# aleflabo/COSKAD

Hardware: AMD Instinct MI355X
Metric: pose_clips_per_sec_fwd_bwd (higher is better)
Workload: dtype f32; 1 GPU; euclidean_encoder_dynamicCenter train step (fwd+mse-to-centre+L2 reg+bwd+Adam), synthetic clips B=4096/GPU T=12 V=17 C=2, channels 2-32-16-32-64, latent 16; clips_per_gpu=4096, global_batch=4096, head=euclidean, parallelism=dp1, hip_graph=False

## Files before the change

coskad_amd/csrc/bottleneck.hip:

```cpp
#include "tile_ops.h"

namespace coskad {

constexpr int kBtlBlock = 256;
constexpr int kBtlWaves = kBtlBlock / 64;
constexpr int kBtlFwdWaves = 8;

__global__ __launch_bounds__(64 * kBtlFwdWaves) void k_btlnk_fwd(const float* __restrict__ U,
                                                     const float* __restrict__ W,
                                                     const float* __restrict__ bias,
                                                     const float* __restrict__ slope,
                                                     float* __restrict__ z, int B, int K, int L) {
  __shared__ float red[kBtlFwdWaves][256];
  const int lane = threadIdx.x & 63, wave = threadIdx.x >> 6;
  const int i = lane & 15, kk = lane >> 4;
  const int n = blockIdx.x * 16 + i;
  const bool pre = slope != nullptr;
  const float a = pre ? slope[0] : 0.f;
  const bool rowok = n < B, colok = i < L;
  const float* up = U + (size_t)(rowok ? n : 0) * K;
  const float* wp = W + (size_t)(colok ? i : 0) * K;
  const int nsteps = ceil_div(K, 16);
  const int per = ceil_div(nsteps, kBtlFwdWaves);
  const int s0 = wave * per, s1 = min(nsteps, s0 + per);
  f32x4 acc = {0.f, 0.f, 0.f, 0.f};
  constexpr int UB = 4;
  for (int sb = s0; sb < s1; sb += UB) {
    float4 x[UB], w[UB];
#pragma unroll
    for (int u = 0; u < UB; ++u) {
      const int k = (sb + u) * 16 + 4 * kk;
      const bool ok = sb + u < s1 && k < K;
      x[u] = (ok && rowok) ? *reinterpret_cast<const float4*>(up + k) : float4{0.f, 0.f, 0.f, 0.f};
      w[u] = (ok && colok) ? *reinterpret_cast<const float4*>(wp + k) : float4{0.f, 0.f, 0.f, 0.f};
    }
#pragma unroll
    for (int u = 0; u < UB; ++u) {
      float4 xv = x[u];
      if (pre) { xv.x = prelu_f(xv.x, a); xv.y = prelu_f(xv.y, a); xv.z = prelu_f(xv.z, a); xv.w = prelu_f(xv.w, a); }
      acc = __builtin_amdgcn_mfma_f32_16x16x4f32(xv.x, w[u].x, acc, 0, 0, 0);
      acc = __builtin_amdgcn_mfma_f32_16x16x4f32(xv.y, w[u].y, acc, 0, 0, 0);
      acc = __builtin_amdgcn_mfma_f32_16x16x4f32(xv.z, w[u].z, acc, 0, 0, 0);
      acc = __builtin_amdgcn_mfma_f32_16x16x4f32(xv.w, w[u].w, acc, 0, 0, 0);
    }
  }
#pragma unroll
  for (int r = 0; r < 4; ++r) red[wave][(4 * (lane >> 4) + r) * 16 + (lane & 15)] = acc[r];
  __syncthreads();
  const int e = threadIdx.x, row = (e >> 4) & 15, col = e & 15;
  const int nn = blockIdx.x * 16 + row;
  if (e < 256 && nn < B && col < L) {
    float s = 0.f;
#pragma unroll
// ... 124 lines not shown
#pragma unroll
    for (int g = 0; g < 4; ++g) {
      const int nn = n0 + c, j = 4 * g + q;
      const float av = (nn < nend && j < L) ? dz[(size_t)nn * L + j] : 0.f;
      dx[0] = __builtin_amdgcn_mfma_f32_16x16x4f32(av, wf[g].x, dx[0], 0, 0, 0);
      dx[1] = __builtin_amdgcn_mfma_f32_16x16x4f32(av, wf[g].y, dx[1], 0, 0, 0);
      dx[2] = __builtin_amdgcn_mfma_f32_16x16x4f32(av, wf[g].z, dx[2], 0, 0, 0);
      dx[3] = __builtin_amdgcn_mfma_f32_16x16x4f32(av, wf[g].w, dx[3], 0, 0, 0);
    }
#pragma unroll
    for (int s = 0; s < 4; ++s) {
      const int nn = n0 + 4 * q + s;
      const bool ok = kok && nn < nend;
      const float4 u = ucur[s];
      float4 x = u;
      if (pre) { x.x = prelu_f(u.x, a); x.y = prelu_f(u.y, a); x.z = prelu_f(u.z, a); x.w = prelu_f(u.w, a); }
      const float dzv = (nn < nend && c < L) ? dz[(size_t)nn * L + c] : 0.f;
      dw[0] = __builtin_amdgcn_mfma_f32_16x16x4f32(dzv, x.x, dw[0], 0, 0, 0);
      dw[1] = __builtin_amdgcn_mfma_f32_16x16x4f32(dzv, x.y, dw[1], 0, 0, 0);
      dw[2] = __builtin_amdgcn_mfma_f32_16x16x4f32(dzv, x.z, dw[2], 0, 0, 0);
      dw[3] = __builtin_amdgcn_mfma_f32_16x16x4f32(dzv, x.w, dw[3], 0, 0, 0);
      float4 g = {dx[0][s], dx[1][s], dx[2][s], dx[3][s]};
      if (pre) {
        da += (u.x < 0.f ? g.x * u.x : 0.f) + (u.y < 0.f ? g.y * u.y : 0.f) +
              (u.z < 0.f ? g.z * u.z : 0.f) + (u.w < 0.f ? g.w * u.w : 0.f);
        g.x = u.x > 0.f ? g.x : a * g.x; g.y = u.y > 0.f ? g.y : a * g.y;
        g.z = u.z > 0.f ? g.z : a * g.z; g.w = u.w > 0.f ? g.w : a * g.w;
      }
      if (ok) *reinterpret_cast<float4*>(dU + (size_t)nn * K + kc) = g;
    }
#pragma unroll
    for (int s = 0; s < 4; ++s) ucur[s] = unext[s];
  }
  if (kok) {
    float* dst = dWp + (size_t)blockIdx.y * L * K;
#pragma unroll
    for (int r = 0; r < 4; ++r) {
      const int j = 4 * q + r;
      if (j < L) *reinterpret_cast<float4*>(dst + (size_t)j * K + kc) = float4{dw[0][r], dw[1][r], dw[2][r], dw[3][r]};
    }
  }
  da = wave_sum(da);
  if (lane == 0) sred[wave] = da;
  __syncthreads();
  if (threadIdx.x == 0) dap[blockIdx.y * gridDim.x + blockIdx.x] = (sred[0] + sred[1]) + (sred[2] + sred[3]);
}

__global__ __launch_bounds__(256) void k_btlnk_reduce(const float* __restrict__ partials, int P, size_t E,
                                                       float* __restrict__ out, const float* __restrict__ dz,
                                                       int B, int L, float* __restrict__ db,
                                                       const float* __restrict__ dap, int nda,
                                                       float* __restrict__ dslope, int accumulate,
                                                       const float* __restrict__ rows, int RP, int RE,
                                                       double* __restrict__ rsum) {
  __shared__ double sh[256];
  const unsigned nE = (unsigned)((E + 255) / 256);
  if (blockIdx.x > nE + L) {
    const int col = threadIdx.x & 15, slice = threadIdx.x >> 4;
    const int e = (int)(blockIdx.x - (nE + L + 1)) * 16 + col;
    double s = 0.0;
    if (e < RE) {
      const float* base = rows + e;
      int p = slice;
      for (; p + 7 * 16 < RP; p += 8 * 16) {
        float v[8];
#pragma unroll
        for (int u = 0; u < 8; ++u) v[u] = base[(size_t)(p + 16 * u) * RE];
#pragma unroll
        for (int u = 0; u < 8; ++u) s += (double)v[u];
      }
      for (; p < RP; p += 16) s += (double)base[(size_t)p * RE];
    }
    sh[threadIdx.x] = s;
    __syncthreads();
    if (slice == 0 && e < RE) {
      double t = 0.0;
#pragma unroll
      for (int k = 0; k < 16; ++k) t += sh[col + 16 * k];
      rsum[e] = t;
    }
    return;
  }
  if (blockIdx.x < nE) {
    const size_t e = (size_t)blockIdx.x * 256 + threadIdx.x;
    if (e >= E) return;
    double s = 0.0;
    int p = 0;
    for (; p + 8 <= P; p += 8) {
      float v[8];
#pragma unroll
      for (int u = 0; u < 8; ++u) v[u] = partials[(size_t)(p + u) * E + e];
#pragma unroll
      for (int u = 0; u < 8; ++u) s += (double)v[u];
    }
    for (; p < P; ++p) s += (double)partials[(size_t)p * E + e];
    out[e] = accumulate ? out[e] + (float)s : (float)s;
    return;
  }
  const int r = (int)(blockIdx.x - nE);
  double s = 0.0;
  if (r < L) {
    if (!db) return;
    for (int n = threadIdx.x; n < B; n += 256) s += (double)dz[(size_t)n * L + r];
  } else {
    if (!dslope) return;
    for (int i = threadIdx.x; i < nda; i += 256) s += (double)dap[i];
  }
  sh[threadIdx.x] = s;
  __syncthreads();
  for (int w = 128; w > 0; w >>= 1) {
    if ((int)threadIdx.x < w) sh[threadIdx.x] += sh[threadIdx.x + w];
    __syncthreads();
  }
  if (threadIdx.x == 0) {
    float* o = r < L ? db + r : dslope;
    o[0] = accumulate ? o[0] + (float)sh[0] : (float)sh[0];
  }
}

static int btl_chunks(int B, int K) {
  const int gx = ceil_div(K, 256);
  int s = (1024 + gx / 2) / gx;
  const int smax = ceil_div(B, 16);
  if (s > smax) s = smax;
  if (s > 64) s = 64;
  return s < 1 ? 1 : s;
}

int launch_btlnk_reduce(const float* partials, int P, size_t E, float* out, const float* dz, int B, int L, float* db,
                        const float* dap, int nda, float* dslope, int accumulate, hipStream_t stream, const float* rows,
                        int RP, int RE, double* rsum) {
  const unsigned extra = rows ? (unsigned)ceil_div(RE, 16) : 0u;
  hipLaunchKernelGGL(k_btlnk_reduce, dim3((unsigned)((E + 255) / 256) + L + 1 + extra), dim3(256), 0, stream, partials, P, E, out, dz,
                     B, L, db, dap, nda, dslope, accumulate, rows, RP, RE, rsum);
  return check_launch("btlnk_bwd_reduce");
}

constexpr int kBtlWideMax = 512;
size_t wide_btlnk_fwd_ws_bytes(int B, int K, int L);
size_t wide_btlnk_bwd_ws_bytes(int B, int K, int L);
int wide_btlnk_fwd(const float* U, const float* W, const float* bias, const float* slope, float* z, void* ws, int B, int K, int L,
                   hipStream_t stream);
int wide_btlnk_bwd(const float* U, const float* W, const float* dz, const float* slope, float* dU, float* dW, float* db,
                   float* dslope, void* ws, int accumulate, int B, int K, int L, hipStream_t stream);

}

using namespace coskad;

extern "C" {

int coskad_btlnk_fwd_f32(const float* U, const float* W, const float* bias, const float* slope, float* z,
                         int B, int K, int L, hipStream_t stream) {
  if (!U || !W || !z) return fail(COSKAD_ERR_ARG, "btlnk_fwd: null pointer");
  if (B <= 0 || K <= 0 || L <= 0) return fail(COSKAD_ERR_ARG, "btlnk_fwd: B=%d K=%d L=%d", B, K, L);
  if (L > 16) return fail(COSKAD_ERR_SHAPE, "btlnk_fwd: latent_dim=%d > 16 needs the workspace entry point coskad_btlnk_fwd_ws_f32", L);
  if (K % 4) return fail(COSKAD_ERR_SHAPE, "btlnk_fwd: K=%d must be a multiple of 4", K);
  hipLaunchKernelGGL(k_btlnk_fwd, dim3(ceil_div(B, 16)), dim3(64 * kBtlFwdWaves), 0, stream, U, W, bias, slope, z, B, K, L);
  return check_launch("btlnk_fwd");
}

size_t coskad_btlnk_fwd_ws_bytes(int B) { return (size_t)kBtlKS * (size_t)(B > 0 ? B : 0) * 16 * sizeof(float); }

size_t coskad_btlnk_fwd_ws_bytes_l(int B, int K, int L) {
  if (L > 16 && L <= kBtlWideMax) return wide_btlnk_fwd_ws_bytes(B, K, L);
  return coskad_btlnk_fwd_ws_bytes(B);
}

int coskad_btlnk_fwd_ws_f32(const float* U, const float* W, const float* bias, const float* slope, float* z, void* ws,
                            size_t ws_bytes, int B, int K, int L, hipStream_t stream) {
  if (!U || !W || !z || !ws) return fail(COSKAD_ERR_ARG, "btlnk_fwd_ws: null pointer");
  if (B <= 0 || K <= 0 || L <= 0) return fail(COSKAD_ERR_ARG, "btlnk_fwd_ws: B=%d K=%d L=%d", B, K, L);
  if (L > kBtlWideMax) return fail(COSKAD_ERR_SHAPE, "btlnk_fwd_ws: latent_dim=%d > %d not supported", L, kBtlWideMax);
  if (L > 16) {
    if (ws_bytes < wide_btlnk_fwd_ws_bytes(B, K, L)) return fail(COSKAD_ERR_WORKSPACE, "btlnk_fwd_ws: workspace too small");
    return wide_btlnk_fwd(U, W, bias, slope, z, ws, B, K, L, stream);
  }
  if (K % 16) return fail(COSKAD_ERR_SHAPE, "btlnk_fwd_ws: K=%d must be a multiple of 16", K);
  if (ws_bytes < coskad_btlnk_fwd_ws_bytes(B)) return fail(COSKAD_ERR_WORKSPACE, "btlnk_fwd_ws: workspace too small");
  float* part = reinterpret_cast<float*>(ws);
  hipLaunchKernelGGL(k_btlnk_fwd_t, dim3(ceil_div(B, 64), kBtlKS), dim3(256), 0, stream, U, W, slope, part, B, K, L);
  int rc;
  if ((rc = check_launch("btlnk_fwd_t"))) return rc;
  hipLaunchKernelGGL(k_btlnk_fwd_sum, dim3(ceil_div(B * 16, 256)), dim3(256), 0, stream, part, bias, z, B, L, kBtlKS);
  return check_launch("btlnk_fwd_sum");
}

size_t coskad_btlnk_bwd_ws_bytes(int B, int K, int L) {
  if (L > 16 && L <= kBtlWideMax) return wide_btlnk_bwd_ws_bytes(B, K, L);
  const int S = btl_chunks(B, K);
  return ((size_t)S * L * K + (size_t)S * ceil_div(K, 256) + 64) * sizeof(float);
}

int coskad_btlnk_bwd_f32(const float* U, const float* W, const float* dz, const float* slope, float* dU,
                         float* dW, float* db, float* dslope, void* ws, size_t ws_bytes, int accumulate,
                         int B, int K, int L, hipStream_t stream) {
  if (!U || !W || !dz || !dU || !dW || !ws) return fail(COSKAD_ERR_ARG, "btlnk_bwd: null pointer");
  if (B <= 0 || K <= 0 || L <= 0) return fail(COSKAD_ERR_ARG, "btlnk_bwd: B=%d K=%d L=%d", B, K, L);
  if (L > kBtlWideMax) return fail(COSKAD_ERR_SHAPE, "btlnk_bwd: latent_dim=%d > %d not supported", L, kBtlWideMax);
  if (ws_bytes < coskad_btlnk_bwd_ws_bytes(B, K, L)) return fail(COSKAD_ERR_WORKSPACE, "btlnk_bwd: workspace too small");
  if (L > 16) return wide_btlnk_bwd(U, W, dz, slope, dU, dW, db, dslope, ws, accumulate, B, K, L, stream);
  if (K % 4) return fail(COSKAD_ERR_SHAPE, "btlnk_bwd: K=%d must be a multiple of 4", K);
  const int S = btl_chunks(B, K);
  const int chunk = round_up(ceil_div(B, S), 16);
  const int gx = ceil_div(K, 256);
  float* dWp = reinterpret_cast<float*>(ws);
  float* dap = dWp + (size_t)S * L * K;
  {
    ProbeScope probe(KID_BTLNK_BWD, 0, L, stream);
    hipLaunchKernelGGL(k_btlnk_bwd, dim3(gx, S), dim3(kBtlBlock), 0, stream, U, W, dz, slope, dU, dWp, dap, B, K, L, chunk);
  }
  int rc = check_launch("btlnk_bwd");
  if (rc) return rc;
  return launch_btlnk_reduce(dWp, S, (size_t)L * K, dW, dz, B, L, db, dap, gx * S, (dslope && slope) ? dslope : nullptr, accumulate, stream,
                             nullptr, 0, 0, nullptr);
}

}
```

coskad_amd/csrc/btlnk_chain.hip:

```cpp
#include "fused_ops.h"

namespace coskad {
namespace bc {

using ff::f32x4; using ff::mfma; using ff::BufRes; using ff::make_res; using ff::buf_load4; using ff::buf_load1;
__device__ __forceinline__ void buf_store1(BufRes r, int voff, int soff, float v) {
  __builtin_amdgcn_raw_buffer_store_b32(__float_as_uint(v), r, voff, soff, 0);
}

constexpr int HID = 64;
constexpr int PT = 16;
constexpr int NCL = 16;
constexpr int RSTR = 17;
constexpr int kThreads = 512;
#ifndef BC_XCD
#define BC_XCD 1
#endif
#ifndef BC_PF
#define BC_PF 1
#endif
#ifndef BC_SKIP
#define BC_SKIP 0
#endif

// ... 172 lines not shown
        if (j < L && pok) dst[(size_t)j * K + (ch0 + i) * TV] = dw[i][r];
      }
  }
  float* row = lds;
  float* red = lds + E;
  const float s4 = ssum + __shfl_xor(ssum, 16, 64);
  const float sch = s4 + __shfl_xor(s4, 32, 64);
  da = wave_sum(da);
  for (int hh = 0; hh < 2; ++hh) {
    if (h == hh) {
#pragma unroll
      for (int t = 0; t < CT; ++t)
#pragma unroll
        for (int r = 0; r < 4; ++r) {
          const int o = 16 * wc + 4 * q + r, cc = 16 * t + c;
          float* p = row + o * Ci + cc;
          p[0] = (hh ? p[0] : 0.f) + pacc[t][r];
          p[HID * Ci] = (hh ? p[HID * Ci] : 0.f) + qacc[t][r];
        }
      if (q == 0) {
        float* p = row + 2 * HID * Ci + 16 * wc + c;
        p[0] = (hh ? p[0] : 0.f) + sch;
      }
      if (lane == 0) red[wave] = da;
    }
    __syncthreads();
  }
  float* dstrow = prow + (size_t)wg * E;
  for (int e = tid; e < E; e += kThreads) dstrow[e] = row[e];
  if (tid == 0) dap[wg] = ((red[0] + red[1]) + (red[2] + red[3])) + ((red[4] + red[5]) + (red[6] + red[7]));
}

struct Plan {
  int npt, S, chunk;
};
static Plan plan(int B, int TV) {
  Plan p;
  p.npt = ceil_div(TV, PT);
  int s = 256 / p.npt;
  const int smax = ceil_div(B, NCL);
  if (s > smax) s = smax;
  if (s < 1) s = 1;
  p.chunk = round_up(ceil_div(B, s), NCL);
  p.S = ceil_div(B, p.chunk);
  return p;
}
static inline size_t sums_offset(int rows, int E) { return ((size_t)rows * E + 1) / 2 * 2; }

}

int launch_btlnk_reduce(const float* partials, int P, size_t E, float* out, const float* dz, int B, int L, float* db,
                        const float* dap, int nda, float* dslope, int accumulate, hipStream_t stream, const float* rows,
                        int RP, int RE, double* rsum);
}

using namespace coskad;

extern "C" {

int coskad_btlnk_bwd_chain_ok(int K, int TV, int below_Ci) {
  return TV > 0 && TV % 4 == 0 && K == bc::HID * TV && (below_Ci == 16 || below_Ci == 32);
}

int coskad_btlnk_bwd_chain_rows(int B, int TV) {
  if (B <= 0 || TV <= 0) return 0;
  const bc::Plan p = bc::plan(B, TV);
  return p.npt * p.S;
}

size_t coskad_btlnk_bwd_chain_floats(int B, int TV, int below_Ci) {
  const size_t E = 2 * (size_t)bc::HID * below_Ci + bc::HID;
  return bc::sums_offset(coskad_btlnk_bwd_chain_rows(B, TV), (int)E) + 2 * E;
}

size_t coskad_btlnk_bwd_chain_ws_bytes(int B, int K, int L, int TV) {
  if (B <= 0 || TV <= 0) return 0;
  const bc::Plan p = bc::plan(B, TV);
  return ((size_t)p.S * L * K + (size_t)p.S * p.npt + 64) * sizeof(float);
}

int coskad_btlnk_bwd_chain_f32(const float* U, const float* W, const float* dz, const float* slope, float* dU, float* dW,
                               float* db, float* dslope, void* ws, size_t ws_bytes, int accumulate, int B, int K, int L,
                               const float* below_in, const float* below_Z, const float* below_in_slope, int below_Ci, int TV,
                               float* stats_out, size_t stats_out_bytes, int* stats_rows, hipStream_t stream) {
  if (!U || !W || !dz || !dU || !dW || !ws || !below_in || !below_Z || !stats_out || !stats_rows)
    return fail(COSKAD_ERR_ARG, "btlnk_bwd_chain: null pointer");
  if (B <= 0 || K <= 0 || L <= 0) return fail(COSKAD_ERR_ARG, "btlnk_bwd_chain: B=%d K=%d L=%d", B, K, L);
  if (L > 16) return fail(COSKAD_ERR_SHAPE, "btlnk_bwd_chain: latent_dim=%d > 16 not supported", L);
  if (!coskad_btlnk_bwd_chain_ok(K, TV, below_Ci))
    return fail(COSKAD_ERR_SHAPE, "btlnk_bwd_chain: K=%d TV=%d below_Ci=%d (needs K = 64 TV, TV %% 4 == 0, 16 / 32 channels below)", K, TV, below_Ci);
  if ((size_t)stats_out & 7) return fail(COSKAD_ERR_ARG, "btlnk_bwd_chain: stats_out must be 8-byte aligned");
  if (ws_bytes < coskad_btlnk_bwd_chain_ws_bytes(B, K, L, TV)) return fail(COSKAD_ERR_WORKSPACE, "btlnk_bwd_chain: workspace too small");
  if (stats_out_bytes < coskad_btlnk_bwd_chain_floats(B, TV, below_Ci) * sizeof(float))
    return fail(COSKAD_ERR_WORKSPACE, "btlnk_bwd_chain: stats_out %zu bytes too small", stats_out_bytes);
  const bc::Plan p = bc::plan(B, TV);
  const int rows = p.npt * p.S;
  const int E = 2 * bc::HID * below_Ci + bc::HID;
  float* dWp = reinterpret_cast<float*>(ws);
  float* dap = dWp + (size_t)p.S * L * K;
  const size_t lds = (size_t)bc::NCL * ((bc::HID * bc::RSTR + 4) + (2 * below_Ci * bc::RSTR + 4)) * sizeof(float);
  int rc;
  {
  ProbeScope probe(KID_BTLNK_BWD, below_Ci, L, stream);
  if (below_Ci == 32) {
    auto k = bc::k_btlnk_bwd_stats<2>;
    (void)hipFuncSetAttribute((const void*)k, hipFuncAttributeMaxDynamicSharedMemorySize, (int)lds);
    hipLaunchKernelGGL(k, dim3(p.npt * p.S), dim3(bc::kThreads), lds, stream, U, W, dz, slope, dU, dWp, dap, below_in, below_Z,
                       below_in_slope, stats_out, B, TV, L, p.chunk);
  } else {
    auto k = bc::k_btlnk_bwd_stats<1>;
    (void)hipFuncSetAttribute((const void*)k, hipFuncAttributeMaxDynamicSharedMemorySize, (int)lds);
    hipLaunchKernelGGL(k, dim3(p.npt * p.S), dim3(bc::kThreads), lds, stream, U, W, dz, slope, dU, dWp, dap, below_in, below_Z,
                       below_in_slope, stats_out, B, TV, L, p.chunk);
  }
  }
  if ((rc = check_launch("btlnk_bwd_stats"))) return rc;
  *stats_rows = rows;
  return launch_btlnk_reduce(dWp, p.S, (size_t)L * K, dW, dz, B, L, db, dap, rows, (dslope && slope) ? dslope : nullptr, accumulate, stream,
                             stats_out, rows, E, reinterpret_cast<double*>(stats_out + bc::sums_offset(rows, E)));
}

}
```

coskad_amd/csrc/fused_apply_next.hip:

```cpp
#include "fused_ops.h"

#ifndef FN_ABLATE
#define FN_ABLATE 0
#endif

namespace coskad {
namespace fn {

using namespace ff;

struct FtabArgs {
  const float* A[4];
  const float* Tm[4];
  float* tab[4];
};
__global__ void k_build_ftab(FtabArgs args) {
  const int layer = blockIdx.y;
  const float* __restrict__ Aw = args.A[layer];
  const float* __restrict__ Tw = args.Tm[layer];
  const int e = blockIdx.x * blockDim.x + threadIdx.x;
  if (e >= LAYER_F4 * 4) return;
  float val = 0.f;
  if (e < TEMP_F4 * 4) {
    const int v = e / 256, l = (e >> 2) & 63, s = e & 3, j = l & 15, q = l >> 4;
    if (s < 3 && j < T) val = Tw[v * T * T + (4 * s + q) * T + j];
  } else {
    const int r = e - TEMP_F4 * 4;
    const int t = r / (3 * 256), c = (r / 256) % 3, l = (r >> 2) & 63, k = 4 * c + (r & 3), j = l & 15, q = l >> 4;
    if (k < 10) {
      const int s = k < 5 ? k : k - 5, w = 4 * s + q;
      if (w < V) val = Aw[t * V * V + w * V + (k < 5 ? j : 16)];
    }
  }
  args.tab[layer][e] = val;
}

template <int CT, int OTP>
__global__ __launch_bounds__(256, 1) void k_layer_apply_next(const float* __restrict__ in, const float* __restrict__ Zg,
                                                            const float* __restrict__ wfold, const float* __restrict__ bias,
                                                            const float* __restrict__ in_slope, const float* __restrict__ out_slope,
                                                            const float* __restrict__ ftab, float* __restrict__ out,
                                                            float* __restrict__ Znext, float* __restrict__ partials, int B) {
  constexpr int Ci = CT ? 16 * CT : 2, Co = 16 * OTP, CoP = Co, NG = 2 * CT;
  constexpr int NACC = OTP == 1 ? 2 : 3;
  constexpr int E = 2 * (Co * Co + Co);
  static_assert(OTP == 1 || OTP == 2, "the 32-row image holds the whole output");
  extern __shared__ __attribute__((aligned(16))) float lds_all[];
  const int lane = threadIdx.x & 63;
  const int wave = __builtin_amdgcn_readfirstlane(threadIdx.x >> 6);
  float* lds = lds_all + wave * WAVE_LDS_W;
  float* r1 = lds + R1;
  float* r2 = lds + R2;
  auto geo = [&]() {
    int l = lane;
    asm volatile("" : "+v"(l));
    return Lane{l & 15, l >> 4};
  };
  auto olane = [&]() {
    int l = lane;
    asm volatile("" : "+v"(l));
    return l;
  };
  const bool pre = in_slope != nullptr;
  const float a_in = pre ? in_slope[0] : 0.f;
  const float a_out = out_slope[0];
  const int l16 = lane * 16;
  const BufRes wres = make_res(wfold, 2 * Ci * CoP * 4u);
  const BufRes bres = make_res(bias, CoP * 4u);
  const BufRes tabres = make_res(ftab, LAYER_F4 * 16u);
  const int nwaves = gridDim.x * 4;
  auto clip_res = [&](const float* base, int c, int rows) {
    const bool in_range = c < B;
#ifdef COSKAD_HOT
    return make_res(base + (size_t)(in_range ? (c & 63) : 0) * rows * TV, in_range ? rows * TV * 4u : 0u);
#else
    return make_res(base + (size_t)(in_range ? c : 0) * rows * TV, in_range ? rows * TV * 4u : 0u);
#endif
  };
  constexpr int QTAIL = 4 * (TV / 4) - 192;
  const int l16t = lane < QTAIL ? l16 : 0x7ffffff0;
  float4 gb[16];
  auto qload = [&](const BufRes& res, int row0, int q) {
#pragma unroll
    for (int c = 0; c < 4; ++c) gb[4 * q + c] = buf_load4(res, c < 3 ? l16 : l16t, ((row0 + 4 * q) * (TV / 4) + 64 * c) * 16);
  };
  auto qstore = [&](int q, bool act) {
    const int ln = olane();
// ... 337 lines not shown
```

coskad_amd/csrc/fused_ops.h:

```cpp
#pragma once
#include "common.h"

namespace coskad {
namespace ff {

using f32x4 = __attribute__((ext_vector_type(4))) float;

constexpr int T = 12, V = 17, TV = T * V;
#ifndef FF_LD
#define FF_LD 206
#endif
constexpr int LD = FF_LD;
constexpr int R1 = 0, R2 = 32 * LD;
constexpr int PADCOL = TV;
constexpr int WAVE_LDS = 48 * LD;
constexpr int LDW = 208;
constexpr int WAVE_LDS_W = 32 * LD + 16 * LDW;
constexpr int NTILE = T + 1;
#ifndef FF_AB_UNROLL
#define FF_AB_UNROLL _Pragma("unroll")
#endif
#ifndef FF_ABLATE
#define FF_ABLATE 0
#endif
#ifndef FF_CABL
#define FF_CABL 0
#endif
#ifndef FF_TILE_FENCE
#define FF_TILE_FENCE
#endif
constexpr int KP = NTILE * 4 * 64 * 4;
constexpr int TEMP_F4 = V * 64;
constexpr int LAYER_F4 = TEMP_F4 + T * 3 * 64;
enum { W1A = 0, W1B = 2, WP = 4, WR = 12, WX3 = 20, WZ3 = 28, WZ4 = 36, WX4 = 68, B1 = 100, B2 = 108, B3 = 112, B4 = 120, NWREG = 136 };

__device__ __forceinline__ f32x4 mfma(float a, float b, f32x4 c) {
  return __builtin_amdgcn_mfma_f32_16x16x4f32(a, b, c, 0, 0, 0);
}
__device__ __forceinline__ float prelu(float x, float a) { return x > 0.f ? x : a * x; }
__device__ __forceinline__ f32x4 prelu4(f32x4 v, float a) {
  return f32x4{prelu(v[0], a), prelu(v[1], a), prelu(v[2], a), prelu(v[3], a)};
}

struct Lane {
  int j, q;
};

using u32x4 = __attribute__((ext_vector_type(4))) unsigned int;
using BufRes = __amdgpu_buffer_rsrc_t;
__device__ __forceinline__ BufRes make_res(const void* p, unsigned bytes) {
  return __builtin_amdgcn_make_buffer_rsrc(const_cast<void*>(p), 0, bytes, 0x00020000);
}
__device__ __forceinline__ float4 buf_load4(BufRes r, int voff, int soff) {
  const u32x4 v = __builtin_amdgcn_raw_buffer_load_b128(r, voff, soff, 0);
  return float4{__uint_as_float(v[0]), __uint_as_float(v[1]), __uint_as_float(v[2]), __uint_as_float(v[3])};
}
__device__ __forceinline__ float buf_load1(BufRes r, int voff, int soff) {
  return __uint_as_float(__builtin_amdgcn_raw_buffer_load_b32(r, voff, soff, 0));
}
__device__ __forceinline__ void buf_store4(BufRes r, int voff, int soff, const float4& v) {
  const u32x4 u = {__float_as_uint(v.x), __float_as_uint(v.y), __float_as_uint(v.z), __float_as_uint(v.w)};
  __builtin_amdgcn_raw_buffer_store_b128(u, r, voff, soff, 0);
}

struct TOp {
  float a0, a1, a2;
};
template <int ROWS, bool ACT = false>
__device__ __forceinline__ TOp temporal_read(const float* img, int rt, int v, const Lane& L, float slope = 0.f) {
  const float* p = img + (16 * rt + L.j) * LD + L.q * V + v;
  TOp o{p[0], p[4 * V], p[8 * V]};
  if (ACT) { o.a0 = prelu(o.a0, slope); o.a1 = prelu(o.a1, slope); o.a2 = prelu(o.a2, slope); }
  if (ROWS < 16) {
    const bool ok = L.j < ROWS;
    o.a0 = ok ? o.a0 : 0.f; o.a1 = ok ? o.a1 : 0.f; o.a2 = ok ? o.a2 : 0.f;
  }
  return o;
}
__device__ __forceinline__ f32x4 temporal_mm(const TOp& o, const float4& rec) {
  f32x4 acc = {0.f, 0.f, 0.f, 0.f};
  acc = mfma(o.a0, rec.x, acc);
  acc = mfma(o.a1, rec.y, acc);
  acc = mfma(o.a2, rec.z, acc);
  return acc;
}
template <int ROWS>
__device__ __forceinline__ void temporal_store(float* img, int rt, int v, const f32x4& acc, const Lane& L) {
// ... 229 lines not shown
```

coskad_amd/csrc/heads.hip:

```cpp
#include "tile_ops.h"
#include "heads_common.h"

namespace coskad {

struct Vec {
  float v[LMAX];
};

__device__ __forceinline__ Vec load_vec(const float* p, int L) {
  Vec r;
#pragma unroll
  for (int j = 0; j < LMAX; ++j) r.v[j] = j < L ? p[j] : 0.f;
  return r;
}
__device__ __forceinline__ void store_vec(float* p, const Vec& a, int L) {
#pragma unroll
  for (int j = 0; j < LMAX; ++j)
    if (j < L) p[j] = a.v[j];
}
__device__ __forceinline__ float dot(const Vec& a, const Vec& b) {
  float s = 0.f;
#pragma unroll
  for (int j = 0; j < LMAX; ++j) s = fmaf(a.v[j], b.v[j], s);
  return s;
// ... 31 lines not shown
  const float D = den + kMobiusEps;
  Vec m;
#pragma unroll
  for (int j = 0; j < LMAX; ++j) m.v[j] = (alpha * (-c.v[j]) + beta * p.v[j]) / D;
  const float mn = sqrtf(dot(m, m));
  const float mc = fminf(fmaxf(mn, -1.f + kArtanhEps), 1.f - kArtanhEps);
  const float d = (log1pf(mc) - log1pf(-mc));
  if (gp) {
    const float gmn = 2.f / (1.f - mc * mc);
    const float inv = mn > 0.f ? gmn / mn : 0.f;
    Vec gm;
#pragma unroll
    for (int j = 0; j < LMAX; ++j) gm.v[j] = inv * m.v[j];
    const float gD = -dot(gm, m) / D;
    float galpha = 0.f;
#pragma unroll
    for (int j = 0; j < LMAX; ++j) galpha = fmaf(gm.v[j] / D, -c.v[j], galpha);
#pragma unroll
    for (int j = 0; j < LMAX; ++j) {
      const float x = -c.v[j], y = p.v[j];
      gp->v[j] = beta * gm.v[j] / D + galpha * (2.f * x + 2.f * y) + gD * (2.f * x + 2.f * x2 * y);
    }
  }
  return d;
}

__device__ __forceinline__ Vec hyp_embed_bwd(const Vec& u, const Embed& em, const Vec& gp) {
  const float f = em.tn / em.un;
  Vec ge;
  if (em.clamped) {
    const float maxnorm = 1.f - kBallEps;
    const float en = em.en_raw;
    float egp = 0.f;
#pragma unroll
    for (int j = 0; j < LMAX; ++j) egp = fmaf(f * u.v[j], gp.v[j], egp);
#pragma unroll
    for (int j = 0; j < LMAX; ++j) ge.v[j] = maxnorm * (gp.v[j] / en - f * u.v[j] * egp / (en * en * en));
  } else {
    ge = gp;
  }
  Vec gu;
  float gf = dot(ge, u);
  float coef = 0.f;
  if (em.un_raw > kMinNorm) {
    const float sech2 = em.un < kTanhClamp ? 1.f - em.tn * em.tn : 0.f;
    const float df = (sech2 * em.un - em.tn) / (em.un * em.un);
    coef = gf * df / em.un_raw;
  }
#pragma unroll
  for (int j = 0; j < LMAX; ++j) gu.v[j] = f * ge.v[j] + coef * u.v[j];
  return gu;
}

constexpr int kHeadSlots = LMAX + 3;

constexpr int kHeadSingleRows = kFlatBlock;
__host__ __device__ inline int head_blocks(int B) { return B <= kHeadSingleRows ? 1 : ceil_div(B, kFlatBlock); }

__device__ __forceinline__ void block_partials(const float (&vals)[kHeadSlots], float* partials, float scale0, float* stats,
                                               float* acc) {
  __shared__ float sh[kFlatBlock / 64][kHeadSlots];
  const int lane = threadIdx.x & 63, wave = threadIdx.x >> 6;
#pragma unroll
  for (int k = 0; k < kHeadSlots; ++k) {
    const float s = wave_sum(vals[k]);
    if (lane == 0) sh[wave][k] = s;
  }
  __syncthreads();
  if (threadIdx.x < kHeadSlots) {
    float s = 0.f;
    for (int w = 0; w < kFlatBlock / 64; ++w) s += sh[w][threadIdx.x];
    if (gridDim.x == 1) {
      if (stats) stats[threadIdx.x] = threadIdx.x == 0 ? s * scale0 : s;
      if (acc) acc[threadIdx.x] += s;
    } else {
      partials[blockIdx.x * kHeadSlots + threadIdx.x] = s;
    }
  }
}

__global__ __launch_bounds__(kFlatBlock) void k_mse_head(const float* __restrict__ z,
                                                    const float* __restrict__ cvec,
                                                    float* __restrict__ dz, float* __restrict__ score,
                                                    float* __restrict__ partials, int B, int L,
                                                    float gscale, float scale0, float* __restrict__ stats,
                                                    float* __restrict__ acc) {
  float vals[kHeadSlots];
#pragma unroll
  for (int k = 0; k < kHeadSlots; ++k) vals[k] = 0.f;
  const Vec c = load_vec(cvec, L);
#pragma unroll 4
  for (int n = blockIdx.x * kFlatBlock + threadIdx.x; n < B; n += gridDim.x * kFlatBlock) {
    const Vec u = load_vec(z + (size_t)n * L, L);
    Vec g;
    float sq = 0.f;
#pragma unroll
    for (int j = 0; j < LMAX; ++j) {
      const float d = j < L ? u.v[j] - c.v[j] : 0.f;
      sq = fmaf(d, d, sq);
      g.v[j] = 2.f * d * gscale;
      vals[1 + j] += u.v[j];
    }
    vals[0] += sq;
    vals[LMAX + 1] += 1.f;
    vals[LMAX + 2] += sqrtf(dot(u, u));
    if (dz) store_vec(dz + (size_t)n * L, g, L);
    if (score) score[n] = sq / (float)L;
  }
  block_partials(vals, partials, scale0, stats, acc);
}

__global__ __launch_bounds__(kFlatBlock) void k_mahalanobis_head(const float* __restrict__ z,
                                                            const float* __restrict__ cvec,
                                                            const float* __restrict__ VI,
                                                            float* __restrict__ dz, float* __restrict__ score,
                                                            float* __restrict__ partials, int B, int L,
                                                            float gscale, float scale0, float* __restrict__ stats,
                                                            float* __restrict__ acc) {
  __shared__ float vi[LMAX * LMAX];
  for (int e = threadIdx.x; e < LMAX * LMAX; e += kFlatBlock) {
    const int r = e / LMAX, q = e - r * LMAX;
    vi[e] = (r < L && q < L) ? VI[r * L + q] : 0.f;
  }
  __syncthreads();
  float vals[kHeadSlots];
#pragma unroll
  for (int k = 0; k < kHeadSlots; ++k) vals[k] = 0.f;
  const Vec c = load_vec(cvec, L);
  for (int n = blockIdx.x * kFlatBlock + threadIdx.x; n < B; n += gridDim.x * kFlatBlock) {
    const Vec u = load_vec(z + (size_t)n * L, L);
    Vec d, w, wt;
#pragma unroll
    for (int j = 0; j < LMAX; ++j) { d.v[j] = j < L ? u.v[j] - c.v[j] : 0.f; w.v[j] = 0.f; wt.v[j] = 0.f; }
#pragma unroll
    for (int r = 0; r < LMAX; ++r)
#pragma unroll
      for (int q = 0; q < LMAX; ++q) {
        const float a = vi[r * LMAX + q];
        w.v[r] = fmaf(a, d.v[q], w.v[r]);
        wt.v[q] = fmaf(a, d.v[r], wt.v[q]);
      }
    const float dist = sqrtf(dot(d, w));
    vals[0] += dist;
#pragma unroll
    for (int j = 0; j < LMAX; ++j) vals[1 + j] += u.v[j];
    vals[LMAX + 1] += 1.f;
// ... 19 lines not shown
  for (int n0 = 0; n0 < B; n0 += CH) {
    const int nc = min(CH, B - n0);
    __syncthreads();
    for (int e = threadIdx.x; e < nc * L; e += LMAX * LMAX) {
      const int r = e / L, q = e - r * L;
      zs[r * LMAX + q] = z[(size_t)(n0 + r) * L + q];
    }
    __syncthreads();
    if (i < L && j < L)
      for (int r = 0; r < nc; ++r) s = fmaf(zs[r * LMAX + i], zs[r * LMAX + j], s);
  }
  if (i < L && j < L) gram[i * L + j] = accumulate ? gram[i * L + j] + s : s;
}

__global__ __launch_bounds__(kFlatBlock) void k_poincare_head(const float* __restrict__ z,
                                                         const float* __restrict__ cvec,
                                                         float* __restrict__ dz, float* __restrict__ zh,
                                                         float* __restrict__ score,
                                                         float* __restrict__ partials, int B, int L,
                                                         float gscale, float scale0, float* __restrict__ stats,
                                                         float* __restrict__ acc) {
  float vals[kHeadSlots];
#pragma unroll
  for (int k = 0; k < kHeadSlots; ++k) vals[k] = 0.f;
  for (int n = blockIdx.x * kFlatBlock + threadIdx.x; n < B; n += gridDim.x * kFlatBlock) {
    const Vec u = load_vec(z + (size_t)n * L, L);
    const Embed em = hyp_embed(u);
    if (zh) store_vec(zh + (size_t)n * L, em.p, L);
    const float y2 = dot(em.p, em.p);
    const float gamma = 2.f / (1.f - y2);
#pragma unroll
    for (int j = 0; j < LMAX; ++j) vals[1 + j] += gamma * em.p.v[j];
    vals[LMAX + 1] += gamma - 1.f;
    vals[LMAX + 2] += sqrtf(y2);
    if (cvec) {
      const Vec c = load_vec(cvec, L);
      Vec gp;
      const float d = poincare_dist(c, em.p, dz ? &gp : nullptr);
      vals[0] += d;
      if (score) score[n] = d;
      if (dz) {
#pragma unroll
        for (int j = 0; j < LMAX; ++j) gp.v[j] *= gscale;
        store_vec(dz + (size_t)n * L, hyp_embed_bwd(u, em, gp), L);
      }
    }
  }
  block_partials(vals, partials, scale0, stats, acc);
}

__global__ __launch_bounds__(64) void k_head_finalize(const float* __restrict__ partials, int P,
                                                       float scale0, float* __restrict__ stats,
                                                       float* __restrict__ acc) {
  const int k = threadIdx.x;
  if (k >= kHeadSlots) return;
  double s = 0.0;
  for (int p = 0; p < P; ++p) s += (double)partials[p * kHeadSlots + k];
  if (stats) stats[k] = (float)(k == 0 ? s * (double)scale0 : s);
  if (acc) acc[k] += (float)s;
}

__global__ __launch_bounds__(kFlatBlock) void k_poincare_dist(const float* __restrict__ zh,
                                                         const float* __restrict__ cvec,
                                                         float* __restrict__ score, int B, int L) {
  const int n = blockIdx.x * kFlatBlock + threadIdx.x;
  if (n >= B) return;
  const Vec p = load_vec(zh + (size_t)n * L, L), c = load_vec(cvec, L);
  score[n] = poincare_dist(c, p, nullptr);
}

__global__ __launch_bounds__(kFlatBlock) void k_poincare_logmap0(const float* __restrict__ y, float* __restrict__ out, int B, int L) {
  const int n = blockIdx.x * kFlatBlock + threadIdx.x;
  if (n >= B) return;
  const Vec p = load_vec(y + (size_t)n * L, L);
  const float yn = fmaxf(sqrtf(dot(p, p)), kMinNorm);
  const float yc = fminf(fmaxf(yn, -1.f + kArtanhEps), 1.f - kArtanhEps);
  const float at = 0.5f * (log1pf(yc) - log1pf(-yc));
  Vec o;
#pragma unroll
  for (int j = 0; j < LMAX; ++j) o.v[j] = p.v[j] / yn * at;
  store_vec(out + (size_t)n * L, o, L);
}

__global__ void k_midpoint_finalize(const float* __restrict__ acc, float* __restrict__ cvec, int L) {
  if (threadIdx.x != 0 || blockIdx.x != 0) return;
  const double s = fmax((double)acc[LMAX + 1], 1e-10);
  double m[LMAX], mn2 = 0.0;
  for (int j = 0; j < L; ++j) { m[j] = (double)acc[1 + j] / s; mn2 += m[j] * m[j]; }
  const double mn = fmax(sqrt(mn2), 1e-15);
  const double mc = fmin(mn, 1.0 - 1e-7);
  const double at = 0.5 * log((1.0 + mc) / (1.0 - mc));
  const double sc = tanh(0.5 * at) / mn;
  for (int j = 0; j < L; ++j) cvec[j] = (float)(sc * m[j]);
}

__global__ void k_center_finalize(const float* __restrict__ acc, float eps, float* __restrict__ cvec,
                                  int L) {
  const int j = threadIdx.x;
  if (j >= L || blockIdx.x != 0) return;
  float c = acc[1 + j] / acc[LMAX + 1];
  if (fabsf(c) < eps && c < 0.f) c = -eps;
  if (fabsf(c) < eps && c > 0.f) c = eps;
  cvec[j] = c;
}

__global__ __launch_bounds__(256) void k_sqnorm_masked(const float* __restrict__ p,
                                                        const float* __restrict__ mask, size_t n,
                                                        float* __restrict__ partials) {
  __shared__ float sh[4];
  float s = 0.f;
  for (size_t i = (size_t)blockIdx.x * 256 + threadIdx.x; i < n; i += (size_t)gridDim.x * 256) {
    const float v = p[i];
// ... 12 lines not shown
                                               float bc2_sqrt, float gscale, float reg_coef) {
  const size_t i = (size_t)blockIdx.x * 256 + threadIdx.x;
  if (i >= n) return;
  const float pi = p[i];
  float gi = g[i] * gscale;
  if (reg_coef != 0.f) gi = fmaf(reg_coef * (mask ? mask[i] : 1.f), pi, gi);
  const float mi = beta1 * m[i] + (1.f - beta1) * gi;
  const float vi = beta2 * v[i] + (1.f - beta2) * gi * gi;
  m[i] = mi;
  v[i] = vi;
  const float denom = sqrtf(vi) / bc2_sqrt + eps;
  p[i] = pi - (lr / bc1) * (mi / denom);
}

__global__ void k_adam_tick(float* __restrict__ hyper, float beta1, float beta2) {
  if (threadIdx.x == 0 && blockIdx.x == 0) {
    hyper[1] *= beta1;
    hyper[2] *= beta2;
  }
}

__global__ __launch_bounds__(256) void k_adam_dev(float* __restrict__ p, const float* __restrict__ g,
                                                   float* __restrict__ m, float* __restrict__ v,
                                                   const float* __restrict__ mask, size_t n,
                                                   const float* __restrict__ hyper, float beta1, float beta2,
                                                   float eps, float gscale, float reg_coef) {
  const size_t i = (size_t)blockIdx.x * 256 + threadIdx.x;
  if (i >= n) return;
  const float lr = hyper[0], bc1 = 1.f - hyper[1], bc2s = sqrtf(1.f - hyper[2]);
  const float pi = p[i];
  float gi = g[i] * gscale;
  if (reg_coef != 0.f) gi = fmaf(reg_coef * (mask ? mask[i] : 1.f), pi, gi);
  const float mi = beta1 * m[i] + (1.f - beta1) * gi;
  const float vi = beta2 * v[i] + (1.f - beta2) * gi * gi;
  m[i] = mi;
  v[i] = vi;
  p[i] = pi - (lr / bc1) * (mi / (sqrtf(vi) / bc2s + eps));
}

__global__ __launch_bounds__(256) void k_scale_sum(const float* __restrict__ v, int n, float scale,
                                                    float* __restrict__ out) {
  __shared__ double sh[256];
  double s = 0.0;
  for (int i = threadIdx.x; i < n; i += 256) s += (double)v[i];
  sh[threadIdx.x] = s;
  __syncthreads();
  for (int w = 128; w > 0; w >>= 1) {
    if (threadIdx.x < w) sh[threadIdx.x] += sh[threadIdx.x + w];
    __syncthreads();
  }
  if (threadIdx.x == 0) out[0] = (float)(sh[0] * (double)scale);
}

}

using namespace coskad;

extern "C" {

int coskad_head_slots(void) { return kHeadSlots; }
size_t coskad_head_ws_floats(int B) { return (size_t)ceil_div(B, kFlatBlock) * kHeadSlots; }
int coskad_head_slots_l(int L) { return L > 0 && L <= kWideLMax ? head_slots_for(L) : 0; }
size_t coskad_head_ws_floats_l(int B, int L) {
  if (L > LMAX && L <= kWideLMax) return wide_head_ws_floats(B, L);
  return coskad_head_ws_floats(B);
}

int coskad_mse_head_f32(const float* z, const float* c, float* dz, float* score, float* stats, float* acc,
                        float upstream, float* ws, int B, int L, hipStream_t stream) {
  if (!z || !c || !ws) return fail(COSKAD_ERR_ARG, "mse_head: null pointer");
  if (B <= 0 || L <= 0 || L > kWideLMax) return fail(COSKAD_ERR_SHAPE, "mse_head: B=%d latent=%d (max %d)", B, L, kWideLMax);
  if (L > LMAX) return wide_mse_head(z, c, dz, score, stats, acc, upstream, ws, B, L, stream);
  const int P = head_blocks(B);
  hipLaunchKernelGGL(k_mse_head, dim3(P), dim3(kFlatBlock), 0, stream, z, c, dz, score, ws, B, L,
                     upstream / ((float)B * (float)L), 1.f / ((float)B * (float)L), stats, acc);
  if ((stats || acc) && P > 1)
    hipLaunchKernelGGL(k_head_finalize, dim3(1), dim3(64), 0, stream, ws, P, 1.f / ((float)B * (float)L), stats, acc);
  return check_launch("mse_head");
}

int coskad_mahalanobis_head_f32(const float* z, const float* c, const float* VI, float* dz, float* score,
                                float* stats, float* acc, float* gram, int gram_accumulate, float upstream,
                                float* ws, int B, int L, hipStream_t stream) {
  if (!z || !c || !VI || !ws) return fail(COSKAD_ERR_ARG, "mahalanobis_head: null pointer");
  if (B <= 0 || L <= 0 || L > kWideLMax) return fail(COSKAD_ERR_SHAPE, "mahalanobis_head: B=%d latent=%d (max %d)", B, L, kWideLMax);
  if (L > LMAX) return wide_mahalanobis_head(z, c, VI, dz, score, stats, acc, gram, gram_accumulate, upstream, ws, B, L, stream);
  const int P = head_blocks(B);
  hipLaunchKernelGGL(k_mahalanobis_head, dim3(P), dim3(kFlatBlock), 0, stream, z, c, VI, dz, score, ws, B, L,
                     upstream / (float)B, 1.f / (float)B, stats, acc);
  if ((stats || acc) && P > 1)
    hipLaunchKernelGGL(k_head_finalize, dim3(1), dim3(64), 0, stream, ws, P, 1.f / (float)B, stats, acc);
  if (gram) hipLaunchKernelGGL(k_gram, dim3(1), dim3(LMAX * LMAX), 0, stream, z, gram, B, L, gram_accumulate);
  return check_launch("mahalanobis_head");
}

int coskad_poincare_head_f32(const float* z, const float* c, float* dz, float* zh, float* score,
                             float* stats, float* acc, float upstream, float* ws, int B, int L,
                             hipStream_t stream) {
  if (!z || !ws) return fail(COSKAD_ERR_ARG, "poincare_head: null pointer");
  if (B <= 0 || L <= 0 || L > kWideLMax) return fail(COSKAD_ERR_SHAPE, "poincare_head: B=%d latent=%d (max %d)", B, L, kWideLMax);
  if (L > LMAX) return wide_poincare_head(z, c, dz, zh, score, stats, acc, upstream, ws, B, L, stream);
  const int P = head_blocks(B);
  hipLaunchKernelGGL(k_poincare_head, dim3(P), dim3(kFlatBlock), 0, stream, z, c, dz, zh, score, ws, B, L,
                     upstream / (float)B, 1.f / (float)B, stats, acc);
  if ((stats || acc) && P > 1)
    hipLaunchKernelGGL(k_head_finalize, dim3(1), dim3(64), 0, stream, ws, P, 1.f / (float)B, stats, acc);
  return check_launch("poincare_head");
}

int coskad_poincare_dist_f32(const float* zh, const float* c, float* score, int B, int L, hipStream_t stream) {
  if (!zh || !c || !score) return fail(COSKAD_ERR_ARG, "poincare_dist: null pointer");
  if (B <= 0 || L <= 0 || L > kWideLMax) return fail(COSKAD_ERR_SHAPE, "poincare_dist: B=%d latent=%d (max %d)", B, L, kWideLMax);
  if (L > LMAX) return wide_poincare_dist(zh, c, score, B, L, stream);
  hipLaunchKernelGGL(k_poincare_dist, dim3(ceil_div(B, kFlatBlock)), dim3(kFlatBlock), 0, stream, zh, c, score, B, L);
  return check_launch("poincare_dist");
}

int coskad_poincare_logmap0_f32(const float* y, float* out, int B, int L, hipStream_t stream) {
  if (!y || !out) return fail(COSKAD_ERR_ARG, "poincare_logmap0: null pointer");
  if (B <= 0 || L <= 0 || L > kWideLMax) return fail(COSKAD_ERR_SHAPE, "poincare_logmap0: B=%d latent=%d (max %d)", B, L, kWideLMax);
  if (L > LMAX) return wide_poincare_logmap0(y, out, B, L, stream);
  hipLaunchKernelGGL(k_poincare_logmap0, dim3(ceil_div(B, kFlatBlock)), dim3(kFlatBlock), 0, stream, y, out, B, L);
  return check_launch("poincare_logmap0");
}

int coskad_center_finalize_f32(const float* acc, float* c, float eps, int L, hipStream_t stream) {
  if (!acc || !c || L <= 0 || L > kWideLMax) return fail(COSKAD_ERR_ARG, "center_finalize: bad argument (latent=%d, max %d)", L, kWideLMax);
// ... 52 lines not shown
```

coskad_amd/csrc/heads_common.h:

```cpp
#pragma once
#include "common.h"

namespace coskad {

constexpr int LMAX = 16;
constexpr int kWideLMax = 512;
constexpr float kMinNorm = 1e-5f;
constexpr float kBallEps = 1e-3f;
constexpr float kArtanhEps = 1e-5f;
constexpr float kMobiusEps = 1e-5f;
constexpr float kTanhClamp = 15.f;

__host__ __device__ inline int head_lp(int L) { return L > LMAX ? L : LMAX; }
__host__ __device__ inline int head_slots_for(int L) { return head_lp(L) + 3; }

size_t wide_head_ws_floats(int B, int L);
int wide_mse_head(const float* z, const float* c, float* dz, float* score, float* stats, float* acc, float upstream, float* ws,
                  int B, int L, hipStream_t stream);
int wide_mahalanobis_head(const float* z, const float* c, const float* VI, float* dz, float* score, float* stats, float* acc,
                          float* gram, int gram_accumulate, float upstream, float* ws, int B, int L, hipStream_t stream);
int wide_poincare_head(const float* z, const float* c, float* dz, float* zh, float* score, float* stats, float* acc,
                       float upstream, float* ws, int B, int L, hipStream_t stream);
int wide_poincare_dist(const float* zh, const float* c, float* score, int B, int L, hipStream_t stream);
int wide_poincare_logmap0(const float* y, float* out, int B, int L, hipStream_t stream);
int wide_center_finalize(const float* acc, float* c, float eps, int L, hipStream_t stream);
int wide_midpoint_finalize(const float* acc, float* c, int L, hipStream_t stream);

}
```

coskad_amd/csrc/stsgcn_train.hip:

```cpp
#include "mfma_ops.h"

namespace coskad {

constexpr int kMaxGrid = 768;

template <int T, int V, int NTC>
__global__ __launch_bounds__((Geo<T, V>::Block), (Geo<T, V>::Block <= 512 && NTC <= 2 ? 6 : 4)) void k_fwd_moments(const float* __restrict__ in,
                                                       const float* __restrict__ Aw,
                                                       const float* __restrict__ Tw,
                                                       const float* __restrict__ in_slope,
                                                       float* __restrict__ partials, int B, int Ci,
                                                       int NB, int need_x, float* __restrict__ Zout) {
  constexpr int kScratchFloats = Geo<T, V>::Scratch;
  constexpr int TV = Geo<T, V>::TV, LD = TV + 2;
  extern __shared__ __attribute__((aligned(16))) float lds[];
  float* scratch = lds;
  float* AwL = lds + max(NB * Ci * LD, kScratchFloats);
  float* TwL = AwL + T * V * V;
  copy_to_lds(AwL, Aw, T * V * V);
  copy_to_lds(TwL, Tw, V * T * T);
  const bool pre = in_slope != nullptr;
  const float a_in = pre ? in_slope[0] : 0.f;
  f32x4 mx[NTC][NTC], mz[NTC][NTC];
  float sx[NTC], sz[NTC];
  zero_acc(mx); zero_acc(mz);
#pragma unroll
  for (int t = 0; t < NTC; ++t) { sx[t] = 0.f; sz[t] = 0.f; }

  const int ntiles = ceil_div(B, NB);
  for (int tile = blockIdx.x; tile < ntiles; tile += gridDim.x) {
    const int clip0 = tile * NB;
    const int nb = min(NB, B - clip0);
    const int rows = nb * Ci;
    lds_barrier();
    stage_rows<T, V, LD>(in + (size_t)clip0 * Ci * TV, lds, rows * TV, pre, a_in);
    lds_barrier();
    if (need_x) {
      for (int n = 0; n < nb; ++n) moment_accum<T, V, NTC, LD>(lds + n * Ci * LD, Ci, mx, sx);
      lds_barrier();
    }
    gcn_mfma<T, V, false, LD>(lds, rows, AwL, TwL);
    lds_barrier();
    if (Zout) unstage_rows<T, V, LD>(Zout + (size_t)clip0 * Ci * TV, lds, rows * TV);
    for (int n = 0; n < nb; ++n) moment_accum<T, V, NTC, LD>(lds + n * Ci * LD, Ci, mz, sz);
  }
  float* dst = partials + (size_t)blockIdx.x * (2 * (Ci * Ci + Ci));
  store_moments<NTC>(mx, sx, scratch, dst, Ci, dst + Ci * Ci, Ci);
  store_moments<NTC>(mz, sz, scratch, dst + Ci * Ci + Ci, Ci, dst + 2 * Ci * Ci + Ci, Ci);
}

constexpr int kRedCols = 16;
__global__ __launch_bounds__(1024) void k_reduce_partials(const float* __restrict__ partials, int P, int E,
                                                           double* __restrict__ out) {
  __shared__ double sh[1024];
  const int e = blockIdx.x * kRedCols + (threadIdx.x % kRedCols);
  const double t = column_sum_f64<kRedCols>(partials, P, (size_t)E, e, e < E, sh);
  if ((int)threadIdx.x < kRedCols && e < E) out[e] = t;
}

__host__ __device__ inline int stat_floats(int Ci, int Co) { return 2 * Ci + 2 * Co * Ci + 4 * Co; }

#ifdef COSKAD_FOLD_TIMING
__device__ long long g_tfold_stamps[16];
#define TFOLD_STAMP(k) do { if (threadIdx.x == 0) g_tfold_stamps[k] = wall_clock64(); } while (0)
#else
#define TFOLD_STAMP(k) do {} while (0)
#endif

constexpr int kFoldSelfSum = 48;
__global__ __launch_bounds__(1024) void k_train_fold(
    const double* __restrict__ red, double npos, const float* __restrict__ Wt,
    const float* __restrict__ bt, const float* __restrict__ gs, const float* __restrict__ bs,
    float* __restrict__ rm_s, float* __restrict__ rv_s, long long* __restrict__ nbt_s,
    const float* __restrict__ Wr, const float* __restrict__ br, const float* __restrict__ gr,
    const float* __restrict__ brr, float* __restrict__ rm_r, float* __restrict__ rv_r,
    long long* __restrict__ nbt_r, float momentum, float* __restrict__ wfold,
    float* __restrict__ bias, float* __restrict__ stat, int Ci, int Co, int CoP,
    const float* __restrict__ parts, int P) {
  extern __shared__ double shd[];
  const bool ident = Wr == nullptr;
  const int CC = Co * Ci;
  double* Cl = shd;
  double* mul = shd + 2 * Ci * Ci;
  float* Wl = reinterpret_cast<float*>(mul + 2 * Ci);
  float* WCl = Wl + 2 * CC;
  float* meanl = WCl + 2 * CC;
  float* istdl = meanl + 2 * Co;
  __shared__ double red_l[kFoldSelfSum];
  if (parts) {
    __shared__ double shs[1024];
    const int E = 2 * (Ci * Ci + Ci);
    for (int e0 = 0; e0 < E; e0 += kRedCols) {
      const int e = e0 + (int)(threadIdx.x % kRedCols);
      const double t = column_sum_f64<kRedCols>(parts, P, (size_t)E, e, e < E, shs);
      if ((int)threadIdx.x < kRedCols && e < E) red_l[e] = t;
      __syncthreads();
    }
  }
  const double* redp = parts ? red_l : red;
  const double* MX = redp;
  const double* SX = redp + Ci * Ci;
  const double* MZ = redp + Ci * Ci + Ci;
  const double* SZ = redp + 2 * Ci * Ci + Ci;
  float* muX = stat;
  float* muZ = stat + Ci;
  float* WCs = stat + 2 * Ci;
  float* WCr = WCs + CC;
  float* mean_s = WCr + CC;
  float* istd_s = mean_s + Co;
  float* mean_r = istd_s + Co;
  float* istd_r = mean_r + Co;
  const double inv_n = 1.0 / npos;
  const int chunk = (Co + gridDim.x - 1) / gridDim.x;
  const int o_lo = blockIdx.x * chunk, o_hi = min(Co, o_lo + chunk), no = max(0, o_hi - o_lo);
  const bool first = blockIdx.x == 0;

  TFOLD_STAMP(0);
  for (int c = threadIdx.x; c < Ci; c += blockDim.x) {
    const double mz = SZ[c] * inv_n, mx = SX[c] * inv_n;
    mul[c] = mz;
    mul[Ci + c] = mx;
    if (first) { muZ[c] = (float)mz; muX[c] = (float)mx; }
  }
  for (int i = threadIdx.x; i < CC; i += blockDim.x) {
    Wl[i] = Wt[i];
    Wl[CC + i] = ident ? 0.f : Wr[i];
  }
  for (int i = threadIdx.x; i < Ci * Ci; i += blockDim.x) {
    const int k = i / Ci, c = i - k * Ci;
    Cl[i] = MZ[i] * inv_n - (SZ[k] * inv_n) * (SZ[c] * inv_n);
    Cl[Ci * Ci + i] = ident ? 0.0 : MX[i] * inv_n - (SX[k] * inv_n) * (SX[c] * inv_n);
  }
  __syncthreads();
  TFOLD_STAMP(1);
  const int Cq = (Ci + 3) / 4;
  for (int i = threadIdx.x; i < 2 * no * Cq; i += blockDim.x) {
    const int b = i / (no * Cq);
    const int j = i - b * no * Cq;
    const int o = o_lo + j / Cq, c0 = 4 * (j % Cq);
    double a0 = 0.0, a1 = 0.0, a2 = 0.0, a3 = 0.0;
    if (!(b == 1 && ident)) {
      const float* W = Wl + b * CC + o * Ci;
      const double* C = Cl + b * Ci * Ci + c0;
      if (c0 + 3 < Ci) {
        for (int k = 0; k < Ci; ++k) {
          const double w = (double)W[k];
          const double* r = C + k * Ci;
          a0 += w * r[0]; a1 += w * r[1]; a2 += w * r[2]; a3 += w * r[3];
        }
      } else {
        for (int k = 0; k < Ci; ++k) {
          const double w = (double)W[k];
          const double* r = C + k * Ci;
          a0 += w * r[0];
          if (c0 + 1 < Ci) a1 += w * r[1];
          if (c0 + 2 < Ci) a2 += w * r[2];
        }
      }
    }
    const double acc[4] = {a0, a1, a2, a3};
#pragma unroll
    for (int u = 0; u < 4; ++u)
      if (c0 + u < Ci) {
        const int e = b * CC + o * Ci + c0 + u;
        WCl[e] = (float)acc[u];
        (b ? WCr : WCs)[o * Ci + c0 + u] = (float)acc[u];
      }
  }
  __syncthreads();
  TFOLD_STAMP(2);
  const double unbias = npos > 1.0 ? npos / (npos - 1.0) : 1.0;
  for (int i0 = 0; i0 < 2 * no; i0 += blockDim.x / 8) {
    const int ii = i0 + (threadIdx.x >> 3), l8 = threadIdx.x & 7;
    const bool live = ii < 2 * no;
    const int b = live ? ii / no : 0, o = live ? o_lo + ii - b * no : 0;
    const int i = b * Co + o;
    double m = 0.0, var = 0.0;
    if (live && !(b == 1 && ident)) {
      const float* W = Wl + b * CC + o * Ci;
      const float* WC = WCl + b * CC + o * Ci;
      for (int k = l8; k < Ci; k += 8) {
        const double w = (double)W[k];
        m += w * mul[b * Ci + k];
        var += w * (double)WC[k];
      }
    }
#pragma unroll
    for (int off = 4; off > 0; off >>= 1) {
      m += __shfl_xor(m, off, 8);
      var += __shfl_xor(var, off, 8);
    }
    if (live && l8 == 0) {
      if (b == 1 && ident) { mean_r[o] = 0.f; istd_r[o] = 1.f; meanl[i] = 0.f; istdl[i] = 1.f; }
      else {
        const float* bb = b ? br : bt;
        m += bb ? (double)bb[o] : 0.0;
        var = var > 0.0 ? var : 0.0;
        const float mf = (float)m, isf = (float)(1.0 / sqrt(var + (double)kBnEps));
        (b ? mean_r : mean_s)[o] = mf;
        (b ? istd_r : istd_s)[o] = isf;
        meanl[i] = mf;
        istdl[i] = isf;
        float* rm = b ? rm_r : rm_s;
        float* rv = b ? rv_r : rv_s;
        if (rm) {
          rm[o] = (1.f - momentum) * rm[o] + momentum * (float)m;
          rv[o] = (1.f - momentum) * rv[o] + momentum * (float)(var * unbias);
        }
      }
    }
  }
  if (threadIdx.x == 0 && first) {
    if (nbt_s) nbt_s[0] += 1;
    if (nbt_r && !ident) nbt_r[0] += 1;
  }
  __syncthreads();
  TFOLD_STAMP(3);
  const bool last = blockIdx.x == gridDim.x - 1;
  const int w_hi = last ? CoP : min(o_lo + chunk, CoP), nw = max(0, w_hi - o_lo);
  for (int i = threadIdx.x; i < 2 * Ci * nw; i += blockDim.x) {
    const int row = i / nw, o = o_lo + i - row * nw;
    float w = 0.f;
    if (o < Co) {
      if (row < Ci) w = gs[o] * istdl[o] * Wl[o * Ci + row];
      else {
        const int c = row - Ci;
        w = ident ? (c == o ? 1.f : 0.f) : gr[o] * istdl[Co + o] * Wl[CC + o * Ci + c];
      }
    }
    wfold[row * CoP + o] = w;
  }
  for (int o = o_lo + threadIdx.x; o < w_hi; o += blockDim.x) {
    float b = 0.f;
    if (o < Co) {
      b = bs[o] + gs[o] * istdl[o] * ((bt ? bt[o] : 0.f) - meanl[o]);
      if (!ident) b += brr[o] + gr[o] * istdl[Co + o] * ((br ? br[o] : 0.f) - meanl[Co + o]);
    }
    bias[o] = b;
  }
  TFOLD_STAMP(4);
}

static int pick_nb_rows(int rows_per_clip, int B, int LD, int budget_bytes) {
  int nb = rows_per_clip >= 64 ? 1 : 64 / rows_per_clip;
  if (nb < 1) nb = 1;
  while (nb > 1 && (size_t)nb * rows_per_clip * LD * 4 > (size_t)budget_bytes) --nb;
  if (nb > B) nb = B;
  return nb;
}

int launch_first_moments(const float* in, const float* Aw, const float* Tw, const float* in_slope, float* partials, int B, int Ci,
                         int T, int V, float* Zout, int max_rows, hipStream_t st, int* rows_out);
bool fwd_moments_bpc_ok(int T_, int V_, int Ci);
int launch_fwd_moments_bpc(const float* in, const float* Aw, const float* Tw, const float* in_slope, float* partials, int B, int Ci,
                           int T_, int V_, int need_x, float* Zout, hipStream_t st, int* rows_out);

size_t train_stats_ws_bytes(int Ci) {
  const size_t E = 2 * ((size_t)Ci * Ci + Ci);
  return kMaxGrid * E * sizeof(float) + round_up((int)(E * sizeof(double)), 256) + 256;
}

static int launch_reduce_fold(const float* partials, int rows, double* red, double npos, const float* Wt, const float* bt,
                              const float* gs, const float* bs, float* rm_s, float* rv_s, long long* nbt_s, const float* Wr,
                              const float* br, const float* gr, const float* brr, float* rm_r, float* rv_r, long long* nbt_r,
                              float momentum, float* wfold, float* bias, float* stat, int Ci, int Co, hipStream_t st) {
  const int E = 2 * (Ci * Ci + Ci);
  int rc = 0;
  const bool self_sum = partials && Wt && E <= kFoldSelfSum;
  if (partials && !self_sum) {
    hipLaunchKernelGGL(k_reduce_partials, dim3(ceil_div(E, kRedCols)), dim3(1024), 0, st, partials, rows, E, red);
    if ((rc = check_launch("reduce_partials"))) return rc;
  }
  if (!Wt) return 0;
  const size_t fold_lds = (2 * (size_t)Ci * Ci + 2 * Ci) * sizeof(double) + (4 * (size_t)Co * Ci + 4 * Co) * sizeof(float);
  if (fold_lds > 64 * 1024) (void)hipFuncSetAttribute((const void*)k_train_fold, hipFuncAttributeMaxDynamicSharedMemorySize, (int)fold_lds);
  const int fold_blocks = Co >= 32 ? 8 : (Co >= 16 ? 4 : 1);
  hipLaunchKernelGGL(k_train_fold, dim3(fold_blocks), dim3(1024), fold_lds, st, red, npos, Wt, bt, gs, bs, rm_s,
                     rv_s, nbt_s, Wr, br, gr, brr, rm_r, rv_r, nbt_r, momentum, wfold, bias, stat, Ci,
                     Co, round_up(Co, 16), self_sum ? partials : (const float*)nullptr, rows);
  return check_launch("train_fold");
}

template <int T, int V>
static int launch_train_stats(const float* in, const float* Aw, const float* Tw, const float* in_slope,
                              const float* Wt, const float* bt, const float* gs, const float* bs,
                              float* rm_s, float* rv_s, long long* nbt_s, const float* Wr,
                              const float* br, const float* gr, const float* brr, float* rm_r,
                              float* rv_r, long long* nbt_r, float momentum, float* wfold, float* bias,
                              float* stat, void* ws, size_t ws_bytes, int B, int Ci, int Co,
                              hipStream_t st, float* Zout = nullptr, double* sums_out = nullptr, int need_x_sums = 1) {
  constexpr int kBlock = Geo<T, V>::Block;
  constexpr int kScratchFloats = Geo<T, V>::Scratch;
  constexpr int TV = Geo<T, V>::TV, LD = TV + 2;
  static_assert(TV % 4 == 0, "the moments kernel stages with float4 and needs TV + 2 == 2 (mod 4)");
  if (Ci > 64) return fail(COSKAD_ERR_SHAPE, "train_stats: C_in=%d > 64 not supported", Ci);
  if (ws_bytes < train_stats_ws_bytes(Ci))
    return fail(COSKAD_ERR_WORKSPACE, "train_stats: workspace %zu < %zu bytes", ws_bytes, train_stats_ws_bytes(Ci));
  const int E = 2 * (Ci * Ci + Ci);
  int NB = Ci >= 32 ? 1 : 32 / Ci;
  if (NB > B) NB = B;
  const size_t img = (size_t)NB * Ci * LD > (size_t)kScratchFloats ? (size_t)NB * Ci * LD : (size_t)kScratchFloats;
  const size_t lds = (img + (size_t)T * V * V + (size_t)V * T * T) * sizeof(float);
  if (lds > (size_t)kMaxLdsBytes) return fail(COSKAD_ERR_SHAPE, "train_stats: LDS %zu too large", lds);
  const int ntiles = ceil_div(B, NB);
  const int per_cu = lds <= (size_t)52 * 1024 && Ci <= 32 && kBlock <= 512 ? 3 : (lds <= (size_t)80 * 1024 ? 2 : 1);
  const int grid = ntiles < 256 * per_cu ? ntiles : 256 * per_cu;
  float* partials = reinterpret_cast<float*>(ws);
  double* red = reinterpret_cast<double*>(reinterpret_cast<char*>(ws) + round_up((int)(kMaxGrid * (size_t)E * sizeof(float)), 256));
  const int need_x = sums_out ? need_x_sums : (Wr != nullptr);
  const int ntc = ceil_div(Ci, 16);
  int rows = grid;
  if (Zout && Ci <= 4 && TV % 4 == 0) {
    int rc1 = launch_first_moments(in, Aw, Tw, in_slope, partials, B, Ci, T, V, Zout, kMaxGrid, st, &rows);
    if (rc1) return rc1;
  } else if (Zout && fwd_moments_bpc_ok(T, V, Ci)) {
    ProbeScope probe(KID_FWD_MOMENTS, Ci, Co, st);
    int rc1 = launch_fwd_moments_bpc(in, Aw, Tw, in_slope, partials, B, Ci, T, V, need_x, Zout, st, &rows);
    if (rc1) return rc1;
  } else {
#define LAUNCH_M(NTC)                                                                           \
  do {                                                                                          \
    auto k = k_fwd_moments<T, V, NTC>;                                                          \
    if (lds > 64 * 1024) (void)hipFuncSetAttribute((const void*)k, hipFuncAttributeMaxDynamicSharedMemorySize, (int)lds); \
    hipLaunchKernelGGL(k, dim3(grid), dim3(kBlock), lds, st, in, Aw, Tw, in_slope, partials, B, Ci, NB, need_x, Zout); \
  } while (0)
  {
  ProbeScope probe(KID_FWD_MOMENTS, Ci, Co, st);
  if (ntc == 1) LAUNCH_M(1);
  else if (ntc == 2) LAUNCH_M(2);
  else if (ntc == 3) LAUNCH_M(3);
  else LAUNCH_M(4);
  }
#undef LAUNCH_M
  }
  int rc = check_launch("fwd_moments");
  if (rc) return rc;
  if (sums_out)
    return launch_reduce_fold(partials, rows, sums_out, 0.0, nullptr, nullptr, nullptr, nullptr, nullptr, nullptr, nullptr, nullptr,
                              nullptr, nullptr, nullptr, nullptr, nullptr, nullptr, 0.f, nullptr, nullptr, nullptr, Ci, Co, st);
  return launch_reduce_fold(partials, rows, red, (double)B * TV, Wt, bt, gs, bs, rm_s, rv_s, nbt_s, Wr, br, gr, brr, rm_r, rv_r,
                            nbt_r, momentum, wfold, bias, stat, Ci, Co, st);
}

}

using namespace coskad;

extern "C" {

size_t coskad_train_stats_ws_bytes(int Ci) { return train_stats_ws_bytes(Ci); }
int coskad_stat_floats(int Ci, int Co) { return stat_floats(Ci, Co); }

int coskad_layer_train_stats_f32(const float* in, const float* A, const float* Tm, const float* in_slope,
                                 const float* Wt, const float* bt, const float* gamma_t,
                                 const float* beta_t, float* rmean_t, float* rvar_t, long long* nbt_t,
                                 const float* Wr, const float* br, const float* gamma_r,
                                 const float* beta_r, float* rmean_r, float* rvar_r, long long* nbt_r,
                                 float momentum, float* wfold, float* bias, float* stat, void* ws,
                                 size_t ws_bytes, int B, int Ci, int Co, int T, int V,
                                 hipStream_t stream) {
  if (!in || !A || !Tm || !Wt || !gamma_t || !beta_t || !wfold || !bias || !stat || !ws)
    return fail(COSKAD_ERR_ARG, "layer_train_stats: null pointer");
  if (Wr && (!gamma_r || !beta_r)) return fail(COSKAD_ERR_ARG, "layer_train_stats: residual BN missing");
  if (!Wr && Ci != Co) return fail(COSKAD_ERR_ARG, "layer_train_stats: identity residual needs Ci == Co");
  if (B <= 0 || Ci <= 0 || Co <= 0) return fail(COSKAD_ERR_ARG, "layer_train_stats: B=%d Ci=%d Co=%d", B, Ci, Co);
#define CALL(T_, V_)                                                                                   \
  return launch_train_stats<T_, V_>(in, A, Tm, in_slope, Wt, bt, gamma_t, beta_t, rmean_t, rvar_t, nbt_t, \
                                    Wr, br, gamma_r, beta_r, rmean_r, rvar_r, nbt_r, momentum, wfold, \
                                    bias, stat, ws, ws_bytes, B, Ci, Co, stream)
  COSKAD_DISPATCH_TV(T, V, CALL);
#undef CALL
}

int coskad_layer_train_stats_z_f32(const float* in, const float* A, const float* Tm, const float* in_slope,
                                 const float* Wt, const float* bt, const float* gamma_t,
                                 const float* beta_t, float* rmean_t, float* rvar_t, long long* nbt_t,
                                 const float* Wr, const float* br, const float* gamma_r,
                                 const float* beta_r, float* rmean_r, float* rvar_r, long long* nbt_r,
                                 float momentum, float* wfold, float* bias, float* stat, void* ws,
                                 size_t ws_bytes, int B, int Ci, int Co, int T, int V,
                                 hipStream_t stream, float* Z) {
  if (!in || !A || !Tm || !Wt || !gamma_t || !beta_t || !wfold || !bias || !stat || !ws)
    return fail(COSKAD_ERR_ARG, "layer_train_stats: null pointer");
  if (Wr && (!gamma_r || !beta_r)) return fail(COSKAD_ERR_ARG, "layer_train_stats: residual BN missing");
  if (!Wr && Ci != Co) return fail(COSKAD_ERR_ARG, "layer_train_stats: identity residual needs Ci == Co");
  if (B <= 0 || Ci <= 0 || Co <= 0) return fail(COSKAD_ERR_ARG, "layer_train_stats: B=%d Ci=%d Co=%d", B, Ci, Co);
#define CALL(T_, V_)                                                                                   \
  return launch_train_stats<T_, V_>(in, A, Tm, in_slope, Wt, bt, gamma_t, beta_t, rmean_t, rvar_t, nbt_t, \
                                    Wr, br, gamma_r, beta_r, rmean_r, rvar_r, nbt_r, momentum, wfold, \
                                    bias, stat, ws, ws_bytes, B, Ci, Co, stream, Z)
  COSKAD_DISPATCH_TV(T, V, CALL);
#undef CALL
}

int coskad_layer_train_fold_f32(const float* partials, int rows, const float* Wt, const float* bt, const float* gamma_t,
                                const float* beta_t, float* rmean_t, float* rvar_t, long long* nbt_t,
                                const float* Wr, const float* br, const float* gamma_r,
                                const float* beta_r, float* rmean_r, float* rvar_r, long long* nbt_r,
                                float momentum, float* wfold, float* bias, float* stat, void* ws,
                                size_t ws_bytes, int B, int Ci, int Co, int T, int V, hipStream_t stream) {
  if (!partials || !Wt || !gamma_t || !beta_t || !wfold || !bias || !stat || !ws)
    return fail(COSKAD_ERR_ARG, "layer_train_fold: null pointer");
  if (Wr && (!gamma_r || !beta_r)) return fail(COSKAD_ERR_ARG, "layer_train_fold: residual BN missing");
  if (!Wr && Ci != Co) return fail(COSKAD_ERR_ARG, "layer_train_fold: identity residual needs Ci == Co");
  if (B <= 0 || Ci <= 0 || Co <= 0 || Ci > 64 || rows <= 0) return fail(COSKAD_ERR_ARG, "layer_train_fold: B=%d Ci=%d Co=%d rows=%d", B, Ci, Co, rows);
  const size_t E = 2 * ((size_t)Ci * Ci + Ci);
  if (ws_bytes < round_up((int)(E * sizeof(double)), 256)) return fail(COSKAD_ERR_WORKSPACE, "layer_train_fold: workspace %zu too small", ws_bytes);
  return launch_reduce_fold(partials, rows, reinterpret_cast<double*>(ws), (double)B * T * V, Wt, bt, gamma_t, beta_t, rmean_t,
                            rvar_t, nbt_t, Wr, br, gamma_r, beta_r, rmean_r, rvar_r, nbt_r, momentum, wfold, bias, stat, Ci, Co,
                            stream);
}


int coskad_layer_train_moments_f32(const float* in, const float* A, const float* Tm, const float* in_slope, float* Z, double* sums,
                                   void* ws, size_t ws_bytes, int B, int Ci, int T, int V, hipStream_t stream) {
  if (!in || !A || !Tm || !sums || !ws) return fail(COSKAD_ERR_ARG, "layer_train_moments: null pointer");
  if (B <= 0 || Ci <= 0) return fail(COSKAD_ERR_ARG, "layer_train_moments: B=%d Ci=%d", B, Ci);
  if ((size_t)sums & 7) return fail(COSKAD_ERR_ARG, "layer_train_moments: sums must be 8-byte aligned");
#define CALL(T_, V_)                                                                                                       \
  return launch_train_stats<T_, V_>(in, A, Tm, in_slope, nullptr, nullptr, nullptr, nullptr, nullptr, nullptr, nullptr, nullptr, \
                                    nullptr, nullptr, nullptr, nullptr, nullptr, nullptr, 0.f, nullptr, nullptr, nullptr, ws,     \
                                    ws_bytes, B, Ci, Ci, stream, Z, sums, 1)
  COSKAD_DISPATCH_TV(T, V, CALL);
#undef CALL
}

int coskad_layer_moment_sums_f32(const float* partials, int rows, int Ci, double* sums, hipStream_t stream) {
  if (!partials || !sums || rows <= 0 || Ci <= 0 || Ci > 64) return fail(COSKAD_ERR_ARG, "layer_moment_sums: bad argument");
  if ((size_t)sums & 7) return fail(COSKAD_ERR_ARG, "layer_moment_sums: sums must be 8-byte aligned");
  return launch_reduce_fold(partials, rows, sums, 0.0, nullptr, nullptr, nullptr, nullptr, nullptr, nullptr, nullptr, nullptr,
                            nullptr, nullptr, nullptr, nullptr, nullptr, nullptr, 0.f, nullptr, nullptr, nullptr, Ci, Ci, stream);
}

int coskad_layer_train_fold_sums_f32(const double* sums, double count, const float* Wt, const float* bt, const float* gamma_t,
                                     const float* beta_t, float* rmean_t, float* rvar_t, long long* nbt_t,
                                     const float* Wr, const float* br, const float* gamma_r,
                                     const float* beta_r, float* rmean_r, float* rvar_r, long long* nbt_r,
                                     float momentum, float* wfold, float* bias, float* stat, int Ci, int Co, hipStream_t stream) {
  if (!sums || !Wt || !gamma_t || !beta_t || !wfold || !bias || !stat) return fail(COSKAD_ERR_ARG, "layer_train_fold_sums: null pointer");
  if (Wr && (!gamma_r || !beta_r)) return fail(COSKAD_ERR_ARG, "layer_train_fold_sums: residual BN missing");
  if (!Wr && Ci != Co) return fail(COSKAD_ERR_ARG, "layer_train_fold_sums: identity residual needs Ci == Co");
  if (count <= 0.0 || Ci <= 0 || Co <= 0 || Ci > 64) return fail(COSKAD_ERR_ARG, "layer_train_fold_sums: count=%g Ci=%d Co=%d", count, Ci, Co);
  return launch_reduce_fold(nullptr, 0, const_cast<double*>(sums), count, Wt, bt, gamma_t, beta_t, rmean_t, rvar_t, nbt_t, Wr, br,
                            gamma_r, beta_r, rmean_r, rvar_r, nbt_r, momentum, wfold, bias, stat, Ci, Co, stream);
}

#ifdef COSKAD_FOLD_TIMING
// ... 5 lines not shown
```

coskad_amd/engine.py:

```python
from __future__ import annotations

import os
from dataclasses import dataclass, field
from typing import Dict, List, Optional

import torch

from . import ops

Tensor = torch.Tensor


@dataclass
class LayerTensors:
    A: Tensor
    T: Tensor
    Wt: Tensor
    bt: Optional[Tensor]
    gt: Tensor
    bet: Tensor
    rm_t: Tensor
    rv_t: Tensor
    nbt_t: Tensor
    Wr: Optional[Tensor]
# ... 45 lines not shown
            ns.append("bt")
        ns += ["gt", "bet"]
        if self.Wr is not None:
            ns.append("Wr")
            if self.br is not None:
                ns.append("br")
            ns += ["gr", "ber"]
        ns.append("slope")
        return ns


class Workspace:

    def __init__(self) -> None:
        self.buf: Optional[Tensor] = None

    def get(self, nbytes: int, device) -> Tensor:
        if self.buf is None or self.buf.numel() < nbytes or self.buf.device != device:
            self.buf = torch.empty(int(nbytes), dtype=torch.uint8, device=device)
        return self.buf


@dataclass
class ChainCtx:
    inputs: List[Tensor] = field(default_factory=list)
    stats: List[Tensor] = field(default_factory=list)
    zs: List[Optional[Tensor]] = field(default_factory=list)
    in_slope: Optional[Tensor] = None
    sync: object = None
    sync_count: float = 0.0


EVAL_FIRST_PAIR = True


def chain_forward(x: Tensor, layers: List[LayerTensors], training: bool, ws: Workspace,
                  in_slope: Optional[Tensor] = None, want_ctx: bool = False, sync=None, pending0=None):
    B, C, T, V = x.shape
    ctx = ChainCtx(in_slope=in_slope) if want_ctx else None
    sync_count = None
    batch_stats = [training or L.rm_t is None for L in layers]
    if sync is not None and training:
        import torch.distributed as dist
        if not STORE_Z:
            raise ValueError("SyncBN runs on the stored-Z training path")
        cnt = torch.tensor([float(B * T * V)], device=x.device, dtype=torch.float64)
        dist.all_reduce(cnt, group=sync)
        sync_count = float(cnt.item())
        if ctx is not None:
            ctx.sync, ctx.sync_count = sync, sync_count
    h, slope = x, in_slope
    n = len(layers)
    fuse = [False] * n
    ftab = None
    if all(batch_stats) and STORE_Z and FUSE_NEXT:
        for i in range(n - 1):
            fuse[i] = layers[i + 1].Ci == layers[i].Co and ops.layer_apply_next_ok(layers[i].Ci, layers[i].Co, T, V)
        nxt = [i + 1 for i in range(n - 1) if fuse[i]]
        if nxt:
            ftab = torch.empty(n, ops.ftab_floats(), device=x.device, dtype=torch.float32)
            for k in range(0, len(nxt), 4):
                grp = nxt[k:k + 4]
                ops.build_ftabs([layers[i].A for i in grp], [layers[i].T for i in grp], [ftab[i] for i in grp])
    fuse_flat = [False] * n
    if all(batch_stats) and STORE_Z and FUSE_NEXT and sync is None:
        for i in range(n - 1):
            fuse_flat[i] = (not fuse[i] and layers[i + 1].Ci == layers[i].Co and layers[i].Wr is not None
                            and ops.layer_apply_next_flat_ok(layers[i].Ci, layers[i].Co, T, V))
    def eval_fold(L):
        key = L.fold_key() if L.cache is not None else None
        if key is not None and L.cache.get("key") == key:
            return L.cache["fold"]
        wb = ops.bn_fold(L.w2(L.Wt), L.bt, L.gt, L.bet, L.rm_t, L.rv_t, L.w2(L.Wr), L.br, L.gr, L.ber, L.rm_r, L.rv_r)
        if key is not None:
            L.cache["key"], L.cache["fold"] = key, wb
        return wb

    skip = -1
    pending = pending0
    if pending0 is not None and not (batch_stats[0] and STORE_Z and sync is None):
        raise ValueError("chain_forward: pending0 is for the stored-Z training path without SyncBN")
    for i, L in enumerate(layers):
        if i == skip:
            continue
        if h.shape[1] != L.Ci:
            raise ValueError(f"layer expects {L.Ci} input channels, got {h.shape[1]}")
        Z = None
        if batch_stats[i]:
            if L.cache:
                L.cache.clear()
            buf = ws.get(ops.train_stats_ws_bytes(L.Ci), x.device)
            if sync_count is not None:
                if pending is not None:
                    Z, partials, rows = pending
                    sums = ops.layer_moment_sums(partials, rows, L.Ci)
                else:
                    Z = torch.empty_like(h)
                    sums = ops.layer_train_moments(h, L.A, L.T, slope, buf, Z=Z)
                dist.all_reduce(sums, group=sync)
                wfold, bias, stat = ops.layer_train_fold_sums(
                    sums, sync_count, L.w2(L.Wt), L.bt, L.gt, L.bet, L.rm_t, L.rv_t, L.nbt_t,
                    L.w2(L.Wr), L.br, L.gr, L.ber, L.rm_r, L.rv_r, L.nbt_r, momentum=L.step_momentum())
            elif pending is not None:
                Z, partials, rows = pending
                wfold, bias, stat = ops.layer_train_fold(
                    partials, rows, B, T, V, L.w2(L.Wt), L.bt, L.gt, L.bet, L.rm_t, L.rv_t, L.nbt_t,
                    L.w2(L.Wr), L.br, L.gr, L.ber, L.rm_r, L.rv_r, L.nbt_r, buf, momentum=L.step_momentum())
            else:
                if STORE_Z:
                    Z = torch.empty_like(h)
                wfold, bias, stat = ops.layer_train_stats(
                    h, L.A, L.T, slope, L.w2(L.Wt), L.bt, L.gt, L.bet, L.rm_t, L.rv_t, L.nbt_t,
                    L.w2(L.Wr), L.br, L.gr, L.ber, L.rm_r, L.rv_r, L.nbt_r, buf, momentum=L.step_momentum(), Z=Z)
        else:
            wfold, bias = eval_fold(L)
            stat = None
            if (EVAL_FIRST_PAIR and i == 0 and ctx is None and slope is None and n > 1 and not batch_stats[1] and layers[1].Ci == L.Co
                    and L.Wr is not None and wfold.shape[1] == L.Co
                    and ops.layer_first_pair_ok(L.Ci, L.Co, layers[1].Co, T, V)):
                N = layers[1]
                wf2, b2 = eval_fold(N)
                if wf2.shape[1] == N.Co:
                    h = ops.layer_first_pair_apply(h, L.A, L.T, wfold, bias, N.A, N.T, wf2, b2, L.Co, N.Co, L.slope)
                    slope, skip = N.slope, 1
                    continue
        pending = None
        if fuse[i]:
            rows_max = ops.layer_apply_next_rows(B, h.shape[1], L.Co)
            partials = torch.empty(rows_max * 2 * (L.Co * L.Co + L.Co), device=x.device, dtype=torch.float32)
            u, Zn, rows = ops.layer_apply_next(Z, h, wfold, bias, L.Co, slope, L.slope, ftab[i + 1], partials, T, V)
            pending = (Zn, partials, rows)
        elif fuse_flat[i] and Z is not None:
            u, Zn, partials, rows = ops.layer_apply_next_flat(Z, h, wfold, bias, L.Co, slope, L.slope, layers[i + 1].A, layers[i + 1].T)
            pending = (Zn, partials, rows)
        elif Z is not None:
            u = ops.layer_apply_z(Z, h, L.A, L.T, wfold, bias, L.Co, in_slope=slope)
        else:
            u = ops.layer_apply(h, L.A, L.T, wfold, bias, L.Co, in_slope=slope)
        if ctx is not None:
            ctx.inputs.append(h)
            ctx.stats.append(stat)
            ctx.zs.append(Z)
        h, slope = u, L.slope
    return h, ctx


STORE_Z = True
FUSE_BELOW = True
CHAIN_SKIP = frozenset()
FUSE_TOP = True
FUSE_NEXT = True


class SideStream:

    def __init__(self) -> None:
        self.stream: Optional[torch.cuda.Stream] = None
        self.dz = [None, None]
        self.ws = None
        self.done = [None, None]

    def ensure(self, nfloats: int, ws_bytes: int, device) -> None:
        if self.stream is None:
            self.stream = torch.cuda.Stream(device=device)
        for k in range(2):
            if self.dz[k] is None or self.dz[k].numel() < nfloats:
                self.dz[k] = torch.empty(nfloats, device=device, dtype=torch.float32)
        if self.ws is None or self.ws.numel() < ws_bytes:
            self.ws = torch.empty(ws_bytes, device=device, dtype=torch.uint8)


def btlnk_backward(ctx: Optional[ChainCtx], layers: List[LayerTensors], U: Tensor, W: Tensor, dz: Tensor, slope: Optional[Tensor],
                   dW: Tensor, db: Optional[Tensor], dslope: Optional[Tensor], ws: Workspace):
    B = U.shape[0]
    K, L = U.numel() // B, W.shape[0]
    i = len(layers) - 1 if layers else -1
    Z = ctx.zs[i] if (ctx is not None and ctx.zs and i >= 0) else None
    if (FUSE_TOP and Z is not None and U.dim() == 4 and layers[i].Wr is not None and L <= 16
            and ops.btlnk_bwd_chain_ok(K, U.shape[2] * U.shape[3], layers[i].Ci)):
        in_slope = layers[i - 1].slope if i > 0 else ctx.in_slope
        return ops.btlnk_bwd_chain(U, W, dz, slope, dW, db, dslope, ws, ctx.inputs[i], Z, in_slope)
    buf = ws.get(ops.btlnk_bwd_ws_bytes(B, K, L), U.device)
    return ops.btlnk_bwd(U, W, dz, slope, dW, db, dslope, buf), None


def chain_backward(ctx: ChainCtx, layers: List[LayerTensors], dU: Tensor, ws: Workspace,
                   grads: List[Dict[str, Tensor]], need_dx: bool, accumulate: bool = False,
                   side: Optional[SideStream] = None, stats_in=None, in_slope_grad: Optional[Tensor] = None) -> Optional[Tensor]:
    n = len(layers)
    if side is not None and stats_in is not None:
        raise ValueError("chain_backward: the side-stream path runs its own batch reductions (stats_in must be None)")
    if ctx.sync is not None and side is not None:
        raise ValueError("SyncBN runs on the main stream (side=None)")
    main = torch.cuda.current_stream() if side is not None else None
    if side is not None:
        side.done = [None, None]
    for i in range(n - 1, -1, -1):
        L = layers[i]
        x_in = ctx.inputs[i]
        B, Ci, T, V = x_in.shape
        in_slope = layers[i - 1].slope if i > 0 else ctx.in_slope
        g = dict(grads[i])
        g.pop("slope", None)
        if i > 0:
            g["slope_in"] = grads[i - 1]["slope"]
        elif in_slope_grad is not None and in_slope is not None:
            g["slope_in"] = in_slope_grad
        want_dx = need_dx or i > 0
        buf = ws.get(ops.layer_bwd_ws_bytes(B, Ci, L.Co, T, V), x_in.device)
        args = (x_in, dU, L.A, L.T, in_slope, ctx.stats[i], L.w2(L.Wt), L.gt, L.w2(L.Wr), L.gr, _as2d(g), buf)
        if side is None:
            sync = ctx.sync
            if sync is not None:
                import torch.distributed as dist
                if stats_in is None:
                    stats_in = ops.layer_bwd_stats(x_in, dU, L.A, L.T, in_slope, L.Wr is not None, buf, Z=ctx.zs[i])
                dist.all_reduce(ops.chain_sums(stats_in[0], stats_in[1], Ci, L.Co), group=sync)
            below = None
            Zi = ctx.zs[i] if ctx.zs else None
            if (FUSE_BELOW and i not in CHAIN_SKIP and Zi is not None and i > 0 and ctx.zs[i - 1] is not None
                    and in_slope is not None and layers[i - 1].Wr is not None):
                cb = ctx.inputs[i - 1].shape[1]
                rows = ops.layer_bwd_below_rows(B, Ci, L.Co, cb, T, V)
                if rows:
                    below = (ctx.inputs[i - 1], ctx.zs[i - 1], layers[i - 2].slope if i > 1 else ctx.in_slope,
                             torch.empty(ops.layer_bwd_below_floats(B, Ci, L.Co, cb, T, V), device=x_in.device, dtype=torch.float32))
            dIn = ops.layer_bwd(*args, need_dx=want_dx, accumulate=accumulate, Z=Zi,
                                stats_in=stats_in, below=below, stats_count=ctx.sync_count if sync is not None else 0.0)
            stats_in = (below[3], rows) if below is not None else None
        else:
            k = i & 1
            side.ensure(max(x.numel() for x in ctx.inputs), ops.layer_gcn_params_ws_bytes(T, V), x_in.device)
            if side.done[k] is not None:
                main.wait_event(side.done[k])
            dz = side.dz[k][:x_in.numel()].view(B, Ci, T, V)
            dIn = ops.layer_bwd_data(*args, dZ=dz, need_dx=want_dx, accumulate=accumulate, Z=ctx.zs[i] if ctx.zs else None)
# ... 68 lines not shown
```

coskad_amd/ops.py:

```python
from __future__ import annotations

import ctypes
from typing import Optional

import torch

from . import _lib
from ._lib import call, i32, ptr

Tensor = torch.Tensor


def _stream() -> ctypes.c_void_p:
    return ctypes.c_void_p(torch.cuda.current_stream().cuda_stream)


def _chk(t: Optional[Tensor], name: str, shape=None, dtype=torch.float32, optional=False) -> None:
    if t is None:
        if optional:
            return
        raise ValueError(f"{name}: tensor required")
    if not t.is_cuda:
        raise _lib.CoskadHipError(f"{name}: expected a CUDA (ROCm) tensor, got device {t.device}; "
                                  "the COSKAD hot path runs only on the HIP extension (no CPU fallback)")
# ... 37 lines not shown


def layer_apply(x: Tensor, A: Tensor, Tm: Tensor, wfold: Tensor, bias: Tensor, Co: int,
                in_slope: Optional[Tensor] = None, out_slope: Optional[Tensor] = None,
                out: Optional[Tensor] = None) -> Tensor:
    B, Ci, T, V = x.shape
    _chk(x, "x"); _chk(A, "A", (T, V, V)); _chk(Tm, "T", (V, T, T))
    _chk(wfold, "wfold", (2 * Ci, cop(Co))); _chk(bias, "bias", (cop(Co),))
    _chk(in_slope, "in_slope", (1,), optional=True); _chk(out_slope, "out_slope", (1,), optional=True)
    if out is None:
        out = torch.empty(B, Co, T, V, device=x.device, dtype=torch.float32)
    else:
        _chk(out, "out", (B, Co, T, V))
    call("coskad_layer_apply_f32", ptr(x), ptr(out), ptr(A), ptr(Tm), ptr(wfold), ptr(bias),
         ptr(in_slope), ptr(out_slope), i32(B), i32(Ci), i32(Co), i32(T), i32(V), _stream(), tag=(Ci, Co))
    return out


def layer_first_pair_ok(Ci: int, Cm: int, Co: int, T: int, V: int) -> bool:
    return bool(_lib.lib().coskad_layer_first_pair_ok(i32(T), i32(V), i32(Ci), i32(Cm), i32(Co)))


def layer_first_pair_apply(x: Tensor, A1: Tensor, T1: Tensor, wfold1: Tensor, bias1: Tensor, A2: Tensor, T2: Tensor, wfold2: Tensor,
                           bias2: Tensor, Cm: int, Co: int, mid_slope: Tensor, out_slope: Optional[Tensor] = None) -> Tensor:
    B, Ci, T, V = x.shape
    _chk(x, "x", (B, 2, T, V)); _chk(A1, "A1", (T, V, V)); _chk(T1, "T1", (V, T, T)); _chk(A2, "A2", (T, V, V)); _chk(T2, "T2", (V, T, T))
    _chk(wfold1, "wfold1", (4, Cm)); _chk(bias1, "bias1", (Cm,)); _chk(wfold2, "wfold2", (2 * Cm, Co)); _chk(bias2, "bias2", (Co,))
    _chk(mid_slope, "mid_slope", (1,)); _chk(out_slope, "out_slope", (1,), optional=True)
    out = torch.empty(B, Co, T, V, device=x.device, dtype=torch.float32)
    call("coskad_layer_first_pair_apply_f32", ptr(x), ptr(out), ptr(A1), ptr(T1), ptr(wfold1), ptr(bias1), ptr(A2), ptr(T2), ptr(wfold2),
         ptr(bias2), ptr(mid_slope), ptr(out_slope), i32(B), i32(Cm), i32(Co), i32(T), i32(V), _stream())
    return out


def layer_fits(Ci: int, Co: int, T: int, V: int) -> bool:
    fn = _lib.lib().coskad_layer_fits
    fn.restype = ctypes.c_int
    return bool(fn(i32(Ci), i32(Co), i32(T), i32(V)))


def stat_floats(Ci: int, Co: int) -> int:
    fn = _lib.lib().coskad_stat_floats
    fn.restype = ctypes.c_int
    return fn(i32(Ci), i32(Co))


def train_stats_ws_bytes(Ci: int) -> int:
    fn = _lib.lib().coskad_train_stats_ws_bytes
    fn.restype = ctypes.c_size_t
    return fn(i32(Ci))


def layer_train_stats(x, A, Tm, in_slope, Wt, bt, gt, bet, rm_t, rv_t, nbt_t,
                      Wr, br, gr, ber, rm_r, rv_r, nbt_r, ws, momentum: float = 0.1, Z: Optional[Tensor] = None):
    B, Ci, T, V = x.shape
    Co = Wt.shape[0]
    _chk(x, "x"); _chk(A, "A", (T, V, V)); _chk(Tm, "T", (V, T, T))
    _chk(Wt, "Wt", (Co, Ci)); _chk(gt, "gamma_t", (Co,)); _chk(bet, "beta_t", (Co,))
    for n, t in (("bt", bt), ("rm_t", rm_t), ("rv_t", rv_t), ("br", br), ("gamma_r", gr), ("beta_r", ber),
                 ("rm_r", rm_r), ("rv_r", rv_r)):
        _chk(t, n, (Co,), optional=True)
    _chk(Wr, "Wr", (Co, Ci), optional=True)
    _chk(in_slope, "in_slope", (1,), optional=True)
    _chk(nbt_t, "nbt_t", (), dtype=torch.int64, optional=True)
    _chk(nbt_r, "nbt_r", (), dtype=torch.int64, optional=True)
    need = train_stats_ws_bytes(Ci)
    if ws is None or ws.numel() * ws.element_size() < need:
        raise ValueError(f"workspace too small: need {need} bytes")
    wfold = torch.empty(2 * Ci, cop(Co), device=x.device, dtype=torch.float32)
    bias = torch.empty(cop(Co), device=x.device, dtype=torch.float32)
    stat = torch.empty(stat_floats(Ci, Co), device=x.device, dtype=torch.float32)
    _chk(Z, "Z", tuple(x.shape), optional=True)
    args = (ptr(x), ptr(A), ptr(Tm), ptr(in_slope), ptr(Wt), ptr(bt), ptr(gt),
            ptr(bet), ptr(rm_t), ptr(rv_t), ptr(nbt_t), ptr(Wr), ptr(br), ptr(gr), ptr(ber), ptr(rm_r),
            ptr(rv_r), ptr(nbt_r), ctypes.c_float(momentum), ptr(wfold), ptr(bias), ptr(stat), ptr(ws),
            ctypes.c_size_t(ws.numel() * ws.element_size()), i32(B), i32(Ci), i32(Co), i32(T), i32(V), _stream())
    if Z is None:
        call("coskad_layer_train_stats_f32", *args)
    else:
        call("coskad_layer_train_stats_z_f32", *args, ptr(Z))
    return wfold, bias, stat


def layer_train_moments(x, A, Tm, in_slope, ws, Z: Optional[Tensor] = None) -> Tensor:
    B, Ci, T, V = x.shape
    _chk(x, "x"); _chk(A, "A", (T, V, V)); _chk(Tm, "T", (V, T, T)); _chk(in_slope, "in_slope", (1,), optional=True)
    _chk(Z, "Z", tuple(x.shape), optional=True)
    need = train_stats_ws_bytes(Ci)
    if ws is None or _bytes(ws) < need:
        raise ValueError(f"workspace too small: need {need} bytes")
    sums = torch.empty(2 * (Ci * Ci + Ci), device=x.device, dtype=torch.float64)
    call("coskad_layer_train_moments_f32", ptr(x), ptr(A), ptr(Tm), ptr(in_slope), ptr(Z), ptr(sums), ptr(ws),
         ctypes.c_size_t(_bytes(ws)), i32(B), i32(Ci), i32(T), i32(V), _stream())
    return sums


def layer_moment_sums(partials: Tensor, rows: int, Ci: int) -> Tensor:
    _chk(partials, "partials")
    if partials.numel() < rows * 2 * (Ci * Ci + Ci):
        raise ValueError("layer_moment_sums: partials smaller than rows x 2 (Ci^2 + Ci)")
    sums = torch.empty(2 * (Ci * Ci + Ci), device=partials.device, dtype=torch.float64)
    call("coskad_layer_moment_sums_f32", ptr(partials), i32(rows), i32(Ci), ptr(sums), _stream())
    return sums


def layer_train_fold_sums(sums, count, Wt, bt, gt, bet, rm_t, rv_t, nbt_t, Wr, br, gr, ber, rm_r, rv_r, nbt_r, momentum: float = 0.1):
    Co, Ci = Wt.shape
    _chk(sums, "sums", (2 * (Ci * Ci + Ci),), dtype=torch.float64); _chk(Wt, "Wt", (Co, Ci)); _chk(gt, "gamma_t", (Co,)); _chk(bet, "beta_t", (Co,))
    for n, t in (("bt", bt), ("rm_t", rm_t), ("rv_t", rv_t), ("br", br), ("gamma_r", gr), ("beta_r", ber), ("rm_r", rm_r), ("rv_r", rv_r)):
        _chk(t, n, (Co,), optional=True)
    _chk(Wr, "Wr", (Co, Ci), optional=True)
    _chk(nbt_t, "nbt_t", (), dtype=torch.int64, optional=True); _chk(nbt_r, "nbt_r", (), dtype=torch.int64, optional=True)
    wfold = torch.empty(2 * Ci, cop(Co), device=Wt.device, dtype=torch.float32)
    bias = torch.empty(cop(Co), device=Wt.device, dtype=torch.float32)
    stat = torch.empty(stat_floats(Ci, Co), device=Wt.device, dtype=torch.float32)
    call("coskad_layer_train_fold_sums_f32", ptr(sums), ctypes.c_double(float(count)), ptr(Wt), ptr(bt), ptr(gt), ptr(bet), ptr(rm_t),
         ptr(rv_t), ptr(nbt_t), ptr(Wr), ptr(br), ptr(gr), ptr(ber), ptr(rm_r), ptr(rv_r), ptr(nbt_r), ctypes.c_float(momentum),
         ptr(wfold), ptr(bias), ptr(stat), i32(Ci), i32(Co), _stream())
    return wfold, bias, stat


def layer_bwd_stats(x_in, dU, A, Tm, in_slope, has_residual: bool, ws, Z=None):
    B, Ci, T, V = x_in.shape
    Co = dU.shape[1]
    _chk(x_in, "x_in"); _chk(dU, "dU", (B, Co, T, V)); _chk(A, "A", (T, V, V)); _chk(Tm, "T", (V, T, T))
    _chk(in_slope, "in_slope", (1,), optional=True); _chk(Z, "Z", (B, Ci, T, V), optional=True)
    need = layer_bwd_ws_bytes(B, Ci, Co, T, V)
    if ws is None or _bytes(ws) < need:
        raise ValueError(f"workspace too small: need {need} bytes")
    fn = _lib.lib().coskad_layer_bwd_stats_floats
    fn.restype = ctypes.c_size_t
    buf = torch.empty(fn(i32(B), i32(Ci), i32(Co), i32(T), i32(V)), device=x_in.device, dtype=torch.float32)
    rows = ctypes.c_int(0)
    call("coskad_layer_bwd_stats_f32", ptr(x_in), ptr(dU), ptr(A), ptr(Tm), ptr(in_slope), i32(1 if has_residual else 0), ptr(buf),
         ctypes.c_size_t(_bytes(buf)), ctypes.byref(rows), ptr(ws), ctypes.c_size_t(_bytes(ws)), i32(B), i32(Ci), i32(Co), i32(T), i32(V),
         _stream(), ptr(Z))
    return buf, rows.value


def chain_sums(buf: Tensor, rows: int, Ci: int, Co: int) -> Tensor:
    fn = _lib.lib().coskad_layer_bwd_sums_offset
    fn.restype = ctypes.c_size_t
    off = fn(i32(rows), i32(Ci), i32(Co))
    E = 2 * Co * Ci + Co
    return buf[off:off + 2 * E].view(torch.float64)


def layer_apply_z(Z, x, A, Tm, wfold, bias, Co, in_slope=None, out_slope=None, out=None):
    B, Ci, T, V = x.shape
    _chk(x, "x"); _chk(Z, "Z", (B, Ci, T, V)); _chk(wfold, "wfold", (2 * Ci, cop(Co))); _chk(bias, "bias", (cop(Co),))
    _chk(in_slope, "in_slope", (1,), optional=True); _chk(out_slope, "out_slope", (1,), optional=True)
    if out is None:
        out = torch.empty(B, Co, T, V, device=x.device, dtype=torch.float32)
    _chk(A, "A", (T, V, V)); _chk(Tm, "T", (V, T, T))
    call("coskad_layer_apply_z_f32", ptr(Z), ptr(x), ptr(out), ptr(A), ptr(Tm), ptr(wfold), ptr(bias), ptr(in_slope), ptr(out_slope),
         i32(B), i32(Ci), i32(Co), i32(T), i32(V), _stream())
    return out


def layer_apply_next_ok(Ci: int, Co: int, T: int, V: int) -> bool:
    fn = _lib.lib().coskad_layer_apply_next_ok
    fn.restype = ctypes.c_int
    return bool(fn(i32(Ci), i32(Co), i32(T), i32(V)))


def layer_apply_next_rows(B: int, Ci: int, Co: int) -> int:
    fn = _lib.lib().coskad_layer_apply_next_rows
    fn.restype = ctypes.c_int
    return fn(i32(B), i32(Ci), i32(Co))


def ftab_floats() -> int:
    fn = _lib.lib().coskad_ftab_floats
    fn.restype = ctypes.c_int
    return fn()


def build_ftabs(As, Ts, tabs) -> None:
    n = len(As)
    if not (1 <= n <= 4) or len(Ts) != n or len(tabs) != n:
        raise ValueError("build_ftabs: 1..4 layers, equal list lengths")
    T, V = As[0].shape[0], As[0].shape[1]
    nf = ftab_floats()
    for A, Tm, tab in zip(As, Ts, tabs):
        _chk(A, "A", (T, V, V)); _chk(Tm, "T", (V, T, T)); _chk(tab, "tab", (nf,))
    arr = ctypes.c_void_p * n
    call("coskad_build_ftab_f32", arr(*[t.data_ptr() for t in As]), arr(*[t.data_ptr() for t in Ts]),
         arr(*[t.data_ptr() for t in tabs]), i32(n), i32(T), i32(V), _stream())


def layer_apply_next(Z, x, wfold, bias, Co, in_slope, out_slope, ftab_next, partials, T, V, out=None, Z_next=None):
    B, Ci = x.shape[0], x.shape[1]
    _chk(x, "x", (B, Ci, T, V)); _chk(Z, "Z", (B, Ci, T, V)); _chk(wfold, "wfold", (2 * Ci, cop(Co))); _chk(bias, "bias", (cop(Co),))
    _chk(in_slope, "in_slope", (1,), optional=True); _chk(out_slope, "out_slope", (1,)); _chk(ftab_next, "ftab_next", (ftab_floats(),))
    _chk(partials, "partials")
    if out is None:
        out = torch.empty(B, Co, T, V, device=x.device, dtype=torch.float32)
    if Z_next is None:
        Z_next = torch.empty(B, Co, T, V, device=x.device, dtype=torch.float32)
    _chk(out, "out", (B, Co, T, V)); _chk(Z_next, "Z_next", (B, Co, T, V))
    rows = layer_apply_next_rows(B, Ci, Co)
    call("coskad_layer_apply_next_f32", ptr(Z), ptr(x), ptr(out), ptr(wfold), ptr(bias), ptr(in_slope), ptr(out_slope),
         ptr(ftab_next), ptr(Z_next), ptr(partials), ctypes.c_size_t(_bytes(partials)), i32(B), i32(Ci), i32(Co), i32(T), i32(V),
         _stream(), tag=(Ci, Co))
    return out, Z_next, rows


def layer_apply_next_flat_ok(Ci: int, Co: int, T: int, V: int) -> bool:
    return bool(_lib.lib().coskad_layer_apply_next_flat_ok(i32(Ci), i32(Co), i32(T), i32(V)))


def layer_apply_next_flat(Z, x, wfold, bias, Co, in_slope, out_slope, A_next, T_next):
    B, Ci, T, V = x.shape
    _chk(x, "x"); _chk(Z, "Z", (B, Ci, T, V)); _chk(wfold, "wfold", (2 * Ci, cop(Co))); _chk(bias, "bias", (cop(Co),))
    _chk(in_slope, "in_slope", (1,), optional=True); _chk(out_slope, "out_slope", (1,))
    _chk(A_next, "A_next", (T, V, V)); _chk(T_next, "T_next", (V, T, T))
    rows = int(_lib.lib().coskad_layer_apply_next_flat_rows(i32(B)))
    out = torch.empty(B, Co, T, V, device=x.device, dtype=torch.float32)
    Zn = torch.empty(B, Co, T, V, device=x.device, dtype=torch.float32)
    partials = torch.empty(rows * 2 * (Co * Co + Co), device=x.device, dtype=torch.float32)
    call("coskad_layer_apply_next_flat_f32", ptr(Z), ptr(x), ptr(out), ptr(wfold), ptr(bias), ptr(in_slope), ptr(out_slope), ptr(A_next),
         ptr(T_next), ptr(Zn), ptr(partials), ctypes.c_size_t(_bytes(partials)), i32(B), i32(Ci), i32(Co), i32(T), i32(V), _stream(),
         tag=(Ci, Co))
    return out, Zn, partials, rows


def layer_train_fold(partials, rows, B, T, V, Wt, bt, gt, bet, rm_t, rv_t, nbt_t, Wr, br, gr, ber, rm_r, rv_r, nbt_r, ws,
                     momentum: float = 0.1):
    Co, Ci = Wt.shape
    _chk(partials, "partials"); _chk(Wt, "Wt", (Co, Ci)); _chk(gt, "gamma_t", (Co,)); _chk(bet, "beta_t", (Co,))
    for n, t in (("bt", bt), ("rm_t", rm_t), ("rv_t", rv_t), ("br", br), ("gamma_r", gr), ("beta_r", ber),
                 ("rm_r", rm_r), ("rv_r", rv_r)):
        _chk(t, n, (Co,), optional=True)
    _chk(Wr, "Wr", (Co, Ci), optional=True)
    _chk(nbt_t, "nbt_t", (), dtype=torch.int64, optional=True)
    _chk(nbt_r, "nbt_r", (), dtype=torch.int64, optional=True)
    if partials.numel() < rows * 2 * (Ci * Ci + Ci):
        raise ValueError("layer_train_fold: partials smaller than rows x 2 (Ci^2 + Ci)")
    need = train_stats_ws_bytes(Ci)
    if ws is None or _bytes(ws) < need:
        raise ValueError(f"workspace too small: need {need} bytes")
# ... 113 lines not shown
        raise ValueError(f"workspace too small: need {need} bytes")
    if need_dx and dIn is None:
        dIn = torch.empty_like(x_in)
    call("coskad_layer_bwd_data_f32", ptr(x_in), ptr(dU), ptr(A), ptr(Tm), ptr(in_slope), ptr(stat), ptr(Wt), ptr(gt),
         ptr(Wr), ptr(gr), ptr(dIn if need_dx else None), ptr(dZ), ptr(grads["Wt"]), ptr(grads.get("bt")),
         ptr(grads["gt"]), ptr(grads["bet"]), ptr(grads.get("Wr")), ptr(grads.get("br")), ptr(grads.get("gr")),
         ptr(grads.get("ber")), ptr(grads.get("slope_in")), ptr(ws), ctypes.c_size_t(_bytes(ws)),
         i32(1 if accumulate else 0), i32(B), i32(Ci), i32(Co), i32(T), i32(V), _stream(), ptr(Z))
    return dIn if need_dx else None


def layer_gcn_params_ws_bytes(T, V) -> int:
    fn = _lib.lib().coskad_layer_gcn_params_ws_bytes
    fn.restype = ctypes.c_size_t
    return fn(i32(T), i32(V))


def layer_gcn_params(x_in, in_slope, dZ, A, Tm, dA, dT, ws, accumulate=False):
    B, Ci, T, V = x_in.shape
    _chk(x_in, "x_in"); _chk(dZ, "dZ", (B, Ci, T, V)); _chk(A, "A", (T, V, V)); _chk(Tm, "T", (V, T, T))
    _chk(dA, "dA", (T, V, V)); _chk(dT, "dT", (V, T, T)); _chk(in_slope, "in_slope", (1,), optional=True)
    if ws is None or _bytes(ws) < layer_gcn_params_ws_bytes(T, V):
        raise ValueError("workspace too small")
    call("coskad_layer_gcn_params_f32", ptr(x_in), ptr(in_slope), ptr(dZ), ptr(A), ptr(Tm), ptr(dA), ptr(dT), ptr(ws),
         ctypes.c_size_t(_bytes(ws)), i32(1 if accumulate else 0), i32(B), i32(Ci), i32(T), i32(V), _stream())


def btlnk_fwd(U: Tensor, W: Tensor, bias: Optional[Tensor], slope: Optional[Tensor], ws=None) -> Tensor:
    B = U.shape[0]
    K = U.numel() // B
    L = W.shape[0]
    _chk(U, "U"); _chk(W, "W", (L, K)); _chk(bias, "bias", (L,), optional=True); _chk(slope, "slope", (1,), optional=True)
    z = torch.empty(B, L, device=U.device, dtype=torch.float32)
    if L > 16:
        fn = _lib.lib().coskad_btlnk_fwd_ws_bytes_l
        fn.restype = ctypes.c_size_t
        nbytes = fn(i32(B), i32(K), i32(L))
        buf = ws.get(nbytes, U.device) if ws is not None else torch.empty(nbytes, dtype=torch.uint8, device=U.device)
        call("coskad_btlnk_fwd_ws_f32", ptr(U), ptr(W), ptr(bias), ptr(slope), ptr(z), ptr(buf), ctypes.c_size_t(nbytes),
             i32(B), i32(K), i32(L), _stream())
        return z
    if B >= BTLNK_SPLITK_MIN_B and K % 16 == 0:
        fn = _lib.lib().coskad_btlnk_fwd_ws_bytes
        fn.restype = ctypes.c_size_t
        nbytes = fn(i32(B))
        buf = ws.get(nbytes, U.device) if ws is not None else torch.empty(nbytes, dtype=torch.uint8, device=U.device)
        call("coskad_btlnk_fwd_ws_f32", ptr(U), ptr(W), ptr(bias), ptr(slope), ptr(z), ptr(buf), ctypes.c_size_t(nbytes),
             i32(B), i32(K), i32(L), _stream())
        return z
    call("coskad_btlnk_fwd_f32", ptr(U), ptr(W), ptr(bias), ptr(slope), ptr(z), i32(B), i32(K), i32(L), _stream())
    return z


BTLNK_SPLITK_MIN_B = 1
BTLNK_LMAX = 512


def btlnk_bwd_ws_bytes(B, K, L) -> int:
    fn = _lib.lib().coskad_btlnk_bwd_ws_bytes
    fn.restype = ctypes.c_size_t
    return fn(i32(B), i32(K), i32(L))


def btlnk_bwd(U, W, dz, slope, dW, db, dslope, ws, dU=None, accumulate=False):
    B = U.shape[0]
    K = U.numel() // B
    L = W.shape[0]
    _chk(U, "U"); _chk(W, "W", (L, K)); _chk(dz, "dz", (B, L)); _chk(dW, "dW", (L, K))
    _chk(db, "db", (L,), optional=True); _chk(dslope, "dslope", (1,), optional=True); _chk(slope, "slope", (1,), optional=True)
    need = btlnk_bwd_ws_bytes(B, K, L)
    if ws is None or _bytes(ws) < need:
        raise ValueError(f"workspace too small: need {need} bytes")
    if dU is None:
        dU = torch.empty_like(U)
    call("coskad_btlnk_bwd_f32", ptr(U), ptr(W), ptr(dz), ptr(slope), ptr(dU), ptr(dW), ptr(db), ptr(dslope), ptr(ws),
         ctypes.c_size_t(_bytes(ws)), i32(1 if accumulate else 0), i32(B), i32(K), i32(L), _stream())
    return dU


def btlnk_bwd_chain_ok(K: int, TV: int, below_Ci: int) -> bool:
    fn = _lib.lib().coskad_btlnk_bwd_chain_ok
    fn.restype = ctypes.c_int
    return bool(fn(i32(K), i32(TV), i32(below_Ci)))


def btlnk_bwd_chain(U, W, dz, slope, dW, db, dslope, ws, below_in, below_Z, below_in_slope, dU=None, accumulate=False):
    B, Ch, T, V = U.shape
    TV = T * V
    K = Ch * TV
    L = W.shape[0]
    Ci = below_in.shape[1]
    _chk(U, "U"); _chk(W, "W", (L, K)); _chk(dz, "dz", (B, L)); _chk(dW, "dW", (L, K))
    _chk(db, "db", (L,), optional=True); _chk(dslope, "dslope", (1,), optional=True); _chk(slope, "slope", (1,), optional=True)
    _chk(below_in, "below_in", (B, Ci, T, V)); _chk(below_Z, "below_Z", (B, Ci, T, V)); _chk(below_in_slope, "below_in_slope", (1,), optional=True)
    if not btlnk_bwd_chain_ok(K, TV, Ci):
        raise ValueError(f"btlnk_bwd_chain: shape K={K} TV={TV} Ci={Ci} not supported")
    lib = _lib.lib()
    lib.coskad_btlnk_bwd_chain_ws_bytes.restype = ctypes.c_size_t
    lib.coskad_btlnk_bwd_chain_floats.restype = ctypes.c_size_t
    need = lib.coskad_btlnk_bwd_chain_ws_bytes(i32(B), i32(K), i32(L), i32(TV))
    buf = ws.get(need, U.device)
    stats = torch.empty(lib.coskad_btlnk_bwd_chain_floats(i32(B), i32(TV), i32(Ci)), device=U.device, dtype=torch.float32)
    if dU is None:
        dU = torch.empty_like(U)
    rows = ctypes.c_int(0)
    call("coskad_btlnk_bwd_chain_f32", ptr(U), ptr(W), ptr(dz), ptr(slope), ptr(dU), ptr(dW), ptr(db), ptr(dslope), ptr(buf),
         ctypes.c_size_t(_bytes(buf)), i32(1 if accumulate else 0), i32(B), i32(K), i32(L), ptr(below_in), ptr(below_Z),
         ptr(below_in_slope), i32(Ci), i32(TV), ptr(stats), ctypes.c_size_t(_bytes(stats)), ctypes.byref(rows), _stream())
    return dU, (stats, rows.value)


def _cuda_f32(t: Tensor, name: str) -> None:
    if not t.is_cuda:
        raise _lib.CoskadHipError(f"{name}: expected a CUDA (ROCm) tensor, got device {t.device}; no CPU fallback")
    if t.dtype != torch.float32:
        raise TypeError(f"{name}: expected float32, got {t.dtype}")


def _b3(t: Tensor):
    if t.dim() == 2:
        return 1, t.shape[0], t.shape[1], 0, t.stride(0), t.stride(1)
    if t.dim() == 3:
        return t.shape[0], t.shape[1], t.shape[2], t.stride(0), t.stride(1), t.stride(2)
    raise ValueError("gemm operands are 2-D or 3-D")


def gemm(A: Tensor, B: Tensor, out: Optional[Tensor] = None, bias: Optional[Tensor] = None, bias_mode: int = 0,
         bias_mod: int = 1, relu: bool = False, accumulate: bool = False) -> Tensor:
    _cuda_f32(A, "A"); _cuda_f32(B, "B")
    ba, M, K, sab, sam, sak = _b3(A)
    bb, K2, N, sbb, sbk, sbn = _b3(B)
    if K != K2:
        raise ValueError(f"gemm: inner sizes differ ({K} vs {K2})")
    batch = max(ba, bb)
    if ba not in (1, batch) or bb not in (1, batch):
        raise ValueError("gemm: batch sizes do not broadcast")
    if ba == 1:
        sab = 0
    if bb == 1:
        sbb = 0
    if out is None:
        out = torch.empty((batch, M, N) if (A.dim() == 3 or B.dim() == 3) else (M, N), device=A.device, dtype=torch.float32)
    _cuda_f32(out, "out")
    bc, Mc, Nc, scb, scm, scn = _b3(out)
    if (Mc, Nc) != (M, N) or bc != batch:
        raise ValueError(f"gemm: out has shape {tuple(out.shape)}, expected batch {batch} x {M} x {N}")
    _chk(bias, "bias", optional=True)
    ll = ctypes.c_longlong
    call("coskad_gemm_f32", ptr(A), ptr(B), ptr(out), ptr(bias), ll(sab), ll(sam), ll(sak), ll(sbb), ll(sbk), ll(sbn),
         ll(scb), ll(scm), ll(scn), i32(M), i32(N), i32(K), i32(batch), i32(bias_mode), i32(bias_mod), i32(1 if relu else 0),
         i32(0), i32(0), ll(0), i32(1 if accumulate else 0), _stream())
    return out


def gemm_reduce(A: Tensor, B: Tensor, out: Tensor, target_chunks: int = 64, ktotal: int = 0, accumulate: bool = False) -> Tensor:
    _cuda_f32(A, "A"); _cuda_f32(B, "B"); _chk(out, "out")
    ba, M, K, sab, sam, sak = _b3(A)
    bb, K2, N, sbb, sbk, sbn = _b3(B)
    if K != K2 or ba != bb or tuple(out.shape) != (M, N):
        raise ValueError("gemm_reduce: shape mismatch")
    chunk = max(1, (ba + target_chunks - 1) // target_chunks)
# ... 660 lines not shown
```

coskad_amd/trainer.py:

```python
from __future__ import annotations

from typing import Dict, List, Optional

import torch
import torch.distributed as dist

from . import engine, ops, parallel
from .models.graph_layers.stsgcn import layer_tensors

Tensor = torch.Tensor


class FlatParams:

    def __init__(self, module: torch.nn.Module) -> None:
        named = [(n, p) for n, p in module.named_parameters()]
        self.names = [n for n, _ in named]
        al = lambda k: (k + 3) // 4 * 4
        total = sum(al(p.numel()) for _, p in named)
        dev = named[0][1].device
        self.flat = torch.zeros(total, device=dev, dtype=torch.float32)
        self.grad = torch.zeros(total, device=dev, dtype=torch.float32)
        self.reg_mask = torch.zeros(total, device=dev, dtype=torch.float32)
        self.views: Dict[str, Tensor] = {}
# ... 330 lines not shown
            g = {"gamma": gv[bname + "weight"], "beta": gv[bname + "bias"], "W2": gv[lname + "weight"], "b2": gv.get(lname + "bias")}
            d = ops.mlp_head_bwd(y_in, stat, bn.weight, bn.bias, lin.weight, d, g, True)
        return d


class STSETrainStep(_FlatStep, _OneClassHead):

    def __init__(self, model, lr: float = 1e-4, alpha: float = 1e-6, head: str = 'euclidean',
                 betas=(0.9, 0.999), eps: float = 1e-8, process_group=None, use_graph: bool = False,
                 side_stream: bool = False, sync_bn: bool = False) -> None:
        from .models.sts.ae import STSE
        from .models.common.components import MLP
        self.mlp = isinstance(model.btlnk, MLP)
        if not isinstance(model, STSE) or not (isinstance(model.btlnk, torch.nn.Linear) or (self.mlp and model.btlnk.hip_ok)):
            raise TypeError("STSETrainStep drives an STSE with projector='linear' or an 'mlp' within the kernels' widths")
        super().__init__(model, lr, alpha, betas, eps, process_group)
        self.head = head
        dev = self.fp.flat.device
        self.hyper = torch.tensor([lr, 1.0, 1.0, 0.0], device=dev, dtype=torch.float32)
        L = model.latent_dim
        self.center_acc = torch.zeros(ops.head_slots(L), device=dev, dtype=torch.float32)
        self.gram_acc = torch.zeros(L, L, device=dev, dtype=torch.float32) if head == 'mahalanobis' else None
        wide = any(l.is_wide for l in model.encoder.model)
        if wide and (side_stream or use_graph):
            raise ValueError("an encoder with wide layers runs on the main stream, outside hipGraph capture")
        self.side = engine.SideStream() if side_stream else None
        self.sync_group = None
        if sync_bn and self.world > 1:
            if self.mlp or side_stream or use_graph or wide:
                raise ValueError("sync_bn: encoder BatchNorm only (STS-GCN encoder within the tile kernels, linear projector), on the "
                                 "main stream, outside hipGraph capture")
            self.sync_group = process_group if process_group is not None else dist.group.WORLD
        plain = not wide and (use_graph or side_stream or sync_bn or not any(_is_commute(l) for l in model.encoder.model))
        self.stack = _FlatStack(list(model.encoder.model), self.fp, "encoder.model.", plain=plain, side=self.side, sync=self.sync_group)
        names = self.fp.names
        first_tail = next((i for i, n in enumerate(names) if n.startswith("btlnk.")), None)
        tail = first_tail is not None and all(n.startswith("btlnk.") for n in names[first_tail:])
        self.tail_off = self.fp.offsets[names[first_tail]] if tail else None
        if use_graph and any(isinstance(b, torch.nn.modules.batchnorm._BatchNorm) and b.momentum is None for b in model.modules()):
            raise ValueError("use_graph: BatchNorm with momentum=None changes its averaging factor every step (a launch argument here); "
                             "capture needs a fixed momentum")
        self.use_graph = use_graph
        self._graph = self._x_static = self._stats_static = None

    @property
    def layers(self) -> List[engine.LayerTensors]:
        segs = self.stack.segs
        return segs[0].layers if len(segs) == 1 and segs[0].kind == 'tile' else []

    def set_lr(self, lr: float) -> None:
        self.hyper[0] = lr
        self.lr = float(lr)

    def _body(self, x: Tensor) -> Tensor:
        m, gv = self.model, self.fp.gviews
        U, slope, saved_stack = self.stack.forward(x, self.ws)
        ctx, top_layers = self.stack.top(saved_stack)
        if self.mlp:
            wname, W = "btlnk.net.0.", m.btlnk.net[0].weight
            z, saved = self._mlp_forward(U, slope)
        else:
            wname, W = "btlnk.", m.btlnk.weight
            z = ops.btlnk_fwd(U, W, m.btlnk.bias, slope, ws=self.ws)
        stats, dz = self._head(z)
        if self.mlp:
            dz = self._mlp_backward(saved, dz)
        dU, top_stats = engine.btlnk_backward(ctx if self.side is None else None, top_layers or [], U, W, dz, slope, gv[wname + "weight"],
                                              gv.get(wname + "bias"), self.stack.last_slope_grad, self.ws)
        work = None
        if self.world > 1 and self.tail_off is not None:
            work = dist.all_reduce(self.fp.grad[self.tail_off:], group=self.pg, async_op=True)
        self.stack.backward(saved_stack, dU, self.ws, need_dx=False, top_stats=top_stats)
        if self.world > 1:
            head = self.fp.grad if work is None else self.fp.grad[:self.tail_off]
            dist.all_reduce(head, group=self.pg)
            if work is not None:
                work.wait()
        self._adam()
        return stats

    def step(self, x: Tensor) -> Tensor:
        self.steps += 1
        x = x.contiguous()
        if not self.use_graph:
            return self._body(x)
        if self._graph is None or self._x_static.shape != x.shape:
            self._x_static = x.clone()
            s = torch.cuda.Stream()
            s.wait_stream(torch.cuda.current_stream())
            with torch.cuda.stream(s):
                self._body(self._x_static)
            torch.cuda.current_stream().wait_stream(s)
            self.steps += 1
            self._graph = torch.cuda.CUDAGraph()
            with torch.cuda.graph(self._graph):
                self._stats_static = self._body(self._x_static)
        self._x_static.copy_(x)
        self._graph.replay()
        return self._stats_static


class STSAETrainStep(_FlatStep):

    def __init__(self, model, mode: str = 'ae', lr: float = 1e-4, alpha: float = 0.0, lambda_: float = 0.01, phi: float = 1.0,
                 beta: float = 1.0, gamma: float = 1.0, betas=(0.9, 0.999), eps: float = 1e-8, process_group=None) -> None:
        from .models.sts.ae import STSAE
        from .models.sts.vae import STSVAE
        from .models.common.components import Encoder
        if not isinstance(model, STSAE) or not isinstance(model.encoder, Encoder):
            raise TypeError("STSAETrainStep drives an STSAE / STSVAE with the STS-GCN encoder")
        if mode not in ('ae', 'vae') or (mode == 'vae') != isinstance(model, STSVAE):
            raise ValueError(f"mode {mode!r} does not fit {type(model).__name__}")
        if not self.supports(model):
            raise TypeError("STSAETrainStep: projector / latent size outside the bottleneck kernels (latent rows <= 16, "
                            "'linear' projector)")
        super().__init__(model, lr, alpha, betas, eps, process_group)
        self.mode = mode
        self.lambda_, self.phi, self.beta, self.gamma = float(lambda_), float(phi), float(beta), float(gamma)
        self.enc = _FlatStack(list(model.encoder.model), self.fp, "encoder.model.")
        from . import lowrank
        dec_layers = list(model.decoder.model)
# ... 201 lines not shown
```

include/coskad_hip.h:

```cpp
#ifndef COSKAD_HIP_H
#define COSKAD_HIP_H
#include <hip/hip_runtime_api.h>

#ifdef __cplusplus
extern "C" {
#endif

int coskad_abi_version(void);
const char* coskad_last_error(void);

int coskad_probe_begin(int kernel, int Ci, int Co);
int coskad_probe_stride(int n);
int coskad_probe_end(float* avg_ms, int* launches);


int coskad_gcn_f32(const float* in, float* out, const float* A, const float* Tm, int rows, int T, int V,
                   int adjoint, hipStream_t stream);

int coskad_bn_fold_f32(const float* Wt, const float* bt, const float* gamma_t, const float* beta_t,
                       const float* mean_t, const float* var_t, const float* Wr, const float* br,
                       const float* gamma_r, const float* beta_r, const float* mean_r,
                       const float* var_r, float* wfold, float* bias, int Ci, int Co,
                       hipStream_t stream);

int coskad_layer_apply_f32(const float* in, float* out, const float* A, const float* Tm,
                           const float* wfold, const float* bias, const float* in_slope,
                           const float* out_slope, int B, int Ci, int Co, int T, int V,
                           hipStream_t stream);

int coskad_prelu_fwd_f32(const float* u, const float* slope, float* out, size_t n, hipStream_t stream);
int coskad_prelu_bwd_f32(const float* u, const float* dout, const float* slope, float* du, float* dslope,
                         float* ws, int accumulate, size_t n, hipStream_t stream);

int coskad_rec_head_f32(const float* U, const float* x, const float* slope, float* xrec, float* dU, float* loss, float* dslope,
                        float upstream, float* ws, int accumulate, size_t n, hipStream_t stream);

size_t coskad_rev_btlnk_ws_floats(int B, int N, int L);
int coskad_rev_btlnk_fwd_f32(const float* z, const float* W, const float* bias, float* H, int B, int N, int L, hipStream_t stream);
int coskad_rev_btlnk_bwd_f32(const float* dH, const float* z, const float* W, float* dz, int dz_accumulate, float* dW, float* db,
                             int accumulate, float* ws, int B, int N, int L, hipStream_t stream);


size_t coskad_train_stats_ws_bytes(int Ci);
int coskad_stat_floats(int Ci, int Co);

int coskad_layer_train_stats_f32(const float* in, const float* A, const float* Tm, const float* in_slope,
                                 const float* Wt, const float* bt, const float* gamma_t,
                                 const float* beta_t, float* rmean_t, float* rvar_t, long long* nbt_t,
                                 const float* Wr, const float* br, const float* gamma_r,
                                 const float* beta_r, float* rmean_r, float* rvar_r, long long* nbt_r,
                                 float momentum, float* wfold, float* bias, float* stat, void* ws,
                                 size_t ws_bytes, int B, int Ci, int Co, int T, int V,
                                 hipStream_t stream);

int coskad_layer_train_stats_z_f32(const float* in, const float* A, const float* Tm, const float* in_slope,
                                   const float* Wt, const float* bt, const float* gamma_t,
                                   const float* beta_t, float* rmean_t, float* rvar_t, long long* nbt_t,
                                   const float* Wr, const float* br, const float* gamma_r,
                                   const float* beta_r, float* rmean_r, float* rvar_r, long long* nbt_r,
                                   float momentum, float* wfold, float* bias, float* stat, void* ws,
                                   size_t ws_bytes, int B, int Ci, int Co, int T, int V,
                                   hipStream_t stream, float* Z);
int coskad_layer_apply_z_f32(const float* Z, const float* in, float* out, const float* A, const float* Tm,
                             const float* wfold, const float* bias, const float* in_slope, const float* out_slope,
                             int B, int Ci, int Co, int T, int V, hipStream_t stream);

int coskad_layer_apply_next_ok(int Ci, int Co, int T, int V);
int coskad_ftab_floats(void);
int coskad_layer_apply_next_rows(int B, int Ci, int Co);
int coskad_build_ftab_f32(const float* const* A, const float* const* Tm, float* const* tab, int n, int T, int V,
                          hipStream_t stream);
int coskad_layer_apply_next_f32(const float* Z, const float* in, float* out, const float* wfold, const float* bias,
                                const float* in_slope, const float* out_slope, const float* ftab_next, float* Z_next,
                                float* partials, size_t partials_bytes, int B, int Ci, int Co, int T, int V,
                                hipStream_t stream);
int coskad_layer_train_fold_f32(const float* partials, int rows, const float* Wt, const float* bt, const float* gamma_t,
                                const float* beta_t, float* rmean_t, float* rvar_t, long long* nbt_t,
                                const float* Wr, const float* br, const float* gamma_r,
                                const float* beta_r, float* rmean_r, float* rvar_r, long long* nbt_r,
                                float momentum, float* wfold, float* bias, float* stat, void* ws,
                                size_t ws_bytes, int B, int Ci, int Co, int T, int V, hipStream_t stream);

int coskad_gather_f32(const float* src, const int* idx, float* out, size_t n, hipStream_t stream);
int coskad_fused_encoder_out_floats(void);
int coskad_fused_encoder_f32(const float* x, float* out, const float* tab, const float* wreg, const float* slopes, int B,
                             int T, int V, hipStream_t stream);

int coskad_gemm_f32(const float* A, const float* B, float* C, const float* bias, long long sa_b, long long sa_m,
                    long long sa_k, long long sb_b, long long sb_k, long long sb_n, long long sc_b, long long sc_m,
                    long long sc_n, int M, int N, int K, int batch, int bias_mode, int bias_mod, int relu, int reduce,
                    int chunk, long long ktotal, int accum, hipStream_t stream);
int coskad_gemm_sum_f32(const float* partials, int chunks, size_t E, float* out, int accumulate, hipStream_t stream);
int coskad_relu_bwd_f32(const float* out, const float* dout, float* g, float* part, int Nb, int C, int P, int slices,
                        hipStream_t stream);
int coskad_softmax_rows_f32(const float* x, float* y, int n, hipStream_t stream);
int coskad_softmax_rows_bwd_f32(const float* y, const float* dy, float* dx, int n, hipStream_t stream);

int coskad_conv1x1_ok(int M, int K, int P);
int coskad_conv1x1_stat_rows(int M, int K, int P, int batch);
int coskad_conv1x1_f32(const float* A, long long sa_m, long long sa_k, const float* In, float* Out, const float* bias, double* stats,
                       int M, int K, int P, int batch, int accumulate, hipStream_t stream);
int coskad_bn2_stats_parts_f32(const double* parts, int rows, float* stat, float* running_mean, float* running_var,
                               long long* num_batches_tracked, float momentum, float eps, double count, int C, hipStream_t stream);
int coskad_conv1x1_wgrad_ok(int M, int K, int P);
int coskad_conv1x1_wgrad_f32(const float* G, const float* X, float* partials, int M, int K, int P, int batch, int chunk,
                             hipStream_t stream);

size_t coskad_bn2_ws_bytes(int Nb, int C);
size_t coskad_bn2_bwd_ws_bytes(int Nb, int C);
int coskad_bn2_stats_f32(const float* x, float* stat, float* running_mean, float* running_var, long long* num_batches_tracked,
                         float momentum, float eps, int training, void* ws, size_t ws_bytes, int Nb, int C, int P,
                         hipStream_t stream);
int coskad_bn2_apply_prelu_f32(const float* Ct, const float* Cr, const float* stat_t, const float* gamma_t, const float* beta_t,
                               const float* stat_r, const float* gamma_r, const float* beta_r, const float* slope, float* out,
                               int Nb, int C, int P, hipStream_t stream, float drop_p, unsigned long long drop_seed);
// ... 41 lines not shown
size_t coskad_layer_bwd_stats_floats(int B, int Ci, int Co, int T, int V);
size_t coskad_layer_bwd_sums_offset(int rows, int Ci, int Co);
int coskad_layer_bwd_stats_f32(const float* in, const float* dU, const float* A, const float* Tm, const float* in_slope,
                               int has_residual, float* stats_out, size_t stats_out_bytes, int* rows_out, void* ws, size_t ws_bytes,
                               int B, int Ci, int Co, int T, int V, hipStream_t stream, const float* Z);

int coskad_layer_bwd_f32(const float* in, const float* dU, const float* A, const float* Tm,
                         const float* in_slope, const float* stat, const float* Wt, const float* gamma_t,
                         const float* Wr, const float* gamma_r, float* dIn, float* dA, float* dT, float* dWt,
                         float* dbt, float* dgamma_t, float* dbeta_t, float* dWr, float* dbr,
                         float* dgamma_r, float* dbeta_r, float* dslope_in, void* ws, size_t ws_bytes,
                         int accumulate, int B, int Ci, int Co, int T, int V, hipStream_t stream);

int coskad_layer_bwd_z_f32(const float* in, const float* dU, const float* A, const float* Tm,
                           const float* in_slope, const float* stat, const float* Wt, const float* gamma_t,
                           const float* Wr, const float* gamma_r, float* dIn, float* dA, float* dT, float* dWt,
                           float* dbt, float* dgamma_t, float* dbeta_t, float* dWr, float* dbr,
                           float* dgamma_r, float* dbeta_r, float* dslope_in, void* ws, size_t ws_bytes,
                           int accumulate, int B, int Ci, int Co, int T, int V, hipStream_t stream, const float* Z);

int coskad_layer_bwd_data_f32(const float* in, const float* dU, const float* A, const float* Tm,
                              const float* in_slope, const float* stat, const float* Wt, const float* gamma_t,
                              const float* Wr, const float* gamma_r, float* dIn, float* dZ, float* dWt, float* dbt,
                              float* dgamma_t, float* dbeta_t, float* dWr, float* dbr, float* dgamma_r,
                              float* dbeta_r, float* dslope_in, void* ws, size_t ws_bytes, int accumulate, int B,
                              int Ci, int Co, int T, int V, hipStream_t stream, const float* Z );
size_t coskad_layer_gcn_params_ws_bytes(int T, int V);
int coskad_layer_gcn_params_f32(const float* in, const float* in_slope, const float* dZ, const float* A,
                                const float* Tm, float* dA, float* dT, void* ws, size_t ws_bytes, int accumulate,
                                int B, int Ci, int T, int V, hipStream_t stream);

size_t coskad_gcn_bwd_params_ws_bytes(int T, int V);
int coskad_gcn_bwd_params_f32(const float* x, const float* dZ, const float* A, const float* Tm, float* dA,
                              float* dT, void* ws, size_t ws_bytes, int accumulate, int rows, int T, int V,
                              hipStream_t stream);

int coskad_gcn_bwd_params_dx_f32(const float* x, const float* dZ, const float* A, const float* Tm, float* dA, float* dT,
                                 float* dX, const float* dX_add, void* ws, size_t ws_bytes, int accumulate, int rows, int T,
                                 int V, hipStream_t stream);


int coskad_btlnk_fwd_f32(const float* U, const float* W, const float* bias, const float* slope, float* z,
                         int B, int K, int L, hipStream_t stream);

size_t coskad_btlnk_fwd_ws_bytes(int B);
size_t coskad_btlnk_fwd_ws_bytes_l(int B, int K, int L);
int coskad_btlnk_fwd_ws_f32(const float* U, const float* W, const float* bias, const float* slope, float* z, void* ws,
                            size_t ws_bytes, int B, int K, int L, hipStream_t stream);
size_t coskad_btlnk_bwd_ws_bytes(int B, int K, int L);
int coskad_btlnk_bwd_f32(const float* U, const float* W, const float* dz, const float* slope, float* dU,
                         float* dW, float* db, float* dslope, void* ws, size_t ws_bytes, int accumulate,
                         int B, int K, int L, hipStream_t stream);

int coskad_btlnk_bwd_chain_ok(int K, int TV, int below_Ci);
int coskad_btlnk_bwd_chain_rows(int B, int TV);
size_t coskad_btlnk_bwd_chain_floats(int B, int TV, int below_Ci);
size_t coskad_btlnk_bwd_chain_ws_bytes(int B, int K, int L, int TV);
int coskad_btlnk_bwd_chain_f32(const float* U, const float* W, const float* dz, const float* slope, float* dU, float* dW,
                               float* db, float* dslope, void* ws, size_t ws_bytes, int accumulate, int B, int K, int L,
                               const float* below_in, const float* below_Z, const float* below_in_slope, int below_Ci, int TV,
                               float* stats_out, size_t stats_out_bytes, int* stats_rows, hipStream_t stream);


int coskad_gather_transform_f32(const float* xy, const long long* index, const float* mats, float* out, int B, int N,
                                int ntrans, int TV, hipStream_t stream);


int coskad_head_slots(void);
size_t coskad_head_ws_floats(int B);
int coskad_head_slots_l(int L);
size_t coskad_head_ws_floats_l(int B, int L);

int coskad_mse_head_f32(const float* z, const float* c, float* dz, float* score, float* stats, float* acc,
                        float upstream, float* ws, int B, int L, hipStream_t stream);

int coskad_mahalanobis_head_f32(const float* z, const float* c, const float* VI, float* dz, float* score,
                                float* stats, float* acc, float* gram, int gram_accumulate, float upstream,
                                float* ws, int B, int L, hipStream_t stream);

int coskad_poincare_head_f32(const float* z, const float* c, float* dz, float* zh, float* score,
                             float* stats, float* acc, float upstream, float* ws, int B, int L,
                             hipStream_t stream);
int coskad_poincare_dist_f32(const float* zh, const float* c, float* score, int B, int L, hipStream_t stream);
int coskad_poincare_logmap0_f32(const float* y, float* out, int B, int L, hipStream_t stream);

int coskad_lowrank_fold_ok(int latent, int TV);
int coskad_lowrank_fold_fwd_f32(const float* X, const double* G, const float* gamma0, const float* beta0, const float* cbias0,
                                float* rmean0, float* rvar0, long long* nbt0, float momentum0, float eps0, const float* gamma1,
                                const float* beta1, const float* cbias1, float* rmean1, float* rvar1, long long* nbt1, float momentum1,
                                float eps1, double n_pos, float* Mw, float* Mb, double* saved, double* xbar, double* xx, int Co, int TV,
                                hipStream_t stream);
int coskad_lowrank_fold_bwd_f32(const float* X, const double* G, const float* dMw, const float* dMb, const double* saved,
                                const double* xbar, const double* xx, const float* gamma0, const float* gamma1, double n_pos, float* dX,
                                float* dgamma, float* dbeta, double* dGc, int Co, int TV, hipStream_t stream);

int coskad_narrow_conv_rows(int B, int TV);
int coskad_narrow_conv_fwd_f32(const float* U, const float* in_slope, const float* W, float* out, int B, int Ci, int J, int TV,
                               hipStream_t stream);
int coskad_narrow_conv_bwd_f32(const float* U, const float* in_slope, const float* W, const float* dOut, float* dU, float* partials,
                               size_t partials_floats, int B, int Ci, int J, int TV, hipStream_t stream);

int coskad_layer_apply_next_flat_ok(int Ci, int Co, int T, int V);
int coskad_layer_apply_next_flat_rows(int B);
int coskad_layer_apply_next_flat_f32(const float* Z, const float* in, float* out, const float* wfold, const float* bias,
                                     const float* in_slope, const float* out_slope, const float* A_next, const float* T_next,
                                     float* Z_next, float* partials, size_t partials_bytes, int B, int Ci, int Co, int T, int V,
                                     hipStream_t stream);

int coskad_layer_first_pair_ok(int T, int V, int Ci, int Cm, int Co);
int coskad_layer_first_pair_apply_f32(const float* x, float* out, const float* A1, const float* T1, const float* wfold1, const float* bias1,
                                      const float* A2, const float* T2, const float* wfold2, const float* bias2, const float* mid_slope,
                                      const float* out_slope, int B, int Cm, int Co, int T, int V, hipStream_t stream);

int coskad_commute_ok(int T, int V, int Ci, int Co);
// ... 44 lines not shown
```

Before: 2.978 million clips/s.

## Fuse bottleneck split-K sum into MSE head and defer head finalize to bwd reduce

The bottleneck forward now feeds its split-K partials straight into the MSE head kernel, which sums the partials, adds the bias, writes z and computes dz in one pass, removing the separate btlnk_fwd_sum launch. The head's finalize step becomes a pending rider block on the bottleneck backward reduce kernel instead of its own launch. The ftab build is also refactored into a shared helper, and a stats+ftab layer entry point appears in the header. The aim is fewer small kernel launches per train step, at the cost of more plumbing and a dependency on stats being finalized later in the step.

Result: no change. 2.983 million clips/s, median of 6 (+0.2%).

```diff
diff --git a/coskad_amd/csrc/bottleneck.hip b/coskad_amd/csrc/bottleneck.hip
--- a/coskad_amd/csrc/bottleneck.hip
+++ b/coskad_amd/csrc/bottleneck.hip
@@ -1,4 +1,5 @@
 #include "tile_ops.h"
+#include "heads_common.h"
 
 namespace coskad {
 
@@ -229,8 +230,13 @@
                                                        const float* __restrict__ dap, int nda,
                                                        float* __restrict__ dslope, int accumulate,
                                                        const float* __restrict__ rows, int RP, int RE,
-                                                       double* __restrict__ rsum) {
+                                                       double* __restrict__ rsum, const float* __restrict__ hpart, int HP,
+                                                       float hscale0, float* __restrict__ hstats, float* __restrict__ hacc) {
   __shared__ double sh[256];
+  if (hpart && blockIdx.x == gridDim.x - 1) {
+    if (threadIdx.x < kHeadSlots) head_finalize_slot(hpart, HP, hscale0, hstats, hacc, threadIdx.x);
+    return;
+  }
   const unsigned nE = (unsigned)((E + 255) / 256);
   if (blockIdx.x > nE + L) {
     const int col = threadIdx.x & 15, slice = threadIdx.x >> 4;
@@ -304,14 +310,31 @@
   return s < 1 ? 1 : s;
 }
 
+int launch_btlnk_reduce_head(const float* partials, int P, size_t E, float* out, const float* dz, int B, int L, float* db,
+                             const float* dap, int nda, float* dslope, int accumulate, hipStream_t stream, const float* rows,
+                             int RP, int RE, double* rsum, const float* hpart, int HP, float hscale0, float* hstats, float* hacc) {
+  const unsigned extra = rows ? (unsigned)ceil_div(RE, 16) : 0u;
+  const unsigned rider = hpart ? 1u : 0u;
+  hipLaunchKernelGGL(k_btlnk_reduce, dim3((unsigned)((E + 255) / 256) + L + 1 + extra + rider), dim3(256), 0, stream, partials, P, E, out,
+                     dz, B, L, db, dap, nda, dslope, accumulate, rows, RP, RE, rsum, hpart, HP, hscale0, hstats, hacc);
+  return check_launch("btlnk_bwd_reduce");
+}
 int launch_btlnk_reduce(const float* partials, int P, size_t E, float* out, const float* dz, int B, int L, float* db,
                         const float* dap, int nda, float* dslope, int accumulate, hipStream_t stream, const float* rows,
                         int RP, int RE, double* rsum) {
-  const unsigned extra = rows ? (unsigned)ceil_div(RE, 16) : 0u;
-  hipLaunchKernelGGL(k_btlnk_reduce, dim3((unsigned)((E + 255) / 256) + L + 1 + extra), dim3(256), 0, stream, partials, P, E, out, dz,
-                     B, L, db, dap, nda, dslope, accumulate, rows, RP, RE, rsum);
-  return check_launch("btlnk_bwd_reduce");
-}
+  return launch_btlnk_reduce_head(partials, P, E, out, dz, B, L, db, dap, nda, dslope, accumulate, stream, rows, RP, RE, rsum, nullptr, 0,
+                                  0.f, nullptr, nullptr);
+}
+
+int check_head_pending(const char* who, const float* hpart, int HP, const float* hstats, const float* hacc) {
+  if (!hpart) return (HP || hstats || hacc) ? fail(COSKAD_ERR_ARG, "%s: head statistics without partial rows", who) : 0;
+  if (HP < 1 || (!hstats && !hacc)) return fail(COSKAD_ERR_ARG, "%s: head partial rows=%d need stats or acc", who, HP);
+  return 0;
+}
+
+int launch_mse_head_parts(const float* part, int KS, const float* bias, const float* c, float* z, float* dz, float* score, float* stats,
+                          float* acc, float upstream, float* ws, int B, int L, hipStream_t stream, int* pending_rows,
+                          float* pending_scale0);
 
 constexpr int kBtlWideMax = 512;
 size_t wide_btlnk_fwd_ws_bytes(int B, int K, int L);
@@ -363,16 +386,49 @@
   return check_launch("btlnk_fwd_sum");
 }
 
+int coskad_btlnk_mse_head_f32(const float* U, const float* W, const float* bias, const float* slope, const float* c, float* z,
+                              float* dz, float* score, float* stats, float* acc, float upstream, void* ws, size_t ws_bytes,
+                              float* head_ws, int B, int K, int L, int* pending_rows, float* pending_scale0, hipStream_t stream) {
+  if (!U || !W || !c || !z || !ws || !head_ws || !pending_rows || !pending_scale0)
+    return fail(COSKAD_ERR_ARG, "btlnk_mse_head: null pointer");
+  if (B <= 0 || K <= 0 || L <= 0) return fail(COSKAD_ERR_ARG, "btlnk_mse_head: B=%d K=%d L=%d", B, K, L);
+  if (L > 16) return fail(COSKAD_ERR_SHAPE, "btlnk_mse_head: latent_dim=%d > 16 not supported", L);
+  if (K % 16) return fail(COSKAD_ERR_SHAPE, "btlnk_mse_head: K=%d must be a multiple of 16", K);
+  if (ws_bytes < coskad_btlnk_fwd_ws_bytes(B)) return fail(COSKAD_ERR_WORKSPACE, "btlnk_mse_head: workspace too small");
+  if ((size_t)ws & 15) return fail(COSKAD_ERR_ARG, "btlnk_mse_head: workspace must be 16-byte aligned");
+  float* part = reinterpret_cast<float*>(ws);
+  hipLaunchKernelGGL(k_btlnk_fwd_t, dim3(ceil_div(B, 64), kBtlKS), dim3(256), 0, stream, U, W, slope, part, B, K, L);
+  int rc;
+  if ((rc = check_launch("btlnk_fwd_t"))) return rc;
+  return launch_mse_head_parts(part, kBtlKS, bias, c, z, dz, score, stats, acc, upstream, head_ws, B, L, stream, pending_rows,
+                               pending_scale0);
+}
+
 size_t coskad_btlnk_bwd_ws_bytes(int B, int K, int L) {
   if (L > 16 && L <= kBtlWideMax) return wide_btlnk_bwd_ws_bytes(B, K, L);
   const int S = btl_chunks(B, K);
   return ((size_t)S * L * K + (size_t)S * ceil_div(K, 256) + 64) * sizeof(float);
 }
 
+int coskad_btlnk_bwd_head_f32(const float* U, const float* W, const float* dz, const float* slope, float* dU,
+                              float* dW, float* db, float* dslope, void* ws, size_t ws_bytes, int accumulate,
+                              int B, int K, int L, const float* head_partials, int head_rows, float head_scale0,
+                              float* head_stats, float* head_acc, hipStream_t stream);
+
 int coskad_btlnk_bwd_f32(const float* U, const float* W, const float* dz, const float* slope, float* dU,
                          float* dW, float* db, float* dslope, void* ws, size_t ws_bytes, int accumulate,
                          int B, int K, int L, hipStream_t stream) {
+  return coskad_btlnk_bwd_head_f32(U, W, dz, slope, dU, dW, db, dslope, ws, ws_bytes, accumulate, B, K, L, nullptr, 0, 0.f, nullptr,
+                                   nullptr, stream);
+}
+
+int coskad_btlnk_bwd_head_f32(const float* U, const float* W, const float* dz, const float* slope, float* dU,
+                              float* dW, float* db, float* dslope, void* ws, size_t ws_bytes, int accumulate,
+                              int B, int K, int L, const float* head_partials, int head_rows, float head_scale0,
+                              float* head_stats, float* head_acc, hipStream_t stream) {
   if (!U || !W || !dz || !dU || !dW || !ws) return fail(COSKAD_ERR_ARG, "btlnk_bwd: null pointer");
+  if (int hrc = check_head_pending("btlnk_bwd", head_partials, head_rows, head_stats, head_acc)) return hrc;
+  if (head_partials && L > 16) return fail(COSKAD_ERR_SHAPE, "btlnk_bwd: a pending head finalize needs latent_dim <= 16 (got %d)", L);
   if (B <= 0 || K <= 0 || L <= 0) return fail(COSKAD_ERR_ARG, "btlnk_bwd: B=%d K=%d L=%d", B, K, L);
   if (L > kBtlWideMax) return fail(COSKAD_ERR_SHAPE, "btlnk_bwd: latent_dim=%d > %d not supported", L, kBtlWideMax);
   if (ws_bytes < coskad_btlnk_bwd_ws_bytes(B, K, L)) return fail(COSKAD_ERR_WORKSPACE, "btlnk_bwd: workspace too small");
@@ -389,8 +445,8 @@
   }
   int rc = check_launch("btlnk_bwd");
   if (rc) return rc;
-  return launch_btlnk_reduce(dWp, S, (size_t)L * K, dW, dz, B, L, db, dap, gx * S, (dslope && slope) ? dslope : nullptr, accumulate, stream,
-                             nullptr, 0, 0, nullptr);
-}
-
-}
+  return launch_btlnk_reduce_head(dWp, S, (size_t)L * K, dW, dz, B, L, db, dap, gx * S, (dslope && slope) ? dslope : nullptr, accumulate,
+                                  stream, nullptr, 0, 0, nullptr, head_partials, head_rows, head_scale0, head_stats, head_acc);
+}
+
+}
diff --git a/coskad_amd/csrc/btlnk_chain.hip b/coskad_amd/csrc/btlnk_chain.hip
--- a/coskad_amd/csrc/btlnk_chain.hip
+++ b/coskad_amd/csrc/btlnk_chain.hip
@@ -248,6 +248,10 @@
 int launch_btlnk_reduce(const float* partials, int P, size_t E, float* out, const float* dz, int B, int L, float* db,
                         const float* dap, int nda, float* dslope, int accumulate, hipStream_t stream, const float* rows,
                         int RP, int RE, double* rsum);
+int launch_btlnk_reduce_head(const float* partials, int P, size_t E, float* out, const float* dz, int B, int L, float* db,
+                             const float* dap, int nda, float* dslope, int accumulate, hipStream_t stream, const float* rows,
+                             int RP, int RE, double* rsum, const float* hpart, int HP, float hscale0, float* hstats, float* hacc);
+int check_head_pending(const char* who, const float* hpart, int HP, const float* hstats, const float* hacc);
 }
 
 using namespace coskad;
@@ -275,10 +279,27 @@
   return ((size_t)p.S * L * K + (size_t)p.S * p.npt + 64) * sizeof(float);
 }
 
+int coskad_btlnk_bwd_chain_head_f32(const float* U, const float* W, const float* dz, const float* slope, float* dU, float* dW,
+                                    float* db, float* dslope, void* ws, size_t ws_bytes, int accumulate, int B, int K, int L,
+                                    const float* below_in, const float* below_Z, const float* below_in_slope, int below_Ci, int TV,
+                                    float* stats_out, size_t stats_out_bytes, int* stats_rows, const float* head_partials,
+                                    int head_rows, float head_scale0, float* head_stats, float* head_acc, hipStream_t stream);
+
 int coskad_btlnk_bwd_chain_f32(const float* U, const float* W, const float* dz, const float* slope, float* dU, float* dW,
                                float* db, float* dslope, void* ws, size_t ws_bytes, int accumulate, int B, int K, int L,
                                const float* below_in, const float* below_Z, const float* below_in_slope, int below_Ci, int TV,
                                float* stats_out, size_t stats_out_bytes, int* stats_rows, hipStream_t stream) {
+  return coskad_btlnk_bwd_chain_head_f32(U, W, dz, slope, dU, dW, db, dslope, ws, ws_bytes, accumulate, B, K, L, below_in, below_Z,
+                                         below_in_slope, below_Ci, TV, stats_out, stats_out_bytes, stats_rows, nullptr, 0, 0.f, nullptr,
+                                         nullptr, stream);
+}
+
+int coskad_btlnk_bwd_chain_head_f32(const float* U, const float* W, const float* dz, const float* slope, float* dU, float* dW,
+                                    float* db, float* dslope, void* ws, size_t ws_bytes, int accumulate, int B, int K, int L,
+                                    const float* below_in, const float* below_Z, const float* below_in_slope, int below_Ci, int TV,
+                                    float* stats_out, size_t stats_out_bytes, int* stats_rows, const float* head_partials,
+                                    int head_rows, float head_scale0, float* head_stats, float* head_acc, hipStream_t stream) {
+  if (int hrc = check_head_pending("btlnk_bwd_chain", head_partials, head_rows, head_stats, head_acc)) return hrc;
   if (!U || !W || !dz || !dU || !dW || !ws || !below_in || !below_Z || !stats_out || !stats_rows)
     return fail(COSKAD_ERR_ARG, "btlnk_bwd_chain: null pointer");
   if (B <= 0 || K <= 0 || L <= 0) return fail(COSKAD_ERR_ARG, "btlnk_bwd_chain: B=%d K=%d L=%d", B, K, L);
@@ -312,8 +333,9 @@
   }
   if ((rc = check_launch("btlnk_bwd_stats"))) return rc;
   *stats_rows = rows;
-  return launch_btlnk_reduce(dWp, p.S, (size_t)L * K, dW, dz, B, L, db, dap, rows, (dslope && slope) ? dslope : nullptr, accumulate, stream,
-                             stats_out, rows, E, reinterpret_cast<double*>(stats_out + bc::sums_offset(rows, E)));
-}
-
-}
+  return launch_btlnk_reduce_head(dWp, p.S, (size_t)L * K, dW, dz, B, L, db, dap, rows, (dslope && slope) ? dslope : nullptr, accumulate,
+                                  stream, stats_out, rows, E, reinterpret_cast<double*>(stats_out + bc::sums_offset(rows, E)),
+                                  head_partials, head_rows, head_scale0, head_stats, head_acc);
+}
+
+}
diff --git a/coskad_amd/csrc/fused_apply_next.hip b/coskad_amd/csrc/fused_apply_next.hip
--- a/coskad_amd/csrc/fused_apply_next.hip
+++ b/coskad_amd/csrc/fused_apply_next.hip
@@ -9,30 +9,11 @@
 
 using namespace ff;
 
-struct FtabArgs {
-  const float* A[4];
-  const float* Tm[4];
-  float* tab[4];
-};
 __global__ void k_build_ftab(FtabArgs args) {
   const int layer = blockIdx.y;
-  const float* __restrict__ Aw = args.A[layer];
-  const float* __restrict__ Tw = args.Tm[layer];
   const int e = blockIdx.x * blockDim.x + threadIdx.x;
   if (e >= LAYER_F4 * 4) return;
-  float val = 0.f;
-  if (e < TEMP_F4 * 4) {
-    const int v = e / 256, l = (e >> 2) & 63, s = e & 3, j = l & 15, q = l >> 4;
-    if (s < 3 && j < T) val = Tw[v * T * T + (4 * s + q) * T + j];
-  } else {
-    const int r = e - TEMP_F4 * 4;
-    const int t = r / (3 * 256), c = (r / 256) % 3, l = (r >> 2) & 63, k = 4 * c + (r & 3), j = l & 15, q = l >> 4;
-    if (k < 10) {
-      const int s = k < 5 ? k : k - 5, w = 4 * s + q;
-      if (w < V) val = Aw[t * V * V + w * V + (k < 5 ? j : 16)];
-    }
-  }
-  args.tab[layer][e] = val;
+  args.tab[layer][e] = ftab_value(args.A[layer], args.Tm[layer], e);
 }
 
 template <int CT, int OTP>
diff --git a/coskad_amd/csrc/fused_ops.h b/coskad_amd/csrc/fused_ops.h
--- a/coskad_amd/csrc/fused_ops.h
+++ b/coskad_amd/csrc/fused_ops.h
@@ -33,6 +33,27 @@
 constexpr int TEMP_F4 = V * 64;
 constexpr int LAYER_F4 = TEMP_F4 + T * 3 * 64;
 enum { W1A = 0, W1B = 2, WP = 4, WR = 12, WX3 = 20, WZ3 = 28, WZ4 = 36, WX4 = 68, B1 = 100, B2 = 108, B3 = 112, B4 = 120, NWREG = 136 };
+
+struct FtabArgs {
+  const float* A[4];
+  const float* Tm[4];
+  float* tab[4];
+};
+__device__ __forceinline__ float ftab_value(const float* __restrict__ Aw, const float* __restrict__ Tw, int e) {
+  float val = 0.f;
+  if (e < TEMP_F4 * 4) {
+    const int v = e / 256, l = (e >> 2) & 63, s = e & 3, j = l & 15, q = l >> 4;
+    if (s < 3 && j < T) val = Tw[v * T * T + (4 * s + q) * T + j];
+  } else {
+    const int r = e - TEMP_F4 * 4;
+    const int t = r / (3 * 256), c = (r / 256) % 3, l = (r >> 2) & 63, k = 4 * c + (r & 3), j = l & 15, q = l >> 4;
+    if (k < 10) {
+      const int s = k < 5 ? k : k - 5, w = 4 * s + q;
+      if (w < V) val = Aw[t * V * V + w * V + (k < 5 ? j : 16)];
+    }
+  }
+  return val;
+}
 
 __device__ __forceinline__ f32x4 mfma(float a, float b, f32x4 c) {
   return __builtin_amdgcn_mfma_f32_16x16x4f32(a, b, c, 0, 0, 0);
diff --git a/coskad_amd/csrc/heads.hip b/coskad_amd/csrc/heads.hip
--- a/coskad_amd/csrc/heads.hip
+++ b/coskad_amd/csrc/heads.hip
@@ -107,7 +107,6 @@
   return gu;
 }
 
-constexpr int kHeadSlots = LMAX + 3;
 
 constexpr int kHeadSingleRows = kFlatBlock;
 __host__ __device__ inline int head_blocks(int B) { return B <= kHeadSingleRows ? 1 : ceil_div(B, kFlatBlock); }
@@ -134,7 +133,37 @@
   }
 }
 
-__global__ __launch_bounds__(kFlatBlock) void k_mse_head(const float* __restrict__ z,
+struct RowFromZ {
+  const float* __restrict__ z;
+  __device__ __forceinline__ Vec load(int n, int L) const { return load_vec(z + (size_t)n * L, L); }
+};
+struct RowFromParts {
+  const float* __restrict__ part;
+  const float* __restrict__ bias;
+  float* __restrict__ z;
+  int B, KS;
+  __device__ __forceinline__ Vec load(int n, int L) const {
+    float s[LMAX];
+#pragma unroll
+    for (int j = 0; j < LMAX; ++j) s[j] = 0.f;
+    for (int k = 0; k < KS; ++k) {
+      const float4* p = reinterpret_cast<const float4*>(part + ((size_t)k * B + n) * 16);
+#pragma unroll
+      for (int q = 0; q < LMAX / 4; ++q) {
+        const float4 v = p[q];
+        s[4 * q] += v.x; s[4 * q + 1] += v.y; s[4 * q + 2] += v.z; s[4 * q + 3] += v.w;
+      }
+    }
+    Vec r;
+#pragma unroll
+    for (int j = 0; j < LMAX; ++j) r.v[j] = j < L ? s[j] + (bias ? bias[j] : 0.f) : 0.f;
+    store_vec(z + (size_t)n * L, r, L);
+    return r;
+  }
+};
+
+template <class Row>
+__global__ __launch_bounds__(kFlatBlock) void k_mse_head(const Row row,
                                                     const float* __restrict__ cvec,
                                                     float* __restrict__ dz, float* __restrict__ score,
                                                     float* __restrict__ partials, int B, int L,
@@ -146,7 +175,7 @@
   const Vec c = load_vec(cvec, L);
 #pragma unroll 4
   for (int n = blockIdx.x * kFlatBlock + threadIdx.x; n < B; n += gridDim.x * kFlatBlock) {
-    const Vec u = load_vec(z + (size_t)n * L, L);
+    const Vec u = row.load(n, L);
     Vec g;
     float sq = 0.f;
 #pragma unroll
@@ -272,12 +301,7 @@
 __global__ __launch_bounds__(64) void k_head_finalize(const float* __restrict__ partials, int P,
                                                        float scale0, float* __restrict__ stats,
                                                        float* __restrict__ acc) {
-  const int k = threadIdx.x;
-  if (k >= kHeadSlots) return;
-  double s = 0.0;
-  for (int p = 0; p < P; ++p) s += (double)partials[p * kHeadSlots + k];
-  if (stats) stats[k] = (float)(k == 0 ? s * (double)scale0 : s);
-  if (acc) acc[k] += (float)s;
+  if (threadIdx.x < kHeadSlots) head_finalize_slot(partials, P, scale0, stats, acc, threadIdx.x);
 }
 
 __global__ __launch_bounds__(kFlatBlock) void k_poincare_dist(const float* __restrict__ zh,
@@ -396,6 +420,18 @@
   if (threadIdx.x == 0) out[0] = (float)(sh[0] * (double)scale);
 }
 
+int launch_mse_head_parts(const float* part, int KS, const float* bias, const float* c, float* z, float* dz, float* score, float* stats,
+                          float* acc, float upstream, float* ws, int B, int L, hipStream_t stream, int* pending_rows,
+                          float* pending_scale0) {
+  const int P = head_blocks(B);
+  const float scale0 = 1.f / ((float)B * (float)L);
+  hipLaunchKernelGGL(k_mse_head<RowFromParts>, dim3(P), dim3(kFlatBlock), 0, stream, RowFromParts{part, bias, z, B, KS}, c, dz, score,
+                     ws, B, L, upstream / ((float)B * (float)L), scale0, stats, acc);
+  *pending_rows = ((stats || acc) && P > 1) ? P : 0;
+  *pending_scale0 = scale0;
+  return check_launch("btlnk_mse_head");
+}
+
 }
 
 using namespace coskad;
@@ -416,7 +452,7 @@
   if (B <= 0 || L <= 0 || L > kWideLMax) return fail(COSKAD_ERR_SHAPE, "mse_head: B=%d latent=%d (max %d)", B, L, kWideLMax);
   if (L > LMAX) return wide_mse_head(z, c, dz, score, stats, acc, upstream, ws, B, L, stream);
   const int P = head_blocks(B);
-  hipLaunchKernelGGL(k_mse_head, dim3(P), dim3(kFlatBlock), 0, stream, z, c, dz, score, ws, B, L,
+  hipLaunchKernelGGL(k_mse_head<RowFromZ>, dim3(P), dim3(kFlatBlock), 0, stream, RowFromZ{z}, c, dz, score, ws, B, L,
                      upstream / ((float)B * (float)L), 1.f / ((float)B * (float)L), stats, acc);
   if ((stats || acc) && P > 1)
     hipLaunchKernelGGL(k_head_finalize, dim3(1), dim3(64), 0, stream, ws, P, 1.f / ((float)B * (float)L), stats, acc);
diff --git a/coskad_amd/csrc/heads_common.h b/coskad_amd/csrc/heads_common.h
--- a/coskad_amd/csrc/heads_common.h
+++ b/coskad_amd/csrc/heads_common.h
@@ -14,6 +14,15 @@
 __host__ __device__ inline int head_lp(int L) { return L > LMAX ? L : LMAX; }
 __host__ __device__ inline int head_slots_for(int L) { return head_lp(L) + 3; }
 
+constexpr int kHeadSlots = LMAX + 3;
+__device__ __forceinline__ void head_finalize_slot(const float* __restrict__ partials, int P, float scale0, float* __restrict__ stats,
+                                                   float* __restrict__ acc, int k) {
+  double s = 0.0;
+  for (int p = 0; p < P; ++p) s += (double)partials[p * kHeadSlots + k];
+  if (stats) stats[k] = (float)(k == 0 ? s * (double)scale0 : s);
+  if (acc) acc[k] += (float)s;
+}
+
 size_t wide_head_ws_floats(int B, int L);
 int wide_mse_head(const float* z, const float* c, float* dz, float* score, float* stats, float* acc, float upstream, float* ws,
                   int B, int L, hipStream_t stream);
diff --git a/coskad_amd/csrc/stsgcn_train.hip b/coskad_amd/csrc/stsgcn_train.hip
--- a/coskad_amd/csrc/stsgcn_train.hip
+++ b/coskad_amd/csrc/stsgcn_train.hip
@@ -1,4 +1,5 @@
 #include "mfma_ops.h"
+#include "fused_ops.h"
 
 namespace coskad {
 
@@ -68,6 +69,7 @@
 #endif
 
 constexpr int kFoldSelfSum = 48;
+constexpr int kFtabBlocks = (ff::LAYER_F4 * 4 + 1023) / 1024;
 __global__ __launch_bounds__(1024) void k_train_fold(
     const double* __restrict__ red, double npos, const float* __restrict__ Wt,
     const float* __restrict__ bt, const float* __restrict__ gs, const float* __restrict__ bs,
@@ -76,7 +78,13 @@
     const float* __restrict__ brr, float* __restrict__ rm_r, float* __restrict__ rv_r,
     long long* __restrict__ nbt_r, float momentum, float* __restrict__ wfold,
     float* __restrict__ bias, float* __restrict__ stat, int Ci, int Co, int CoP,
-    const float* __restrict__ parts, int P) {
+    const float* __restrict__ parts, int P, int nfold, int nft, ff::FtabArgs ft) {
+  if ((int)blockIdx.x >= nfold) {
+    const int r = (int)blockIdx.x - nfold, layer = r / kFtabBlocks;
+    const int e = (r - layer * kFtabBlocks) * 1024 + (int)threadIdx.x;
+    if (layer < nft && e < ff::LAYER_F4 * 4) ft.tab[layer][e] = ff::ftab_value(ft.A[layer], ft.Tm[layer], e);
+    return;
+  }
   extern __shared__ double shd[];
   const bool ident = Wr == nullptr;
   const int CC = Co * Ci;
@@ -111,7 +119,7 @@
   float* mean_r = istd_s + Co;
   float* istd_r = mean_r + Co;
   const double inv_n = 1.0 / npos;
-  const int chunk = (Co + gridDim.x - 1) / gridDim.x;
+  const int chunk = (Co + nfold - 1) / nfold;
   const int o_lo = blockIdx.x * chunk, o_hi = min(Co, o_lo + chunk), no = max(0, o_hi - o_lo);
   const bool first = blockIdx.x == 0;
 
@@ -216,7 +224,7 @@
   }
   __syncthreads();
   TFOLD_STAMP(3);
-  const bool last = blockIdx.x == gridDim.x - 1;
+  const bool last = (int)blockIdx.x == nfold - 1;
   const int w_hi = last ? CoP : min(o_lo + chunk, CoP), nw = max(0, w_hi - o_lo);
   for (int i = threadIdx.x; i < 2 * Ci * nw; i += blockDim.x) {
     const int row = i / nw, o = o_lo + i - row * nw;
@@ -263,7 +271,8 @@
 static int launch_reduce_fold(const float* partials, int rows, double* red, double npos, const float* Wt, const float* bt,
                               const float* gs, const float* bs, float* rm_s, float* rv_s, long long* nbt_s, const float* Wr,
                               const float* br, const float* gr, const float* brr, float* rm_r, float* rv_r, long long* nbt_r,
-                              float momentum, float* wfold, float* bias, float* stat, int Ci, int Co, hipStream_t st) {
+                              float momentum, float* wfold, float* bias, float* stat, int Ci, int Co, hipStream_t st,
+                              const ff::FtabArgs* ft = nullptr, int nft = 0) {
   const int E = 2 * (Ci * Ci + Ci);
   int rc = 0;
   const bool self_sum = partials && Wt && E <= kFoldSelfSum;
@@ -275,9 +284,11 @@
   const size_t fold_lds = (2 * (size_t)Ci * Ci + 2 * Ci) * sizeof(double) + (4 * (size_t)Co * Ci + 4 * Co) * sizeof(float);
   if (fold_lds > 64 * 1024) (void)hipFuncSetAttribute((const void*)k_train_fold, hipFuncAttributeMaxDynamicSharedMemorySize, (int)fold_lds);
   const int fold_blocks = Co >= 32 ? 8 : (Co >= 16 ? 4 : 1);
-  hipLaunchKernelGGL(k_train_fold, dim3(fold_blocks), dim3(1024), fold_lds, st, red, npos, Wt, bt, gs, bs, rm_s,
+  if (!ft) nft = 0;
+  hipLaunchKernelGGL(k_train_fold, dim3(fold_blocks + nft * kFtabBlocks), dim3(1024), fold_lds, st, red, npos, Wt, bt, gs, bs, rm_s,
                      rv_s, nbt_s, Wr, br, gr, brr, rm_r, rv_r, nbt_r, momentum, wfold, bias, stat, Ci,
-                     Co, round_up(Co, 16), self_sum ? partials : (const float*)nullptr, rows);
+                     Co, round_up(Co, 16), self_sum ? partials : (const float*)nullptr, rows, fold_blocks, nft,
+                     ft ? *ft : ff::FtabArgs{});
   return check_launch("train_fold");
 }
 
@@ -288,7 +299,8 @@
                               const float* br, const float* gr, const float* brr, float* rm_r,
                               float* rv_r, long long* nbt_r, float momentum, float* wfold, float* bias,
                               float* stat, void* ws, size_t ws_bytes, int B, int Ci, int Co,
-                              hipStream_t st, float* Zout = nullptr, double* sums_out = nullptr, int need_x_sums = 1) {
+                              hipStream_t st, float* Zout = nullptr, double* sums_out = nullptr, int need_x_sums = 1,
+                              const ff::FtabArgs* ft = nullptr, int nft = 0) {
   constexpr int kBlock = Geo<T, V>::Block;
   constexpr int kScratchFloats = Geo<T, V>::Scratch;
   constexpr int TV = Geo<T, V>::TV, LD = TV + 2;
@@ -339,7 +351,7 @@
     return launch_reduce_fold(partials, rows, sums_out, 0.0, nullptr, nullptr, nullptr, nullptr, nullptr, nullptr, nullptr, nullptr,
                               nullptr, nullptr, nullptr, nullptr, nullptr, nullptr, 0.f, nullptr, nullptr, nullptr, Ci, Co, st);
   return launch_reduce_fold(partials, rows, red, (double)B * TV, Wt, bt, gs, bs, rm_s, rv_s, nbt_s, Wr, br, gr, brr, rm_r, rv_r,
-                            nbt_r, momentum, wfold, bias, stat, Ci, Co, st);
+                            nbt_r, momentum, wfold, bias, stat, Ci, Co, st, ft, nft);
 }
 
 }
@@ -393,6 +405,31 @@
 #undef CALL
 }
 
+int coskad_layer_train_stats_ftab_f32(const float* in, const float* A, const float* Tm, const float* in_slope,
+                                      const float* Wt, const float* bt, const float* gamma_t,
+                                      const float* beta_t, float* rmean_t, float* rvar_t, long long* nbt_t,
+                                      const float* Wr, const float* br, const float* gamma_r,
+                                      const float* beta_r, float* rmean_r, float* rvar_r, long long* nbt_r,
+                                      float momentum, float* wfold, float* bias, float* stat, void* ws,
+                                      size_t ws_bytes, int B, int Ci, int Co, int T, int V, hipStream_t stream, float* Z,
+                                      const float* const* ftab_A, const float* const* ftab_T, float* const* ftab, int n) {
+  if (!in || !A || !Tm || !Wt || !gamma_t || !beta_t || !wfold || !bias || !stat || !ws || !ftab_A || !ftab_T || !ftab)
+    return fail(COSKAD_ERR_ARG, "layer_train_stats_ftab: null pointer");
+  if (Wr && (!gamma_r || !beta_r)) return fail(COSKAD_ERR_ARG, "layer_train_stats_ftab: residual BN missing");
+  if (!Wr && Ci != Co) return fail(COSKAD_ERR_ARG, "layer_train_stats_ftab: identity residual needs Ci == Co");
+  if (B <= 0 || Ci <= 0 || Co <= 0) return fail(COSKAD_ERR_ARG, "layer_train_stats_ftab: B=%d Ci=%d Co=%d", B, Ci, Co);
+  if (T != ff::T || V != ff::V) return fail(COSKAD_ERR_SHAPE, "layer_train_stats_ftab: built for T=12, V=17 (got %d, %d)", T, V);
+  if (n < 1 || n > 4) return fail(COSKAD_ERR_ARG, "layer_train_stats_ftab: 1..4 tables per launch, got %d", n);
+  ff::FtabArgs ft{};
+  for (int i = 0; i < n; ++i) {
+    if (!ftab_A[i] || !ftab_T[i] || !ftab[i]) return fail(COSKAD_ERR_ARG, "layer_train_stats_ftab: null pointer (table %d)", i);
+    ft.A[i] = ftab_A[i]; ft.Tm[i] = ftab_T[i]; ft.tab[i] = ftab[i];
+  }
+  return launch_train_stats<ff::T, ff::V>(in, A, Tm, in_slope, Wt, bt, gamma_t, beta_t, rmean_t, rvar_t, nbt_t, Wr, br, gamma_r, beta_r,
+                                          rmean_r, rvar_r, nbt_r, momentum, wfold, bias, stat, ws, ws_bytes, B, Ci, Co, stream, Z, nullptr,
+                                          1, &ft, n);
+}
+
 int coskad_layer_train_fold_f32(const float* partials, int rows, const float* Wt, const float* bt, const float* gamma_t,
                                 const float* beta_t, float* rmean_t, float* rvar_t, long long* nbt_t,
                                 const float* Wr, const float* br, const float* gamma_r,
diff --git a/coskad_amd/engine.py b/coskad_amd/engine.py
--- a/coskad_amd/engine.py
+++ b/coskad_amd/engine.py
@@ -121,15 +121,18 @@
     h, slope = x, in_slope
     n = len(layers)
     fuse = [False] * n
-    ftab = None
+    ftab = ftab_ride = None
     if all(batch_stats) and STORE_Z and FUSE_NEXT:
         for i in range(n - 1):
             fuse[i] = layers[i + 1].Ci == layers[i].Co and ops.layer_apply_next_ok(layers[i].Ci, layers[i].Co, T, V)
         nxt = [i + 1 for i in range(n - 1) if fuse[i]]
         if nxt:
             ftab = torch.empty(n, ops.ftab_floats(), device=x.device, dtype=torch.float32)
-            for k in range(0, len(nxt), 4):
-                grp = nxt[k:k + 4]
+            groups = [nxt[k:k + 4] for k in range(0, len(nxt), 4)]
+            if FUSE_FTAB and pending0 is None and sync is None:
+                ftab_ride = ([layers[i].A for i in groups[0]], [layers[i].T for i in groups[0]], [ftab[i] for i in groups[0]])
+                groups = groups[1:]
+            for grp in groups:
                 ops.build_ftabs([layers[i].A for i in grp], [layers[i].T for i in grp], [ftab[i] for i in grp])
     fuse_flat = [False] * n
     if all(batch_stats) and STORE_Z and FUSE_NEXT and sync is None:
@@ -180,7 +183,8 @@
                     Z = torch.empty_like(h)
                 wfold, bias, stat = ops.layer_train_stats(
                     h, L.A, L.T, slope, L.w2(L.Wt), L.bt, L.gt, L.bet, L.rm_t, L.rv_t, L.nbt_t,
-                    L.w2(L.Wr), L.br, L.gr, L.ber, L.rm_r, L.rv_r, L.nbt_r, buf, momentum=L.step_momentum(), Z=Z)
+                    L.w2(L.Wr), L.br, L.gr, L.ber, L.rm_r, L.rv_r, L.nbt_r, buf, momentum=L.step_momentum(), Z=Z,
+                    ftabs=ftab_ride if i == 0 else None)
         else:
             wfold, bias = eval_fold(L)
             stat = None
@@ -219,6 +223,8 @@
 CHAIN_SKIP = frozenset()
 FUSE_TOP = True
 FUSE_NEXT = True
+FUSE_FTAB = True
+FUSE_HEAD = True
 
 
 class SideStream:
@@ -240,7 +246,7 @@
 
 
 def btlnk_backward(ctx: Optional[ChainCtx], layers: List[LayerTensors], U: Tensor, W: Tensor, dz: Tensor, slope: Optional[Tensor],
-                   dW: Tensor, db: Optional[Tensor], dslope: Optional[Tensor], ws: Workspace):
+                   dW: Tensor, db: Optional[Tensor], dslope: Optional[Tensor], ws: Workspace, head=None):
     B = U.shape[0]
     K, L = U.numel() // B, W.shape[0]
     i = len(layers) - 1 if layers else -1
@@ -248,9 +254,9 @@
     if (FUSE_TOP and Z is not None and U.dim() == 4 and layers[i].Wr is not None and L <= 16
             and ops.btlnk_bwd_chain_ok(K, U.shape[2] * U.shape[3], layers[i].Ci)):
         in_slope = layers[i - 1].slope if i > 0 else ctx.in_slope
-        return ops.btlnk_bwd_chain(U, W, dz, slope, dW, db, dslope, ws, ctx.inputs[i], Z, in_slope)
+        return ops.btlnk_bwd_chain(U, W, dz, slope, dW, db, dslope, ws, ctx.inputs[i], Z, in_slope, head=head)
     buf = ws.get(ops.btlnk_bwd_ws_bytes(B, K, L), U.device)
-    return ops.btlnk_bwd(U, W, dz, slope, dW, db, dslope, buf), None
+    return ops.btlnk_bwd(U, W, dz, slope, dW, db, dslope, buf, head=head), None
 
 
 def chain_backward(ctx: ChainCtx, layers: List[LayerTensors], dU: Tensor, ws: Workspace,
diff --git a/coskad_amd/ops.py b/coskad_amd/ops.py
--- a/coskad_amd/ops.py
+++ b/coskad_amd/ops.py
@@ -113,7 +113,7 @@
 
 
 def layer_train_stats(x, A, Tm, in_slope, Wt, bt, gt, bet, rm_t, rv_t, nbt_t,
-                      Wr, br, gr, ber, rm_r, rv_r, nbt_r, ws, momentum: float = 0.1, Z: Optional[Tensor] = None):
+                      Wr, br, gr, ber, rm_r, rv_r, nbt_r, ws, momentum: float = 0.1, Z: Optional[Tensor] = None, ftabs=None):
     B, Ci, T, V = x.shape
     Co = Wt.shape[0]
     _chk(x, "x"); _chk(A, "A", (T, V, V)); _chk(Tm, "T", (V, T, T))
@@ -136,7 +136,9 @@
             ptr(bet), ptr(rm_t), ptr(rv_t), ptr(nbt_t), ptr(Wr), ptr(br), ptr(gr), ptr(ber), ptr(rm_r),
             ptr(rv_r), ptr(nbt_r), ctypes.c_float(momentum), ptr(wfold), ptr(bias), ptr(stat), ptr(ws),
             ctypes.c_size_t(ws.numel() * ws.element_size()), i32(B), i32(Ci), i32(Co), i32(T), i32(V), _stream())
-    if Z is None:
+    if ftabs is not None:
+        call("coskad_layer_train_stats_ftab_f32", *args, ptr(Z), *_ftab_args(*ftabs, T, V))
+    elif Z is None:
         call("coskad_layer_train_stats_f32", *args)
     else:
         call("coskad_layer_train_stats_z_f32", *args, ptr(Z))
@@ -237,17 +239,22 @@
     return fn()
 
 
-def build_ftabs(As, Ts, tabs) -> None:
+def _ftab_args(As, Ts, tabs, T: int, V: int):
     n = len(As)
     if not (1 <= n <= 4) or len(Ts) != n or len(tabs) != n:
-        raise ValueError("build_ftabs: 1..4 layers, equal list lengths")
-    T, V = As[0].shape[0], As[0].shape[1]
+        raise ValueError("mixing tables: 1..4 layers, equal list lengths")
     nf = ftab_floats()
     for A, Tm, tab in zip(As, Ts, tabs):
         _chk(A, "A", (T, V, V)); _chk(Tm, "T", (V, T, T)); _chk(tab, "tab", (nf,))
     arr = ctypes.c_void_p * n
-    call("coskad_build_ftab_f32", arr(*[t.data_ptr() for t in As]), arr(*[t.data_ptr() for t in Ts]),
-         arr(*[t.data_ptr() for t in tabs]), i32(n), i32(T), i32(V), _stream())
+    return arr(*[t.data_ptr() for t in As]), arr(*[t.data_ptr() for t in Ts]), arr(*[t.data_ptr() for t in tabs]), i32(n)
+
+
+def build_ftabs(As, Ts, tabs) -> None:
+    if not As:
+        raise ValueError("build_ftabs: 1..4 layers, equal list lengths")
+    T, V = As[0].shape[0], As[0].shape[1]
+    call("coskad_build_ftab_f32", *_ftab_args(As, Ts, tabs, T, V), i32(T), i32(V), _stream())
 
 
 def layer_apply_next(Z, x, wfold, bias, Co, in_slope, out_slope, ftab_next, partials, T, V, out=None, Z_next=None):
@@ -467,6 +474,47 @@
     return z
 
 
+def btlnk_mse_head_ok(K: int, L: int) -> bool:
+    return L <= 16 and K % 16 == 0 and BTLNK_SPLITK_MIN_B <= 1
+
+
+def btlnk_mse_head(U: Tensor, W: Tensor, bias: Optional[Tensor], slope: Optional[Tensor], c: Tensor, need_grad=True, need_score=False,
+                   acc=None, upstream=1.0, ws=None):
+    B = U.shape[0]
+    K = U.numel() // B
+    L = W.shape[0]
+    S = head_slots(L)
+    _chk(U, "U"); _chk(W, "W", (L, K)); _chk(bias, "bias", (L,), optional=True); _chk(slope, "slope", (1,), optional=True)
+    _chk(c, "c", (L,)); _chk(acc, "acc", (S,), optional=True)
+    if not btlnk_mse_head_ok(K, L):
+        raise ValueError(f"btlnk_mse_head: K={K} latent={L} not supported (K % 16 == 0, latent <= 16)")
+    fn = _lib.lib().coskad_btlnk_fwd_ws_bytes
+    fn.restype = ctypes.c_size_t
+    nbytes = fn(i32(B))
+    buf = ws.get(nbytes, U.device) if ws is not None else torch.empty(nbytes, dtype=torch.uint8, device=U.device)
+    hws = head_ws(B, U.device, L)
+    z = torch.empty(B, L, device=U.device, dtype=torch.float32)
+    dz = torch.empty_like(z) if need_grad else None
+    score = torch.empty(B, device=U.device, dtype=torch.float32) if need_score else None
+    stats = torch.empty(S, device=U.device, dtype=torch.float32)
+    rows, scale0 = ctypes.c_int(0), ctypes.c_float(0.0)
+    call("coskad_btlnk_mse_head_f32", ptr(U), ptr(W), ptr(bias), ptr(slope), ptr(c), ptr(z), ptr(dz), ptr(score), ptr(stats), ptr(acc),
+         ctypes.c_float(upstream), ptr(buf), ctypes.c_size_t(nbytes), ptr(hws), i32(B), i32(K), i32(L), ctypes.byref(rows),
+         ctypes.byref(scale0), _stream())
+    pending = (hws, rows.value, scale0.value, stats, acc) if rows.value else None
+    return z, stats, dz, score, pending
+
+
+def _head_args(head):
+    if head is None:
+        return ptr(None), i32(0), ctypes.c_float(0.0), ptr(None), ptr(None)
+    hws, rows, scale0, stats, acc = head
+    _chk(hws, "head partials"); _chk(stats, "head stats", optional=True); _chk(acc, "head acc", optional=True)
+    if hws.numel() < rows * HEAD_SLOTS:
+        raise ValueError("pending head: partial rows beyond the buffer")
+    return ptr(hws), i32(rows), ctypes.c_float(scale0), ptr(stats), ptr(acc)
+
+
 BTLNK_SPLITK_MIN_B = 1
 BTLNK_LMAX = 512
 
@@ -477,7 +525,7 @@
     return fn(i32(B), i32(K), i32(L))
 
 
-def btlnk_bwd(U, W, dz, slope, dW, db, dslope, ws, dU=None, accumulate=False):
+def btlnk_bwd(U, W, dz, slope, dW, db, dslope, ws, dU=None, accumulate=False, head=None):
     B = U.shape[0]
     K = U.numel() // B
     L = W.shape[0]
@@ -488,8 +536,12 @@
         raise ValueError(f"workspace too small: need {need} bytes")
     if dU is None:
         dU = torch.empty_like(U)
-    call("coskad_btlnk_bwd_f32", ptr(U), ptr(W), ptr(dz), ptr(slope), ptr(dU), ptr(dW), ptr(db), ptr(dslope), ptr(ws),
-         ctypes.c_size_t(_bytes(ws)), i32(1 if accumulate else 0), i32(B), i32(K), i32(L), _stream())
+    args = (ptr(U), ptr(W), ptr(dz), ptr(slope), ptr(dU), ptr(dW), ptr(db), ptr(dslope), ptr(ws),
+            ctypes.c_size_t(_bytes(ws)), i32(1 if accumulate else 0), i32(B), i32(K), i32(L))
+    if head is None:
+        call("coskad_btlnk_bwd_f32", *args, _stream())
+    else:
+        call("coskad_btlnk_bwd_head_f32", *args, *_head_args(head), _stream())
     return dU
 
 
@@ -499,7 +551,7 @@
     return bool(fn(i32(K), i32(TV), i32(below_Ci)))
 
 
-def btlnk_bwd_chain(U, W, dz, slope, dW, db, dslope, ws, below_in, below_Z, below_in_slope, dU=None, accumulate=False):
+def btlnk_bwd_chain(U, W, dz, slope, dW, db, dslope, ws, below_in, below_Z, below_in_slope, dU=None, accumulate=False, head=None):
     B, Ch, T, V = U.shape
     TV = T * V
     K = Ch * TV
@@ -519,9 +571,13 @@
     if dU is None:
         dU = torch.empty_like(U)
     rows = ctypes.c_int(0)
-    call("coskad_btlnk_bwd_chain_f32", ptr(U), ptr(W), ptr(dz), ptr(slope), ptr(dU), ptr(dW), ptr(db), ptr(dslope), ptr(buf),
-         ctypes.c_size_t(_bytes(buf)), i32(1 if accumulate else 0), i32(B), i32(K), i32(L), ptr(below_in), ptr(below_Z),
-         ptr(below_in_slope), i32(Ci), i32(TV), ptr(stats), ctypes.c_size_t(_bytes(stats)), ctypes.byref(rows), _stream())
+    args = (ptr(U), ptr(W), ptr(dz), ptr(slope), ptr(dU), ptr(dW), ptr(db), ptr(dslope), ptr(buf),
+            ctypes.c_size_t(_bytes(buf)), i32(1 if accumulate else 0), i32(B), i32(K), i32(L), ptr(below_in), ptr(below_Z),
+            ptr(below_in_slope), i32(Ci), i32(TV), ptr(stats), ctypes.c_size_t(_bytes(stats)), ctypes.byref(rows))
+    if head is None:
+        call("coskad_btlnk_bwd_chain_f32", *args, _stream())
+    else:
+        call("coskad_btlnk_bwd_chain_head_f32", *args, *_head_args(head), _stream())
     return dU, (stats, rows.value)
 
 
diff --git a/coskad_amd/trainer.py b/coskad_amd/trainer.py
--- a/coskad_amd/trainer.py
+++ b/coskad_amd/trainer.py
@@ -406,6 +406,14 @@
         self.hyper[0] = lr
         self.lr = float(lr)
 
+    def _head_fused_ok(self, U: Tensor, W: Tensor) -> bool:
+        return (engine.FUSE_HEAD and self.head == 'euclidean' and not self.mlp and self.side is None
+                and ops.btlnk_mse_head_ok(U.numel() // U.shape[0], W.shape[0]))
+
+    def _btlnk_head(self, U: Tensor, W: Tensor, bias, slope):
+        _, stats, dz, _, pending = ops.btlnk_mse_head(U, W, bias, slope, self.model.c, acc=self.center_acc, ws=self.ws)
+        return stats, dz, pending
+
     def _body(self, x: Tensor) -> Tensor:
         m, gv = self.model, self.fp.gviews
         U, slope, saved_stack = self.stack.forward(x, self.ws)
@@ -415,12 +423,17 @@
             z, saved = self._mlp_forward(U, slope)
         else:
             wname, W = "btlnk.", m.btlnk.weight
-            z = ops.btlnk_fwd(U, W, m.btlnk.bias, slope, ws=self.ws)
-        stats, dz = self._head(z)
+        pending = None
+        if self._head_fused_ok(U, W):
+            stats, dz, pending = self._btlnk_head(U, W, m.btlnk.bias, slope)
+        else:
+            if not self.mlp:
+                z = ops.btlnk_fwd(U, W, m.btlnk.bias, slope, ws=self.ws)
+            stats, dz = self._head(z)
         if self.mlp:
             dz = self._mlp_backward(saved, dz)
         dU, top_stats = engine.btlnk_backward(ctx if self.side is None else None, top_layers or [], U, W, dz, slope, gv[wname + "weight"],
-                                              gv.get(wname + "bias"), self.stack.last_slope_grad, self.ws)
+                                              gv.get(wname + "bias"), self.stack.last_slope_grad, self.ws, head=pending)
         work = None
         if self.world > 1 and self.tail_off is not None:
             work = dist.all_reduce(self.fp.grad[self.tail_off:], group=self.pg, async_op=True)
diff --git a/include/coskad_hip.h b/include/coskad_hip.h
--- a/include/coskad_hip.h
+++ b/include/coskad_hip.h
@@ -61,6 +61,14 @@
                                    float momentum, float* wfold, float* bias, float* stat, void* ws,
                                    size_t ws_bytes, int B, int Ci, int Co, int T, int V,
                                    hipStream_t stream, float* Z);
+int coskad_layer_train_stats_ftab_f32(const float* in, const float* A, const float* Tm, const float* in_slope,
+                                      const float* Wt, const float* bt, const float* gamma_t,
+                                      const float* beta_t, float* rmean_t, float* rvar_t, long long* nbt_t,
+                                      const float* Wr, const float* br, const float* gamma_r,
+                                      const float* beta_r, float* rmean_r, float* rvar_r, long long* nbt_r,
+                                      float momentum, float* wfold, float* bias, float* stat, void* ws,
+                                      size_t ws_bytes, int B, int Ci, int Co, int T, int V, hipStream_t stream, float* Z,
+                                      const float* const* ftab_A, const float* const* ftab_T, float* const* ftab, int n);
 int coskad_layer_apply_z_f32(const float* Z, const float* in, float* out, const float* A, const float* Tm,
                              const float* wfold, const float* bias, const float* in_slope, const float* out_slope,
                              int B, int Ci, int Co, int T, int V, hipStream_t stream);
@@ -208,6 +216,15 @@
                          float* dW, float* db, float* dslope, void* ws, size_t ws_bytes, int accumulate,
                          int B, int K, int L, hipStream_t stream);
 
+int coskad_btlnk_bwd_head_f32(const float* U, const float* W, const float* dz, const float* slope, float* dU,
+                              float* dW, float* db, float* dslope, void* ws, size_t ws_bytes, int accumulate,
+                              int B, int K, int L, const float* head_partials, int head_rows, float head_scale0,
+                              float* head_stats, float* head_acc, hipStream_t stream);
+
+int coskad_btlnk_mse_head_f32(const float* U, const float* W, const float* bias, const float* slope, const float* c, float* z,
+                              float* dz, float* score, float* stats, float* acc, float upstream, void* ws, size_t ws_bytes,
+                              float* head_ws, int B, int K, int L, int* pending_rows, float* pending_scale0, hipStream_t stream);
+
 int coskad_btlnk_bwd_chain_ok(int K, int TV, int below_Ci);
 int coskad_btlnk_bwd_chain_rows(int B, int TV);
 size_t coskad_btlnk_bwd_chain_floats(int B, int TV, int below_Ci);
@@ -216,6 +233,12 @@
                                float* db, float* dslope, void* ws, size_t ws_bytes, int accumulate, int B, int K, int L,
                                const float* below_in, const float* below_Z, const float* below_in_slope, int below_Ci, int TV,
                                float* stats_out, size_t stats_out_bytes, int* stats_rows, hipStream_t stream);
+
+int coskad_btlnk_bwd_chain_head_f32(const float* U, const float* W, const float* dz, const float* slope, float* dU, float* dW,
+                                    float* db, float* dslope, void* ws, size_t ws_bytes, int accumulate, int B, int K, int L,
+                                    const float* below_in, const float* below_Z, const float* below_in_slope, int below_Ci, int TV,
+                                    float* stats_out, size_t stats_out_bytes, int* stats_rows, const float* head_partials,
+                                    int head_rows, float head_scale0, float* head_stats, float* head_acc, hipStream_t stream);
 
 
 int coskad_gather_transform_f32(const float* xy, const long long* index, const float* mats, float* out, int B, int N,
```
